# BUTSpeechFIT/TS-ASR-Whisper

Measured on AMD Instinct MI355X. Metric: train utterances/sec (30 s clips) whisper-large-v3-turbo DiCoW, higher is better.
Workload: dtype bf16; 1 GPU; whisper-large-v3-turbo DiCoW fine-tune step, per-GPU batch 16, L=128, decoder frozen, bf16 AMP; global_batch=16, parallelism=dp1, split_streams=False, trainable_params=637306880

## Files before the change

### include/dicow_hip.h

```cpp
#ifndef DICOW_HIP_H
#define DICOW_HIP_H

#include <stdint.h>

#ifdef __cplusplus
extern "C" {
#endif

#define DICOW_OK 0
#define DICOW_ERR_INVALID (-1)
#define DICOW_ERR_LAUNCH (-2)

#define DICOW_ABI_VERSION 7

int dicow_abi_version(void);
int dicow_set_gemm_cus(int n);
int dicow_gemm_dispatch_log(char* buf, int cap);
const char* dicow_last_error(void);

int dicow_cast_f32_to_bf16(const float* src, void* dst, int64_t n, void* stream);
int dicow_cast_transpose_f32_to_bf16(const float* src, void* dst, int64_t ld, void* dst_t, int64_t ld_t, int R, int C,
                                     void* stream);
#define DICOW_CAST_GROUP_MAX 8
typedef struct { const float* src; void* dst; void* dst_t; int R, C; int64_t ld, ld_t; } dicow_cast_problem;
// ... 213 lines not shown

int dicow_embed_fwd(const int64_t* ids, const float* tok, const float* pos, float* out, int B, int Lq, int D, void* stream);
int dicow_embed_bwd(const int64_t* ids, const float* g, float* d_tok, float* d_pos, int B, int Lq, int D, void* stream);

int dicow_gelu_bwd_bf16(const void* g, const void* pre, void* out, int64_t n, void* stream);
int dicow_conv2_col2im_gelu_bwd(const void* dA2, const void* pre1, void* d_pre1, int B, int T2, int C, void* stream);

int64_t dicow_logmel_ws_bytes(int B, int n_samples);
int dicow_logmel(const float* wave, int B, int n_samples, const float* tw_cos, const float* tw_sin, const float* fb,
                 const int* mel_range, int M, float* out, void* ws, int64_t ws_bytes, void* stream);

#define DICOW_NOISE_MIX_CHUNK 8192
int64_t dicow_noise_mix_ws_bytes(int n_plan, int max_len);
int dicow_noise_mix(const float* wave, int64_t ld_wave, float* out, int64_t ld_out, const float* bank, const int64_t* clip_start,
                    const int* clip_len, const int* plan_i, const float* plan_snr, int n_plan, void* ws, int64_t ws_bytes, void* stream);


#define DICOW_DIAR_FRAME 320
#define DICOW_DIAR_BIN 1600
#define DICOW_DIAR_WINDOW 300
#define DICOW_DIAR_MAX_SPEAKERS 64
int64_t dicow_diar_table_ws_bytes(int E);
int64_t dicow_diar_targets_ws_bytes(int n_targets);
int64_t dicow_enrollment_windows_ws_bytes(int64_t n_samples, int n_targets);
int dicow_diar_frame_counts(const int64_t* bounds, const uint64_t* active, int E, int S, int64_t n_samples, int32_t* cnt, int32_t* excl,
                            void* ws, int64_t ws_bytes, void* stream);
int dicow_stno_from_counts(const int32_t* cnt, int S, int64_t n_samples, const int* targets, int n_targets, float* out, int64_t ld_out,
                           void* ws, int64_t ws_bytes, void* stream);
int dicow_enrollment_windows(const int32_t* cnt, const int32_t* excl, int S, int64_t n_samples, const int* targets, int n_targets,
                             int32_t* start, int32_t* count, int32_t* fallback, int32_t* weights, int64_t ld_w, void* ws, int64_t ws_bytes,
                             void* stream);

#define DICOW_ENR_MIX_MAX_TRACKS 8
int dicow_enrollment_mix(float* out, int64_t ld_out, int B, int n, const float* bank, const int64_t* clip_start, const int32_t* plan_dev,
                         const int32_t* plan_host, int n_tracks, const int32_t* clip_len_host, int n_clips, void* stream);

#define DICOW_RESAMPLE_LDS_BYTES 49152
#define DICOW_RESAMPLE_MAX_RATIO 1048576
#define DICOW_RESAMPLE_MAX_CHANNELS 512
int64_t dicow_resample_ws_bytes(int n_segs, int n);
int dicow_resample(const void* in, int in_int16, int C, int channel, int64_t in_frames, float* out, int64_t out_samples, const float* taps_t,
                   const int32_t* first, int o, int n, int width, int S, const int64_t* segs, int n_segs, int frames_per_tile, void* ws,
                   int64_t ws_bytes, void* stream);

#define DICOW_EDIT_MAX_LEN 65535
#define DICOW_EDIT_K 8
#define DICOW_EDIT_LANES 512
#define DICOW_EDIT_LANES_NARROW 64
int64_t dicow_edit_distance_ws_bytes(const int64_t* pairs, int n_pairs);
int dicow_edit_distance(const int32_t* ref_ids, int64_t n_ref, const int32_t* hyp_ids, int64_t n_hyp, const int32_t* ref_iv, const int32_t* hyp_iv,
                        const int64_t* pairs, int n_pairs, int32_t* out, int lanes, int along, void* ws, int64_t ws_bytes, void* stream);

#define DICOW_ALIGN_MAX_WS_BYTES 1073741824LL
#define DICOW_ALIGN_TABLE_BYTES 56
int64_t dicow_edit_alignment_ws_bytes(const int64_t* pairs, int n_pairs, int lanes, int along);
int dicow_edit_alignment(const int32_t* ref_ids, int64_t n_ref, const int32_t* hyp_ids, int64_t n_hyp, const int32_t* ref_iv, const int32_t* hyp_iv,
                         const int64_t* pairs, int n_pairs, int32_t* out, uint8_t* ops, int64_t* spans, int lanes, int along, void* ws,
                         int64_t ws_bytes, void* stream);

#define DICOW_ORC_MAX_STREAMS 8
#define DICOW_ORC_K 8
#define DICOW_ORC_MAX_WORDS 65527
#define DICOW_ORC_MAX_STATES 4194304
#define DICOW_ORC_MAX_WS_BYTES 1073741824LL
#define DICOW_ORC_DESC_BYTES 288
#define DICOW_ORC_UTT_BYTES 16
int64_t dicow_orc_distance_ws_bytes(const int64_t* problems, int n_problems, const int64_t* utts, const int64_t* streams, int want_assignment);
int dicow_orc_distance(const int32_t* ref_ids, int64_t n_ref, const int32_t* hyp_ids, int64_t n_hyp, const int32_t* ref_iv, const int32_t* hyp_iv,
                       const int64_t* problems, int n_problems, const int64_t* utts, const int64_t* streams, int32_t* out, int32_t* assignment,
                       void* ws, int64_t ws_bytes, void* stream);

#define DICOW_DIAR_SCORE_CHUNK 256
#define DICOW_DIAR_SCORE_ROW 12
#define DICOW_DIAR_SCORE_OUT_WORDS 4232
#define DICOW_DIAR_SCORE_DESC_BYTES 120
#define DICOW_DIAR_SCORE_MAX_E 16777216
#define DICOW_DIAR_SCORE_MAX_TICK 1099511627776LL
#define DICOW_DIAR_SCORE_MAX_WS_BYTES 4294967296LL
int64_t dicow_diar_score_ws_bytes(const int64_t* bounds, int64_t n_bounds, const uint64_t* active, int64_t n_active, const int64_t* unscored,
                                  int64_t n_unscored, const int64_t* problems, int n_problems, int chunk);
int dicow_diar_score(const int64_t* bounds, int64_t n_bounds, const uint64_t* active, int64_t n_active, const int64_t* unscored,
                     int64_t n_unscored, const int64_t* problems, int n_problems, int chunk, int64_t* out, void* ws, int64_t ws_bytes,
                     void* stream);

#define DICOW_NGRAM_MAX_N 16
#define DICOW_NGRAM_MAX_WORDS 65535
#define DICOW_NGRAM_PLANS 4
#define DICOW_NGRAM_MAX_WS_BYTES 1073741824LL
#define DICOW_NGRAM_SEG_BYTES 24
#define DICOW_NGRAM_ITEM_BYTES 8
int64_t dicow_ngram_repeats_ws_bytes(const int64_t* table, int n, int plan);
int dicow_ngram_repeats(const int32_t* ids, const int32_t* fold, int64_t n_words, const int64_t* table, int n, int min_n, int max_n,
                        int min_words, int unigram_min_repeat, int repeat_threshold, int32_t* keep, int32_t* reason, int plan, void* ws,
                        int64_t ws_bytes, void* stream);

#define DICOW_BOOT_MAX_N 16777216
#define DICOW_BOOT_MAX_C 32
#define DICOW_BOOT_MAX_R 2147483647LL
#define DICOW_BOOT_LDS_BYTES 65536
#define DICOW_BOOT_PLANS 3
#define DICOW_BOOT_LANE_LDS 1
#define DICOW_BOOT_WAVE_LDS 2
#define DICOW_BOOT_WAVE_L2 3
#define DICOW_BOOT_RESAMPLE 0
#define DICOW_BOOT_SWAP 1
int dicow_bootstrap_plan(int n, int C);
int dicow_bootstrap_sums(const int64_t* table, int64_t ld, int n, int C, const int64_t* strata, const int64_t* strata_dev, int n_strata,
                         int64_t R, uint64_t first_replicate, uint64_t seed, int mode, int plan, int64_t* out, void* stream);

int dicow_stno_noise_rescale(float* stno, const int* rows, const float* noise, int n_rows, int C, int T, float sd,
                             void* stream);
int dicow_stno_segment_augment(float* stno, const int* segs, const float* coef, int n_seg, int C, int T, void* stream);
int dicow_specaug_joint(const float* mel, const float* stno, float* mel_out, float* stno_out, int B, int M, int T, int sub,
                        int center, int warped, const int* fmask, int n_fmask, const int* tmask, int n_tmask,
                        int n_maskable, void* stream);

typedef struct {
    const void* logits; int in_bf16; int64_t ld; const float* lse; const int* alias;
    const int* rows; const int* cs; const int* decoded_len; const int* last; const float* r_prev;
    float* psi; float* r;
    int n, C, T, blank, eos;
} dicow_ctc_prefix_args;
int dicow_ctc_frame_lse(const void* logits, int in_bf16, int64_t rows, int V1, int64_t ld, float* lse, void* stream);
int dicow_ctc_prefix_init(const void* logits, int in_bf16, int64_t ld, const float* lse, int B, int T, int blank_col, float* r0,
                          void* stream);
int dicow_ctc_prefix_score(const dicow_ctc_prefix_args* a, void* stream);

int dicow_whisper_timestamp_rules(float* scores, int64_t ld, int B, int V, const int64_t* input_ids, int L, int begin_index,
                                  int timestamp_begin, int eos, int no_timestamps, int max_initial_timestamp_index,
                                  int detect_from_logprob, void* stream);

int dicow_repetition_rules(float* scores, int64_t ld, int rows, int V, const int64_t* input_ids, int64_t ids_stride, int L,
                           float penalty, int ngram, void* stream);

int dicow_ctc_greedy_decode(const void* logits, int in_bf16, int64_t batch_stride, int64_t ld, int B, int Tn, int V1, int64_t blank,
                            int64_t pad_id, int* ws, int64_t* out, int64_t out_stride, void* stream);

#define DICOW_CTC_ALIGN_MAX_L 511
#define DICOW_CTC_ALIGN_MAX_WS_BYTES 1073741824LL
#define DICOW_CTC_ALIGN_PROB_BYTES 56
int64_t dicow_ctc_align_ws_bytes(const int64_t* table, int n);
int dicow_ctc_forced_align(const void* logits, int in_bf16, int B, int T, int V1, int64_t ld, const float* lse, const int32_t* alias, int blank,
                           const int64_t* table, int n, const int32_t* targets, int64_t n_targets, int32_t* path, int Fmax, int32_t* spans,
                           int Lmax, float* token_score, float* score, int32_t* status, int plan, void* ws, int64_t ws_bytes, void* stream);

int dicow_sumsq_f32(const float* x, int64_t n, float* out, void* stream);
int dicow_fabric_emulate(void* buf, int64_t bytes, double gbps, int workgroups, int passes, void* stream);
int dicow_adamw_f32(float* p, const float* g, float* m, float* v, int64_t n, float lr, float beta1, float beta2,
                    float eps, float weight_decay, int step, const float* gnorm_sq, float max_norm, void* stream);
int dicow_adamw_hyper(int* counters, float* hyper, const int* is_pre, int n_runs, int preheat_only, double lr, double mult,
                      int warmup_steps, int max_steps, int cosine, double beta1, double beta2, void* stream);
int dicow_adamw_f32_dev(float* p, const float* g, float* m, float* v, int64_t n, const float* hyper, float beta1, float beta2,
                        float eps, float weight_decay, const float* gnorm_sq, float max_norm, void* stream);

#define DICOW_MT_CHUNK 2048
#define DICOW_MT_MAX_CLASSES 32
#define DICOW_MT_ALIGNED_ALL 1
#define DICOW_MT_ALIGNED_G   2
typedef struct {
    float* p; float* g; float* m; float* v;
    int64_t n;
    int32_t cls;
    int32_t flags;
} dicow_mt_tensor;
typedef struct { int64_t start; int32_t tensor; int32_t len; } dicow_mt_chunk;
typedef struct {
    float decay[DICOW_MT_MAX_CLASSES]; float step_size[DICOW_MT_MAX_CLASSES]; float bc2_sqrt[DICOW_MT_MAX_CLASSES];
    float lerp_w[DICOW_MT_MAX_CLASSES]; float beta2[DICOW_MT_MAX_CLASSES]; float one_minus_beta2[DICOW_MT_MAX_CLASSES];
    float eps[DICOW_MT_MAX_CLASSES];
    int32_t n_classes;
} dicow_mt_adamw_classes;
int dicow_multi_chunk_elems(void);
int dicow_multi_adamw_f32(const dicow_mt_tensor* tensors, const dicow_mt_chunk* chunks, int64_t n_chunks,
                          const dicow_mt_adamw_classes* cls, int cls_base, const float* clip_coef, void* stream);
int64_t dicow_multi_sumsq_ws_bytes(int64_t n_chunks);
int dicow_multi_sumsq_f32(const dicow_mt_tensor* tensors, const dicow_mt_chunk* chunks, int64_t n_chunks, void* ws, int64_t ws_bytes,
                          float* out, float max_norm, void* stream);
int dicow_multi_scale_f32(const dicow_mt_tensor* tensors, const dicow_mt_chunk* chunks, int64_t n_chunks, const float* coef, void* stream);

#define DICOW_STATS_MAX_BINS 128
typedef struct {
    double sum, sumsq;
    float min, max, absmax;
    int32_t reserved;
    int64_t n_nan, n_posinf, n_neginf, n_zero;
} dicow_tensor_stats_rec;
int64_t dicow_tensor_stats_ws_bytes(int64_t n_tensors, int64_t n_chunks, int bins);
int dicow_tensor_stats_f32(const dicow_mt_tensor* tensors, const dicow_mt_chunk* chunks, int64_t n_tensors, int64_t n_chunks,
                           const int64_t* first_chunk, int which, int bins, void* ws, int64_t ws_bytes,
                           dicow_tensor_stats_rec* out, int64_t* hist, int grid , void* stream);


#ifdef DICOW_EXPERIMENTAL_ABI
#define DICOW_EPI_LNSTAT  2048
#define DICOW_EPI_LNFOLD  4096
#define DICOW_LN_SLOTS 16
int dicow_gemm_nt_lnstat_ok(const dicow_gemm_args* a);
int dicow_lnfold_prep(const float* W, const float* gamma, const float* beta, const float* bias, void* Wf, int64_t ldw, float* c, float* bf,
                      int N, int K, void* stream);
#endif

#ifdef __cplusplus
}
#endif
#endif
```

### ts-asr-whisper_amd/_lib.py

```python
import ctypes as C
import os

_HERE = os.path.dirname(os.path.abspath(__file__))
LIB_PATH = os.environ.get("DICOW_HIP_LIB") or os.path.join(_HERE, "libdicow_hip.so")
_lib = None

c_vp, c_i, c_i64, c_f, c_d = C.c_void_p, C.c_int, C.c_int64, C.c_float, C.c_double
c_u64 = C.c_uint64


class FddtLnFwdArgs(C.Structure):
    _fields_ = [("h_in", c_vp), ("in_bf16", c_i), ("mode", c_i), ("stno", c_vp), ("stno_bstride", c_i64),
                ("w", c_vp * 4), ("b", c_vp * 4), ("pos", c_vp), ("h_out", c_vp), ("ln_w", c_vp), ("ln_b", c_vp),
                ("y_bf16", c_vp), ("y_f32", c_vp), ("mean", c_vp), ("rstd", c_vp),
                ("rows", c_i), ("T", c_i), ("D", c_i), ("eps", c_f)]


class FddtLnBwdArgs(C.Structure):
    _fields_ = [("h_in", c_vp), ("in_bf16", c_i), ("mode", c_i), ("stno", c_vp), ("stno_bstride", c_i64),
                ("w", c_vp * 4), ("b", c_vp * 4), ("pos", c_vp), ("ln_w", c_vp), ("mean", c_vp), ("rstd", c_vp),
                ("d_y", c_vp), ("dy_f32", c_i), ("g_res", c_vp), ("g_out", c_vp), ("g_out_bf16", c_vp),
                ("dln_w", c_vp), ("dln_b", c_vp), ("dw", c_vp * 4), ("db", c_vp * 4), ("colsum_out", c_vp),
                ("dpos_rows", c_vp), ("rows", c_i), ("T", c_i), ("D", c_i), ("ws", c_vp), ("ws_bytes", c_i64)]


class GemmArgs(C.Structure):
    _fields_ = [("A", c_vp), ("B", c_vp), ("C", c_vp), ("bias", c_vp), ("residual", c_vp), ("aux", c_vp),
                ("M", c_i), ("N", c_i), ("K", c_i),
                ("lda", c_i64), ("ldb", c_i64), ("ldc", c_i64), ("ldr", c_i64), ("ldaux", c_i64),
                ("batch", c_i), ("strideA", c_i64), ("strideB", c_i64), ("strideC", c_i64), ("strideAux", c_i64),
                ("flags", c_i), ("scale", c_f), ("scale_ncols", c_i),
                ("colsum_out", c_vp), ("colsum_ws", c_vp), ("colsum_ws_bytes", c_i64),
                ("fddt_w", c_vp * 4), ("fddt_b", c_vp * 4), ("fddt_rowmask", c_vp),
                ("lnstat", c_vp), ("ln_c", c_vp), ("ln_inv_dim", c_f), ("ln_eps", c_f), ("ln_nslots", c_i)]


class GemmTnArgs(C.Structure):
    _fields_ = [("A", c_vp), ("B", c_vp), ("C", c_vp), ("Mk", c_i), ("N1", c_i), ("N2", c_i),
                ("lda", c_i64), ("ldb", c_i64), ("ldc", c_i64),
                ("batch", c_i), ("strideA", c_i64), ("strideB", c_i64), ("accumulate", c_i),
                ("C_seg", c_vp * 2), ("seg_rows", c_i), ("ws", c_vp), ("ws_bytes", c_i64)]


TN_GROUP_MAX = 24
CAST_GROUP_MAX = 8


class CastProblem(C.Structure):
    _fields_ = [("src", c_vp), ("dst", c_vp), ("dst_t", c_vp), ("R", c_i), ("C", c_i), ("ld", c_i64), ("ld_t", c_i64)]


class GemmTnGroupArgs(C.Structure):
    _fields_ = [("n", c_i), ("p", GemmTnArgs * TN_GROUP_MAX), ("ws", c_vp), ("ws_bytes", c_i64)]


class AttnFwdArgs(C.Structure):
    _fields_ = [("q", c_vp), ("k", c_vp), ("v", c_vp), ("o", c_vp), ("lse", c_vp),
                ("q_bs", c_i64), ("q_rs", c_i64), ("k_bs", c_i64), ("k_rs", c_i64),
                ("v_bs", c_i64), ("v_rs", c_i64), ("o_bs", c_i64), ("o_rs", c_i64),
                ("B", c_i), ("H", c_i), ("Lq", c_i), ("Lk", c_i), ("causal", c_i), ("q_log2", c_i)]


class AttnDecodeArgs(C.Structure):
    _fields_ = [("q", c_vp), ("o", c_vp), ("k", c_vp), ("v", c_vp),
                ("q_rs", c_i64), ("o_rs", c_i64), ("k_bs", c_i64), ("k_rs", c_i64), ("v_bs", c_i64), ("v_rs", c_i64),
                ("anc", c_vp), ("anc_rs", c_i64), ("R", c_i), ("H", c_i), ("Lk", c_i), ("group", c_i), ("n_slots", c_i)]


ATTN_DECODE_MAX_GROUP = 8

NOISE_MIX_CHUNK = 8192

DIAR_FRAME, DIAR_BIN, DIAR_WINDOW, DIAR_MAX_SPEAKERS = 320, 1600, 300, 64

ENR_MIX_MAX_TRACKS = 8

RESAMPLE_LDS_BYTES, RESAMPLE_MAX_RATIO, RESAMPLE_MAX_CHANNELS = 49152, 1 << 20, 512

EDIT_MAX_LEN, EDIT_K, EDIT_LANES, EDIT_LANES_NARROW = 65535, 8, 512, 64

ALIGN_MAX_WS_BYTES, ALIGN_TABLE_BYTES = 1 << 30, 56

CTC_ALIGN_MAX_L, CTC_ALIGN_MAX_WS_BYTES, CTC_ALIGN_PROB_BYTES = 511, 1 << 30, 56

ORC_MAX_STREAMS, ORC_K, ORC_MAX_WORDS, ORC_MAX_STATES, ORC_MAX_WS_BYTES, ORC_DESC_BYTES, ORC_UTT_BYTES = 8, 8, 65527, 1 << 22, 1 << 30, 288, 16

DIAR_SCORE_CHUNK, DIAR_SCORE_ROW, DIAR_SCORE_OUT_WORDS, DIAR_SCORE_DESC_BYTES = 256, 12, 4232, 120
DIAR_SCORE_MAX_E, DIAR_SCORE_MAX_TICK, DIAR_SCORE_MAX_WS_BYTES = 1 << 24, 1 << 40, 1 << 32

NGRAM_MAX_N, NGRAM_MAX_WORDS, NGRAM_PLANS, NGRAM_MAX_WS_BYTES, NGRAM_SEG_BYTES, NGRAM_ITEM_BYTES = 16, 65535, 4, 1 << 30, 24, 8
NGRAM_PLAN_TILES = {1: (64, 256), 2: (64, 1024), 3: (256, 256), 4: (256, 1024)}

BOOT_MAX_N, BOOT_MAX_C, BOOT_MAX_R, BOOT_LDS_BYTES, BOOT_PLANS = 1 << 24, 32, (1 << 31) - 1, 65536, 3
BOOT_LANE_LDS, BOOT_WAVE_LDS, BOOT_WAVE_L2 = 1, 2, 3
BOOT_RESAMPLE, BOOT_SWAP = 0, 1

LORA_MAX_R, LORA_MAX_SEG = 192, 24
LORA_BLOCK, LORA_OUT_F32, LORA_GELU, LORA_MUL_AUX = 1, 2, 4, 8


class LoraDownArgs(C.Structure):
    _fields_ = [("X", c_vp), ("V", c_vp), ("T", c_vp), ("ldx", c_i64), ("ldv", c_i64), ("ldt", c_i64),
                ("M", c_i), ("K", c_i), ("R", c_i), ("r", c_i), ("flags", c_i)]


class LoraUpArgs(C.Structure):
    _fields_ = [("T", c_vp), ("U", c_vp), ("P", c_vp), ("Y", c_vp), ("aux", c_vp),
                ("ldt", c_i64), ("ldu", c_i64), ("ldp", c_i64), ("ldy", c_i64), ("ldaux", c_i64),
                ("M", c_i), ("N", c_i), ("R", c_i), ("r", c_i), ("flags", c_i), ("seg_scale", c_f * LORA_MAX_SEG)]


class LoraWgradArgs(C.Structure):
    _fields_ = [("T", c_vp), ("P", c_vp), ("G", c_vp * LORA_MAX_SEG), ("ldt", c_i64), ("ldp", c_i64), ("g_rs", c_i64), ("g_cs", c_i64),
                ("M", c_i), ("N", c_i), ("R", c_i), ("r", c_i), ("flags", c_i), ("scale", c_f), ("accumulate", c_i),
                ("ws", c_vp), ("ws_bytes", c_i64)]


class AttnBwdArgs(C.Structure):
    _fields_ = [("q", c_vp), ("k", c_vp), ("v", c_vp), ("o", c_vp), ("d_o", c_vp), ("lse", c_vp), ("delta", c_vp),
                ("dq", c_vp), ("dk", c_vp), ("dv", c_vp),
                ("q_bs", c_i64), ("q_rs", c_i64), ("k_bs", c_i64), ("k_rs", c_i64), ("v_bs", c_i64), ("v_rs", c_i64),
                ("o_bs", c_i64), ("o_rs", c_i64), ("do_bs", c_i64), ("do_rs", c_i64),
                ("dq_bs", c_i64), ("dq_rs", c_i64), ("dk_bs", c_i64), ("dk_rs", c_i64), ("dv_bs", c_i64), ("dv_rs", c_i64),
                ("B", c_i), ("H", c_i), ("Lq", c_i), ("Lk", c_i), ("causal", c_i), ("dq_scale", c_f),
                ("dq_colsum", c_vp), ("dv_colsum", c_vp), ("cs_ws", c_vp), ("cs_ws_bytes", c_i64), ("q_log2", c_i),
                ("fused_ws", c_vp), ("fused_ws_bytes", c_i64), ("fused_mode", c_i)]


class CeArgs(C.Structure):
    _fields_ = [("logits", c_vp), ("ld", c_i64), ("rows", c_i), ("V", c_i), ("labels", c_vp), ("upp_labels", c_vp),
                ("soft", c_i), ("ts_index", c_vp), ("ts_ids", c_vp), ("ts_w", c_vp), ("n_ts", c_i),
                ("lse", c_vp), ("row_loss", c_vp), ("choice", c_vp), ("loss_sum", c_vp), ("count", c_vp),
                ("d_logits", c_vp)]


class CtcArgs(C.Structure):
    _fields_ = [("logits", c_vp), ("ld", c_i64), ("B", c_i), ("Tn", c_i), ("C", c_i), ("labels", c_vp), ("Lc", c_i),
                ("blank", c_i), ("lse", c_vp), ("alpha", c_vp), ("beta", c_vp), ("Smax", c_i), ("nll", c_vp), ("tlen", c_vp),
                ("loss_sum", c_vp), ("d_logits", c_vp)]


class CtcPrefixArgs(C.Structure):
    _fields_ = [("logits", c_vp), ("in_bf16", c_i), ("ld", c_i64), ("lse", c_vp), ("alias", c_vp), ("rows", c_vp), ("cs", c_vp),
                ("decoded_len", c_vp), ("last", c_vp), ("r_prev", c_vp), ("psi", c_vp), ("r", c_vp), ("n", c_i), ("C", c_i),
                ("T", c_i), ("blank", c_i), ("eos", c_i)]


MT_MAX_CLASSES = 32
STATS_MAX_BINS = 128
STATS_REC_BYTES = 64


class MtAdamwClasses(C.Structure):
    _fields_ = [("decay", c_f * MT_MAX_CLASSES), ("step_size", c_f * MT_MAX_CLASSES), ("bc2_sqrt", c_f * MT_MAX_CLASSES),
                ("lerp_w", c_f * MT_MAX_CLASSES), ("beta2", c_f * MT_MAX_CLASSES), ("one_minus_beta2", c_f * MT_MAX_CLASSES),
                ("eps", c_f * MT_MAX_CLASSES), ("n_classes", C.c_int32)]


EPI_BIAS, EPI_GELU, EPI_RESIDUAL, EPI_OUT_F32, EPI_SCALE_N, EPI_GELU_BWD, EPI_ACCUM = 1, 2, 4, 8, 16, 32, 64
EPI_GELU_DAUX, EPI_MUL_AUX, EPI_COLSUM, EPI_FDDT = 128, 256, 512, 1024
EPI_LNSTAT, EPI_LNFOLD, LN_SLOTS = 2048, 4096, 16

_SIGS = {
    "dicow_set_gemm_cus": [c_i],
    "dicow_cast_transpose_group": [C.POINTER(CastProblem), c_i, c_vp],
    "dicow_gemm_dispatch_log": [c_vp, c_i],
    "dicow_cast_f32_to_bf16": [c_vp, c_vp, c_i64, c_vp],
    "dicow_cast_transpose_f32_to_bf16": [c_vp, c_vp, c_i64, c_vp, c_i64, c_i, c_i, c_vp],
    "dicow_conv_weight_pack": [c_vp, c_vp, c_vp, c_i, c_i, c_i, c_vp],
    "dicow_conv_weight_unpack_grad": [c_vp, c_vp, c_i, c_i, c_i, c_vp],
    "dicow_mel_to_timemajor": [c_vp, c_vp, c_i, c_i, c_i, c_vp],
    "dicow_colsum_bf16": [c_vp, c_i64, c_vp, c_i, c_i, c_vp, c_i64, c_vp],
    "dicow_sum_over_batch": [c_vp, c_vp, c_i, c_i64, c_vp],
    "dicow_scb_split": [c_vp, c_vp, c_vp, c_vp, c_i64, c_i, c_i, c_i, c_vp],
    "dicow_scb_merge_fwd": [c_vp, c_vp, c_vp, c_vp, c_i, c_i, c_i, c_vp],
    "dicow_scb_gate_bwd": [c_vp, c_vp, c_vp, c_vp, c_vp, c_i, c_i, c_i, c_vp, c_i64, c_vp],
    "dicow_scb_merge_bwd": [c_vp, c_vp, c_vp, c_i64, c_vp, c_vp, c_i, c_i, c_i, c_vp],
    "dicow_fddt_ln_fwd": [C.POINTER(FddtLnFwdArgs), c_vp],
    "dicow_fddt_ln_bwd": [C.POINTER(FddtLnBwdArgs), c_vp],
    "dicow_fddt_full_combine_fwd": [c_vp, c_vp, c_i, c_vp, c_i64, c_i, c_vp, c_i, c_i, c_i, c_vp],
    "dicow_fddt_full_combine_bwd": [c_vp, c_vp, c_i64, c_i, c_vp, c_vp, c_i, c_i, c_i, c_vp],
    "dicow_gemm_nt": [C.POINTER(GemmArgs), c_vp],
    "dicow_gemm_nt_is_persistent": [C.POINTER(GemmArgs)],
    "dicow_gemm_tn": [C.POINTER(GemmTnArgs), c_vp],
    "dicow_gemm_tn_group": [C.POINTER(GemmTnGroupArgs), c_vp],
    "dicow_attn_fwd": [C.POINTER(AttnFwdArgs), c_vp],
    "dicow_attn_decode": [C.POINTER(AttnDecodeArgs), c_vp],
    "dicow_lora_down": [C.POINTER(LoraDownArgs), c_vp],
    "dicow_lora_up": [C.POINTER(LoraUpArgs), c_vp],
    "dicow_lora_wgrad": [C.POINTER(LoraWgradArgs), c_vp],
    "dicow_attn_bwd": [C.POINTER(AttnBwdArgs), c_vp],
    "dicow_attn_bwd_fused_status": [c_vp],
    "dicow_attn_bwd_fused_eligible": [c_i, c_i, c_i, c_i, c_i, c_i],
    "dicow_ce_loss_fwd": [C.POINTER(CeArgs), c_vp],
    "dicow_ce_loss_bwd": [C.POINTER(CeArgs), c_vp, c_vp],
    "dicow_ctc_loss_fwd": [C.POINTER(CtcArgs), c_vp],
    "dicow_ctc_loss_bwd": [C.POINTER(CtcArgs), c_vp, c_vp],
    "dicow_embed_fwd": [c_vp, c_vp, c_vp, c_vp, c_i, c_i, c_i, c_vp],
    "dicow_embed_bwd": [c_vp, c_vp, c_vp, c_vp, c_i, c_i, c_i, c_vp],
    "dicow_gelu_bwd_bf16": [c_vp, c_vp, c_vp, c_i64, c_vp],
    "dicow_conv2_col2im_gelu_bwd": [c_vp, c_vp, c_vp, c_i, c_i, c_i, c_vp],
    "dicow_logmel": [c_vp, c_i, c_i, c_vp, c_vp, c_vp, c_vp, c_i, c_vp, c_vp, c_i64, c_vp],
    "dicow_stno_noise_rescale": [c_vp, c_vp, c_vp, c_i, c_i, c_i, c_f, c_vp],
    "dicow_stno_segment_augment": [c_vp, c_vp, c_vp, c_i, c_i, c_i, c_vp],
    "dicow_specaug_joint": [c_vp, c_vp, c_vp, c_vp, c_i, c_i, c_i, c_i, c_i, c_i, c_vp, c_i, c_vp, c_i, c_i, c_vp],
    "dicow_ctc_frame_lse": [c_vp, c_i, c_i64, c_i, c_i64, c_vp, c_vp],
    "dicow_ctc_prefix_init": [c_vp, c_i, c_i64, c_vp, c_i, c_i, c_i, c_vp, c_vp],
    "dicow_ctc_prefix_score": [C.POINTER(CtcPrefixArgs), c_vp],
    "dicow_whisper_timestamp_rules": [c_vp, c_i64, c_i, c_i, c_vp, c_i, c_i, c_i, c_i, c_i, c_i, c_i, c_vp],
    "dicow_repetition_rules": [c_vp, c_i64, c_i, c_i, c_vp, c_i64, c_i, c_f, c_i, c_vp],
    "dicow_ctc_greedy_decode": [c_vp, c_i, c_i64, c_i64, c_i, c_i, c_i, c_i64, c_i64, c_vp, c_vp, c_i64, c_vp],
    "dicow_ctc_forced_align": [c_vp, c_i, c_i, c_i, c_i, c_i64, c_vp, c_vp, c_i, c_vp, c_i, c_vp, c_i64, c_vp, c_i, c_vp, c_i, c_vp, c_vp, c_vp,
                               c_i, c_vp, c_i64, c_vp],
    "dicow_noise_mix": [c_vp, c_i64, c_vp, c_i64, c_vp, c_vp, c_vp, c_vp, c_vp, c_i, c_vp, c_i64, c_vp],
    "dicow_diar_frame_counts": [c_vp, c_vp, c_i, c_i, c_i64, c_vp, c_vp, c_vp, c_i64, c_vp],
    "dicow_stno_from_counts": [c_vp, c_i, c_i64, c_vp, c_i, c_vp, c_i64, c_vp, c_i64, c_vp],
    "dicow_enrollment_windows": [c_vp, c_vp, c_i, c_i64, c_vp, c_i, c_vp, c_vp, c_vp, c_vp, c_i64, c_vp, c_i64, c_vp],
    "dicow_enrollment_mix": [c_vp, c_i64, c_i, c_i, c_vp, c_vp, c_vp, c_vp, c_i, c_vp, c_i, c_vp],
    "dicow_resample": [c_vp, c_i, c_i, c_i, c_i64, c_vp, c_i64, c_vp, c_vp, c_i, c_i, c_i, c_i, c_vp, c_i, c_i, c_vp, c_i64, c_vp],
    "dicow_edit_distance": [c_vp, c_i64, c_vp, c_i64, c_vp, c_vp, c_vp, c_i, c_vp, c_i, c_i, c_vp, c_i64, c_vp],
    "dicow_edit_alignment": [c_vp, c_i64, c_vp, c_i64, c_vp, c_vp, c_vp, c_i, c_vp, c_vp, c_vp, c_i, c_i, c_vp, c_i64, c_vp],
    "dicow_orc_distance": [c_vp, c_i64, c_vp, c_i64, c_vp, c_vp, c_vp, c_i, c_vp, c_vp, c_vp, c_vp, c_vp, c_i64, c_vp],
    "dicow_diar_score": [c_vp, c_i64, c_vp, c_i64, c_vp, c_i64, c_vp, c_i, c_i, c_vp, c_vp, c_i64, c_vp],
    "dicow_ngram_repeats": [c_vp, c_vp, c_i64, c_vp, c_i, c_i, c_i, c_i, c_i, c_i, c_vp, c_vp, c_i, c_vp, c_i64, c_vp],
    "dicow_bootstrap_plan": [c_i, c_i],
    "dicow_bootstrap_sums": [c_vp, c_i64, c_i, c_i, c_vp, c_vp, c_i, c_i64, c_u64, c_u64, c_i, c_i, c_vp, c_vp],
    "dicow_sumsq_f32": [c_vp, c_i64, c_vp, c_vp],
    "dicow_fabric_emulate": [c_vp, c_i64, c_d, c_i, c_i, c_vp],
    "dicow_adamw_f32": [c_vp, c_vp, c_vp, c_vp, c_i64, c_f, c_f, c_f, c_f, c_f, c_i, c_vp, c_f, c_vp],
    "dicow_adamw_hyper": [c_vp, c_vp, c_vp, c_i, c_i, c_d, c_d, c_i, c_i, c_i, c_d, c_d, c_vp],
    "dicow_adamw_f32_dev": [c_vp, c_vp, c_vp, c_vp, c_i64, c_vp, c_f, c_f, c_f, c_f, c_vp, c_f, c_vp],
    "dicow_multi_chunk_elems": [],
    "dicow_multi_adamw_f32": [c_vp, c_vp, c_i64, C.POINTER(MtAdamwClasses), c_i, c_vp, c_vp],
    "dicow_multi_sumsq_f32": [c_vp, c_vp, c_i64, c_vp, c_i64, c_vp, c_f, c_vp],
    "dicow_multi_scale_f32": [c_vp, c_vp, c_i64, c_vp, c_vp],
    "dicow_tensor_stats_f32": [c_vp, c_vp, c_i64, c_i64, c_vp, c_i, c_i, c_vp, c_i64, c_vp, c_vp, c_i, c_vp],
}


_SIGS_EXPERIMENTAL = {
    "dicow_gemm_nt_lnstat_ok": [C.POINTER(GemmArgs)],
    "dicow_lnfold_prep": [c_vp, c_vp, c_vp, c_vp, c_vp, c_i64, c_vp, c_vp, c_i, c_i, c_vp],
}


class DicowError(RuntimeError):
    pass


def lib():
    global _lib
    if _lib is None:
        if not os.path.exists(LIB_PATH):
            raise DicowError(f"{LIB_PATH} is missing: build it with ts-asr-whisper_amd/csrc/build.sh "
                             "(or __graft_entry__.build()); there is no CPU fallback")
        l = C.CDLL(LIB_PATH)
        l.dicow_abi_version.restype = c_i
        l.dicow_last_error.restype = C.c_char_p
        for name, at in _SIGS.items():
            fn = getattr(l, name)
            fn.argtypes = at
            fn.restype = c_i
        for name, at in _SIGS64.items():
            fn = getattr(l, name)
            fn.argtypes = at
            fn.restype = c_i64
        for name, at in _SIGS_STR.items():
            fn = getattr(l, name)
            fn.argtypes = at
            fn.restype = C.c_char_p
        l._dicow_experimental = True
        for name, at in _SIGS_EXPERIMENTAL.items():
            try:
                fn = getattr(l, name)
            except AttributeError:
                l._dicow_experimental = False
                continue
            fn.argtypes = at
            fn.restype = c_i
        _lib = l
    return _lib


def has_experimental():
    return bool(lib()._dicow_experimental)


_SIGS64 = {
    "dicow_colsum_ws_bytes": [c_i, c_i],
    "dicow_gemm_nt_colsum_ws_bytes": [c_i, c_i],
    "dicow_attn_bwd_colsum_ws_bytes": [c_i, c_i, c_i, c_i],
    "dicow_attn_bwd_fused_ws_bytes": [c_i, c_i, c_i, c_i],
    "dicow_fddt_ln_bwd_ws_bytes": [c_i, c_i],
    "dicow_gemm_tn_ws_bytes": [C.POINTER(GemmTnArgs)],
    "dicow_gemm_nt_splitk_ws_bytes": [C.POINTER(GemmArgs)],
    "dicow_gemm_tn_group_ws_bytes": [C.POINTER(GemmTnGroupArgs)],
    "dicow_logmel_ws_bytes": [c_i, c_i],
    "dicow_scb_gate_bwd_ws_bytes": [],
    "dicow_ctc_ws_bytes": [c_i, c_i, c_i],
    "dicow_multi_sumsq_ws_bytes": [c_i64],
    "dicow_tensor_stats_ws_bytes": [c_i64, c_i64, c_i],
    "dicow_lora_wgrad_ws_bytes": [c_i, c_i, c_i, c_i, c_i],
    "dicow_noise_mix_ws_bytes": [c_i, c_i],
    "dicow_diar_table_ws_bytes": [c_i],
    "dicow_diar_targets_ws_bytes": [c_i],
    "dicow_enrollment_windows_ws_bytes": [c_i64, c_i],
    "dicow_resample_ws_bytes": [c_i, c_i],
    "dicow_edit_distance_ws_bytes": [c_vp, c_i],
    "dicow_edit_alignment_ws_bytes": [c_vp, c_i, c_i, c_i],
    "dicow_ctc_align_ws_bytes": [c_vp, c_i],
    "dicow_orc_distance_ws_bytes": [c_vp, c_i, c_vp, c_vp, c_i],
    "dicow_diar_score_ws_bytes": [c_vp, c_i64, c_vp, c_i64, c_vp, c_i64, c_vp, c_i, c_i],
    "dicow_ngram_repeats_ws_bytes": [c_vp, c_i, c_i],
}


_SIGS_STR = {
    "dicow_fddt_ln_fwd_route": [C.POINTER(FddtLnFwdArgs)],
    "dicow_fddt_ln_bwd_route": [C.POINTER(FddtLnBwdArgs)],
    "dicow_attn_fwd_route": [C.POINTER(AttnFwdArgs)],
    "dicow_attn_bwd_route": [C.POINTER(AttnBwdArgs)],
}


def declared_symbols():
    return ["dicow_abi_version", "dicow_last_error"] + list(_SIGS) + list(_SIGS64) + list(_SIGS_STR)


def check(rc, what):
    if rc != 0:
        raise DicowError(f"{what} failed ({rc}): {lib().dicow_last_error().decode()}")


def ptr(t):
    return None if t is None else t.data_ptr()


def stream():
    import torch
    return torch.cuda.current_stream().cuda_stream


def call(name, *args):
    check(getattr(lib(), name)(*args), name)


def call_struct(name, st):
    check(getattr(lib(), name)(C.byref(st), stream()), name)
```

### ts-asr-whisper_amd/csrc/elementwise.hip

```cpp
#include <stdarg.h>
#include <new>
#include "host_table.h"

static thread_local char g_err[512] = "";

void dicow_set_error(const char* fmt, ...) {
    va_list ap;
    va_start(ap, fmt);
    vsnprintf(g_err, sizeof(g_err), fmt, ap);
    va_end(ap);
}

int dicow_upload(const char* who, void* dst, const void* src, int64_t bytes, hipStream_t stream) {
    if (bytes == 0) return DICOW_OK;
    hipStreamCaptureStatus cs = hipStreamCaptureStatusNone;
    if (hipStreamIsCapturing(stream, &cs) != hipSuccess) (void)hipGetLastError();
    if (cs == hipStreamCaptureStatusActive) src = memcpy(::operator new((size_t)bytes), src, (size_t)bytes);
    hipError_t e = hipMemcpyAsync(dst, src, (size_t)bytes, hipMemcpyHostToDevice, stream);
    if (e != hipSuccess) DICOW_FAIL(DICOW_ERR_LAUNCH, "%s: table upload: %s", who, hipGetErrorString(e));
    return DICOW_OK;
}

extern "C" int dicow_abi_version(void) { return DICOW_ABI_VERSION; }
extern "C" const char* dicow_last_error(void) { return g_err; }

__global__ void cast_f32_bf16_kernel(const float* __restrict__ src, unsigned short* __restrict__ dst, int64_t n) {
    const int64_t n4 = n >> 2;
    const int64_t stride = (int64_t)gridDim.x * blockDim.x;
    for (int64_t i = (int64_t)blockIdx.x * blockDim.x + threadIdx.x; i < n4; i += stride) {
        const float4 v = reinterpret_cast<const float4*>(src)[i];
        reinterpret_cast<uint2*>(dst)[i] = make_uint2(pack_bf16x2(v.x, v.y), pack_bf16x2(v.z, v.w));
    }
    for (int64_t i = (n4 << 2) + (int64_t)blockIdx.x * blockDim.x + threadIdx.x; i < n; i += stride)
        dst[i] = f2bfbits(src[i]);
}

extern "C" int dicow_cast_f32_to_bf16(const float* src, void* dst, int64_t n, void* stream) {
    DICOW_REQUIRE(src && dst && n > 0, "cast_f32_to_bf16: bad args");
    int grid = (int)((n / 4 + 255) / 256);
    if (grid < 1) grid = 1;
    if (grid > 4096) grid = 4096;
    hipLaunchKernelGGL(cast_f32_bf16_kernel, dim3(grid), dim3(256), 0, (hipStream_t)stream, src, (unsigned short*)dst, n);
    DICOW_CHECK_LAUNCH("cast_f32_to_bf16");
    return DICOW_OK;
}

__global__ void cast_transpose_kernel(const float* __restrict__ src, unsigned short* __restrict__ dst,
                                      unsigned short* __restrict__ dst_t, int R, int C, int64_t ld, int64_t ld_t) {
    __shared__ unsigned short tile[64][66];
    const int r0 = blockIdx.y * 64, c0 = blockIdx.x * 64;
    const int tx = threadIdx.x & 63, ty = threadIdx.x >> 6;
    for (int i = ty; i < 64; i += 4) {
        const int r = r0 + i, c = c0 + tx;
        unsigned short v = 0;
        if (r < R && c < C) {
            v = f2bfbits(src[(int64_t)r * C + c]);
            if (dst) dst[(int64_t)r * ld + c] = v;
        }
        tile[i][tx] = v;
    }
    __syncthreads();
    if (!dst_t) return;
    for (int i = ty; i < 64; i += 4) {
        const int c = c0 + i, r = r0 + tx;
        if (r < R && c < C) dst_t[(int64_t)c * ld_t + r] = tile[tx][i];
    }
}

__global__ void cast_transpose4_kernel(const float* __restrict__ src, unsigned short* __restrict__ dst,
                                       unsigned short* __restrict__ dst_t, int R, int C, int64_t ld, int64_t ld_t) {
    __shared__ unsigned short tile[64][68];
    const int r0 = blockIdx.y * 64, c0 = blockIdx.x * 64;
    const int tq = threadIdx.x & 15, tr = threadIdx.x >> 4;
#pragma unroll
    for (int k = 0; k < 4; ++k) {
        const int i = k * 16 + tr, r = r0 + i, c = c0 + tq * 4;
        uint2 u = make_uint2(0, 0);
        if (r < R && c < C) {
            const float4 f = *reinterpret_cast<const float4*>(src + (int64_t)r * C + c);
            u = make_uint2(pack_bf16x2(f.x, f.y), pack_bf16x2(f.z, f.w));
            if (dst) *reinterpret_cast<uint2*>(dst + (int64_t)r * ld + c) = u;
        }
        *reinterpret_cast<uint2*>(&tile[i][tq * 4]) = u;
    }
    __syncthreads();
    if (!dst_t) return;
#pragma unroll
    for (int k = 0; k < 4; ++k) {
        const int i = k * 16 + tr, c = c0 + i, r = r0 + tq * 4;
        if (c < C && r < R) {
            const unsigned lo = (unsigned)tile[tq * 4][i] | ((unsigned)tile[tq * 4 + 1][i] << 16);
            const unsigned hi = (unsigned)tile[tq * 4 + 2][i] | ((unsigned)tile[tq * 4 + 3][i] << 16);
            *reinterpret_cast<uint2*>(dst_t + (int64_t)c * ld_t + r) = make_uint2(lo, hi);
        }
    }
}

extern "C" int dicow_cast_transpose_f32_to_bf16(const float* src, void* dst, int64_t ld, void* dst_t, int64_t ld_t, int R,
                                                int C, void* stream) {
    DICOW_REQUIRE(src && (dst || dst_t) && R > 0 && C > 0, "cast_transpose: bad args");
    DICOW_REQUIRE((!dst || ld >= C) && (!dst_t || ld_t >= R), "cast_transpose: leading dimensions too small");
    dim3 grid(dicow_cdiv(C, 64), dicow_cdiv(R, 64));
    const bool vec = (R % 4 == 0) && (C % 4 == 0) && (ld % 4 == 0) && (ld_t % 4 == 0) &&
                     ((uintptr_t)src % 16 == 0) && ((uintptr_t)dst % 8 == 0) && ((uintptr_t)dst_t % 8 == 0);
    if (vec)
        hipLaunchKernelGGL(cast_transpose4_kernel, grid, dim3(256), 0, (hipStream_t)stream, src, (unsigned short*)dst,
                           (unsigned short*)dst_t, R, C, ld, ld_t);
    else
        hipLaunchKernelGGL(cast_transpose_kernel, grid, dim3(256), 0, (hipStream_t)stream, src, (unsigned short*)dst,
                           (unsigned short*)dst_t, R, C, ld, ld_t);
    DICOW_CHECK_LAUNCH("cast_transpose");
    return DICOW_OK;
}

struct cast_group_kargs_t { dicow_cast_problem p[DICOW_CAST_GROUP_MAX]; int tile0[DICOW_CAST_GROUP_MAX + 1]; int n; };
__global__ void cast_transpose4_group_kernel(const cast_group_kargs_t g) {
    __shared__ unsigned short tile[64][68];
    int pi = 0;
#pragma unroll
    for (int i = 1; i < DICOW_CAST_GROUP_MAX; ++i) if (i < g.n && (int)blockIdx.x >= g.tile0[i]) pi = i;
    const dicow_cast_problem& q = g.p[pi];
    const int R = q.R, C = q.C;
    const int64_t ld = q.ld, ld_t = q.ld_t;
    const float* __restrict__ src = q.src;
    unsigned short* __restrict__ dst = reinterpret_cast<unsigned short*>(q.dst);
    unsigned short* __restrict__ dst_t = reinterpret_cast<unsigned short*>(q.dst_t);
    const int lb = (int)blockIdx.x - g.tile0[pi], ntc = (C + 63) / 64;
    const int r0 = (lb / ntc) * 64, c0 = (lb % ntc) * 64;
    const int tq = threadIdx.x & 15, tr = threadIdx.x >> 4;
#pragma unroll
    for (int k = 0; k < 4; ++k) {
        const int i = k * 16 + tr, r = r0 + i, c = c0 + tq * 4;
        uint2 u = make_uint2(0, 0);
        if (r < R && c < C) {
            const float4 f = *reinterpret_cast<const float4*>(src + (int64_t)r * C + c);
            u = make_uint2(pack_bf16x2(f.x, f.y), pack_bf16x2(f.z, f.w));
            if (dst) *reinterpret_cast<uint2*>(dst + (int64_t)r * ld + c) = u;
        }
        *reinterpret_cast<uint2*>(&tile[i][tq * 4]) = u;
    }
    __syncthreads();
    if (!dst_t) return;
#pragma unroll
    for (int k = 0; k < 4; ++k) {
        const int i = k * 16 + tr, c = c0 + i, r = r0 + tq * 4;
        if (c < C && r < R) {
            const unsigned lo = (unsigned)tile[tq * 4][i] | ((unsigned)tile[tq * 4 + 1][i] << 16);
            const unsigned hi = (unsigned)tile[tq * 4 + 2][i] | ((unsigned)tile[tq * 4 + 3][i] << 16);
            *reinterpret_cast<uint2*>(dst_t + (int64_t)c * ld_t + r) = make_uint2(lo, hi);
        }
    }
}

extern "C" int dicow_cast_transpose_group(const dicow_cast_problem* p, int n, void* stream) {
// ... 363 lines not shown
    __threadfence();
    float t = 0.f;
    for (int i = threadIdx.x; i < (int)gridDim.x; i += 256) t += __builtin_nontemporal_load(&g_sumsq_part[i]);
    t = wave_sum(t);
    if ((threadIdx.x & 63) == 0) red[threadIdx.x >> 6] = t;
    __syncthreads();
    if (threadIdx.x == 0) {
        out[0] += (red[0] + red[1]) + (red[2] + red[3]);
        g_sumsq_ticket = 0;
    }
}

__global__ void __launch_bounds__(256) fabric_emulate_kernel(f32x4_t* buf, int64_t n16, double ticks_per_f4_per_block, int passes) {
    const int64_t per = (n16 + gridDim.x - 1) / gridDim.x, lo = per * blockIdx.x, hi = lo + per < n16 ? lo + per : n16;
    const long long t0 = wall_clock64();
    int64_t done = 0;
    for (int p = 0; p < passes; ++p)
        for (int64_t i = lo; i < hi; i += 256 * 16) {
            f32x4_t v[16];
#pragma unroll
            for (int k = 0; k < 16; ++k) { const int64_t j = i + k * 256 + threadIdx.x; if (j < hi) v[k] = __builtin_nontemporal_load(buf + j); }
#pragma unroll
            for (int k = 0; k < 16; ++k) { const int64_t j = i + k * 256 + threadIdx.x; if (j < hi) __builtin_nontemporal_store(v[k], buf + j); }
            done += (hi - i < 256 * 16 ? hi - i : 256 * 16);
            const long long due = t0 + (long long)((double)done * ticks_per_f4_per_block / passes);
            while (wall_clock64() < due) __builtin_amdgcn_s_sleep(32);
        }
}

extern "C" int dicow_fabric_emulate(void* buf, int64_t bytes, double gbps, int workgroups, int passes, void* stream) {
    DICOW_REQUIRE(buf && bytes > 0 && bytes % 16 == 0 && gbps > 0.0 && workgroups > 0 && workgroups <= 1024 && passes > 0 && passes <= 8,
                  "fabric_emulate: bad arguments");
    const int64_t n16 = bytes / 16;
    const double ticks_total = (double)bytes / (gbps * 1e9) * 1e8;
    const double per_block_f4 = (double)((n16 + workgroups - 1) / workgroups);
    hipLaunchKernelGGL(fabric_emulate_kernel, dim3(workgroups), dim3(256), 0, (hipStream_t)stream, reinterpret_cast<f32x4_t*>(buf), n16,
                       ticks_total / per_block_f4, passes);
    DICOW_CHECK_LAUNCH("fabric_emulate");
    return DICOW_OK;
}

extern "C" int dicow_sumsq_f32(const float* x, int64_t n, float* out, void* stream) {
    DICOW_REQUIRE(x && out && n > 0, "sumsq_f32: bad args");
    int grid = (int)((n / 4 + 255) / 256); if (grid < 1) grid = 1; if (grid > SUMSQ_MAX_BLOCKS) grid = SUMSQ_MAX_BLOCKS;
    hipLaunchKernelGGL(sumsq_kernel, dim3(grid), dim3(256), 0, (hipStream_t)stream, x, n, out);
    DICOW_CHECK_LAUNCH("sumsq_f32");
    return DICOW_OK;
}

#ifndef ADAMW_NT
#define ADAMW_NT 0
#endif
typedef __attribute__((ext_vector_type(4))) float f32x4a_t;
__global__ void adamw_kernel(float* __restrict__ p, const float* __restrict__ g, float* __restrict__ m, float* __restrict__ v,
                             int64_t n, float lr, float b1, float b2, float eps, float wd, float bc1, float bc2,
                             const float* __restrict__ gnorm_sq, float max_norm, const float* __restrict__ hyper) {
    if (hyper) { lr = hyper[0]; bc1 = hyper[1]; bc2 = hyper[2]; }
    float clip = 1.f;
    if (gnorm_sq && max_norm > 0.f) {
        const float c = max_norm / (sqrtf(gnorm_sq[0]) + 1e-6f);
        clip = c < 1.f ? c : 1.f;
    }
    const int64_t n4 = n >> 2;
    for (int64_t i = (int64_t)blockIdx.x * blockDim.x + threadIdx.x; i < n4; i += (int64_t)gridDim.x * blockDim.x) {
        float4 pp, gg, mm, vv;
        if (ADAMW_NT & 1) {
            const f32x4a_t p_ = __builtin_nontemporal_load(reinterpret_cast<const f32x4a_t*>(p) + i), g_ = __builtin_nontemporal_load(reinterpret_cast<const f32x4a_t*>(g) + i);
            const f32x4a_t m_ = __builtin_nontemporal_load(reinterpret_cast<const f32x4a_t*>(m) + i), v_ = __builtin_nontemporal_load(reinterpret_cast<const f32x4a_t*>(v) + i);
            pp = make_float4(p_.x, p_.y, p_.z, p_.w); gg = make_float4(g_.x, g_.y, g_.z, g_.w);
            mm = make_float4(m_.x, m_.y, m_.z, m_.w); vv = make_float4(v_.x, v_.y, v_.z, v_.w);
        } else {
            pp = reinterpret_cast<float4*>(p)[i]; gg = reinterpret_cast<const float4*>(g)[i];
            mm = reinterpret_cast<float4*>(m)[i]; vv = reinterpret_cast<float4*>(v)[i];
        }
        float* pa = &pp.x; float* ga = &gg.x; float* ma = &mm.x; float* va = &vv.x;
#pragma unroll
        for (int e = 0; e < 4; ++e) {
            const float gr = ga[e] * clip;
            pa[e] *= 1.f - lr * wd;
            ma[e] = b1 * ma[e] + (1.f - b1) * gr;
            va[e] = b2 * va[e] + (1.f - b2) * gr * gr;
            const float denom = sqrtf(va[e]) / sqrtf(bc2) + eps;
            pa[e] -= (lr / bc1) * (ma[e] / denom);
        }
        if (ADAMW_NT & 2) {
            __builtin_nontemporal_store(f32x4a_t{pp.x, pp.y, pp.z, pp.w}, reinterpret_cast<f32x4a_t*>(p) + i);
            __builtin_nontemporal_store(f32x4a_t{mm.x, mm.y, mm.z, mm.w}, reinterpret_cast<f32x4a_t*>(m) + i);
            __builtin_nontemporal_store(f32x4a_t{vv.x, vv.y, vv.z, vv.w}, reinterpret_cast<f32x4a_t*>(v) + i);
        } else {
            reinterpret_cast<float4*>(p)[i] = pp; reinterpret_cast<float4*>(m)[i] = mm; reinterpret_cast<float4*>(v)[i] = vv;
        }
    }
    for (int64_t i = (n4 << 2) + (int64_t)blockIdx.x * blockDim.x + threadIdx.x; i < n; i += (int64_t)gridDim.x * blockDim.x) {
        const float gr = g[i] * clip;
        float pv = p[i] * (1.f - lr * wd);
        const float mv = b1 * m[i] + (1.f - b1) * gr, vv2 = b2 * v[i] + (1.f - b2) * gr * gr;
        pv -= (lr / bc1) * (mv / (sqrtf(vv2) / sqrtf(bc2) + eps));
        p[i] = pv; m[i] = mv; v[i] = vv2;
    }
}

extern "C" int dicow_adamw_f32(float* p, const float* g, float* m, float* v, int64_t n, float lr, float beta1, float beta2,
                               float eps, float weight_decay, int step, const float* gnorm_sq, float max_norm, void* stream) {
    DICOW_REQUIRE(p && g && m && v && n > 0 && step >= 1, "adamw_f32: bad args");
    const float bc1 = 1.f - powf(beta1, (float)step), bc2 = 1.f - powf(beta2, (float)step);
    int grid = (int)((n / 4 + 255) / 256); if (grid < 1) grid = 1; if (grid > 4096) grid = 4096;
    hipLaunchKernelGGL(adamw_kernel, dim3(grid), dim3(256), 0, (hipStream_t)stream, p, g, m, v, n, lr, beta1, beta2, eps,
                       weight_decay, bc1, bc2, gnorm_sq, max_norm, (const float*)nullptr);
    DICOW_CHECK_LAUNCH("adamw_f32");
    return DICOW_OK;
}

__global__ void adamw_hyper_kernel(int* __restrict__ counters, float* __restrict__ hyper, const int* __restrict__ is_pre, int n_runs,
                                   int preheat_only, double lr, double mult, int warmup, int max_steps, int cosine, double b1, double b2) {
    const int k = counters[0] + 1;
    __syncthreads();
    if (threadIdx.x == 0) counters[0] = k;
    const int ss = k - 1;
    double l = lr;
    if (ss < warmup) l = lr * (double)ss / (double)(warmup > 1 ? warmup : 1);
    else if (cosine && max_steps > 0) {
        const double prog = (double)(ss - warmup) / (double)((max_steps - warmup) > 1 ? (max_steps - warmup) : 1);
        const double c = 0.5 * (1.0 + cos(3.14159265358979323846 * prog));
        l = lr * (c > 0.0 ? c : 0.0);
    }
    for (int i = threadIdx.x; i < n_runs; i += blockDim.x) {
        const int pre = is_pre[i];
        if (preheat_only && !pre) continue;
        const int t = counters[1 + i] + 1;
        counters[1 + i] = t;
        hyper[3 * i] = (float)(l * (pre ? mult : 1.0));
        hyper[3 * i + 1] = (float)(1.0 - pow(b1, (double)t));
        hyper[3 * i + 2] = (float)(1.0 - pow(b2, (double)t));
    }
}

extern "C" int dicow_adamw_hyper(int* counters, float* hyper, const int* is_pre, int n_runs, int preheat_only, double lr, double mult,
                                 int warmup_steps, int max_steps, int cosine, double beta1, double beta2, void* stream) {
    DICOW_REQUIRE(counters && hyper && is_pre && n_runs > 0, "adamw_hyper: bad args");
    const int block = n_runs >= 1024 ? 1024 : (n_runs + 63) / 64 * 64;
    hipLaunchKernelGGL(adamw_hyper_kernel, dim3(1), dim3(block), 0, (hipStream_t)stream, counters, hyper, is_pre, n_runs, preheat_only,
                       lr, mult, warmup_steps, max_steps, cosine, beta1, beta2);
    DICOW_CHECK_LAUNCH("adamw_hyper");
    return DICOW_OK;
}

extern "C" int dicow_adamw_f32_dev(float* p, const float* g, float* m, float* v, int64_t n, const float* hyper, float beta1,
                                   float beta2, float eps, float weight_decay, const float* gnorm_sq, float max_norm, void* stream) {
    DICOW_REQUIRE(p && g && m && v && n > 0 && hyper, "adamw_f32_dev: bad args");
    int grid = (int)((n / 4 + 255) / 256); if (grid < 1) grid = 1; if (grid > 4096) grid = 4096;
    hipLaunchKernelGGL(adamw_kernel, dim3(grid), dim3(256), 0, (hipStream_t)stream, p, g, m, v, n, 0.f, beta1, beta2, eps,
                       weight_decay, 1.f, 1.f, gnorm_sq, max_norm, hyper);
    DICOW_CHECK_LAUNCH("adamw_f32_dev");
    return DICOW_OK;
}

__device__ __forceinline__ float4 bf4_to_f4(uint2 u) {
    return make_float4(__uint_as_float(u.x << 16), __uint_as_float(u.x & 0xffff0000u), __uint_as_float(u.y << 16), __uint_as_float(u.y & 0xffff0000u));
}
__global__ void scb_split_kernel(const float* __restrict__ hf, unsigned short* __restrict__ q_in, unsigned short* __restrict__ kv_in,
                                 unsigned short* __restrict__ cat, int64_t td, int D, int64_t ldcat, int Bp) {
    const int64_t n4 = (int64_t)Bp * td / 4;
    for (int64_t i = (int64_t)blockIdx.x * blockDim.x + threadIdx.x; i < n4; i += (int64_t)gridDim.x * blockDim.x) {
        const int64_t e = i * 4, b = e / td, off = e - b * td;
        const float4 m = *reinterpret_cast<const float4*>(hf + (2 * b) * td + off);
        const float4 r = *reinterpret_cast<const float4*>(hf + (2 * b + 1) * td + off);
        const uint2 mb = make_uint2(pack_bf16x2(m.x, m.y), pack_bf16x2(m.z, m.w));
        *reinterpret_cast<uint2*>(q_in + e) = mb;
        *reinterpret_cast<uint2*>(kv_in + e) = make_uint2(pack_bf16x2(r.x, r.y), pack_bf16x2(r.z, r.w));
        const int64_t row = e / D; const int col = (int)(e - row * D);
        *reinterpret_cast<uint2*>(cat + row * ldcat + D + col) = mb;
    }
}
__global__ void scb_merge_fwd_kernel(const float* __restrict__ hf, const unsigned short* __restrict__ upd, const float* __restrict__ gate,
                                     float* __restrict__ out, int64_t td, int Bp) {
    const float tg = tanhf(gate[0]);
    const int64_t n4 = (int64_t)2 * Bp * td / 4;
    for (int64_t i = (int64_t)blockIdx.x * blockDim.x + threadIdx.x; i < n4; i += (int64_t)gridDim.x * blockDim.x) {
        const int64_t e = i * 4, slot = e / td, off = e - slot * td;
        float4 v = *reinterpret_cast<const float4*>(hf + e);
        if ((slot & 1) == 0) {
            const float4 u = bf4_to_f4(*reinterpret_cast<const uint2*>(upd + (slot >> 1) * td + off));
            v.x += u.x * tg; v.y += u.y * tg; v.z += u.z * tg; v.w += u.w * tg;
        }
        *reinterpret_cast<float4*>(out + e) = v;
    }
}
__global__ void __launch_bounds__(256) scb_gate_bwd_kernel(const float* __restrict__ g, const unsigned short* __restrict__ upd,
                                                           const float* __restrict__ gate, unsigned short* __restrict__ d_upd,
                                                           float* __restrict__ partial, int64_t td, int Bp) {
    __shared__ float red[4];
    const float tg = tanhf(gate[0]);
    const int64_t n4 = (int64_t)Bp * td / 4;
    float acc = 0.f;
    for (int64_t i = (int64_t)blockIdx.x * blockDim.x + threadIdx.x; i < n4; i += (int64_t)gridDim.x * blockDim.x) {
        const int64_t e = i * 4, b = e / td, off = e - b * td;
        const float4 gq = *reinterpret_cast<const float4*>(g + (2 * b) * td + off);
        const float4 u = bf4_to_f4(*reinterpret_cast<const uint2*>(upd + e));
        acc += (gq.x * u.x + gq.y * u.y) + (gq.z * u.z + gq.w * u.w);
        *reinterpret_cast<uint2*>(d_upd + e) = make_uint2(pack_bf16x2(gq.x * tg, gq.y * tg), pack_bf16x2(gq.z * tg, gq.w * tg));
    }
    acc = wave_sum(acc);
    if ((threadIdx.x & 63) == 0) red[threadIdx.x >> 6] = acc;
    __syncthreads();
    if (threadIdx.x == 0) partial[blockIdx.x] = (red[0] + red[1]) + (red[2] + red[3]);
}
__global__ void scb_gate_finish_kernel(const float* __restrict__ partial, int n, const float* __restrict__ gate, float* __restrict__ d_gate) {
    __shared__ float red[256];
    float t = 0.f;
    for (int i = threadIdx.x; i < n; i += 256) t += partial[i];
    red[threadIdx.x] = t;
    __syncthreads();
    for (int o = 128; o > 0; o >>= 1) { if ((int)threadIdx.x < o) red[threadIdx.x] += red[threadIdx.x + o]; __syncthreads(); }
    if (threadIdx.x == 0) { const float tg = tanhf(gate[0]); d_gate[0] += red[0] * (1.f - tg * tg); }
}
__global__ void scb_merge_bwd_kernel(const float* __restrict__ g, const float* __restrict__ d_qin, const unsigned short* __restrict__ d_cat,
                                     int64_t ldcat, const float* __restrict__ d_kvin, float* __restrict__ gin, int64_t td, int D, int Bp) {
    const int64_t n4 = (int64_t)2 * Bp * td / 4;
    for (int64_t i = (int64_t)blockIdx.x * blockDim.x + threadIdx.x; i < n4; i += (int64_t)gridDim.x * blockDim.x) {
        const int64_t e = i * 4, slot = e / td, off = e - slot * td, b = slot >> 1, pe = b * td + off;
        float4 v = *reinterpret_cast<const float4*>(g + e);
        if ((slot & 1) == 0) {
            const float4 a = *reinterpret_cast<const float4*>(d_qin + pe);
            const int64_t row = pe / D; const int col = (int)(pe - row * D);
            const float4 c = bf4_to_f4(*reinterpret_cast<const uint2*>(d_cat + row * ldcat + D + col));
            v.x += a.x + c.x; v.y += a.y + c.y; v.z += a.z + c.z; v.w += a.w + c.w;
        } else {
            const float4 a = *reinterpret_cast<const float4*>(d_kvin + pe);
            v.x += a.x; v.y += a.y; v.z += a.z; v.w += a.w;
        }
        *reinterpret_cast<float4*>(gin + e) = v;
    }
}
static int scb_grid(int64_t n4) { int64_t g = (n4 + 255) / 256; return (int)(g > 2048 ? 2048 : (g < 1 ? 1 : g)); }
#define SCB_CHECK(name) DICOW_REQUIRE(Bp > 0 && T > 0 && D > 0 && D % 4 == 0, name ": bad shape")
extern "C" int dicow_scb_split(const float* hf, void* q_in, void* kv_in, void* cat, int64_t ldcat, int Bp, int T, int D, void* stream) {
    DICOW_REQUIRE(hf && q_in && kv_in && cat && ldcat >= 2 * D && ldcat % 4 == 0, "scb_split: bad args");
    SCB_CHECK("scb_split");
    const int64_t td = (int64_t)T * D;
    hipLaunchKernelGGL(scb_split_kernel, dim3(scb_grid(Bp * td / 4)), dim3(256), 0, (hipStream_t)stream, hf, (unsigned short*)q_in,
                       (unsigned short*)kv_in, (unsigned short*)cat, td, D, ldcat, Bp);
    DICOW_CHECK_LAUNCH("scb_split");
    return DICOW_OK;
}
extern "C" int dicow_scb_merge_fwd(const float* hf, const void* upd, const float* gate, float* out, int Bp, int T, int D, void* stream) {
    DICOW_REQUIRE(hf && upd && gate && out, "scb_merge_fwd: null operand");
    SCB_CHECK("scb_merge_fwd");
    const int64_t td = (int64_t)T * D;
    hipLaunchKernelGGL(scb_merge_fwd_kernel, dim3(scb_grid(2 * Bp * td / 4)), dim3(256), 0, (hipStream_t)stream, hf,
                       (const unsigned short*)upd, gate, out, td, Bp);
    DICOW_CHECK_LAUNCH("scb_merge_fwd");
    return DICOW_OK;
}
extern "C" int64_t dicow_scb_gate_bwd_ws_bytes(void) { return 1024 * 4; }
extern "C" int dicow_scb_gate_bwd(const float* g, const void* upd, const float* gate, void* d_upd, float* d_gate, int Bp, int T, int D,
                                  void* ws, int64_t ws_bytes, void* stream) {
    DICOW_REQUIRE(g && upd && gate && d_upd && ws && ws_bytes >= 1024 * 4, "scb_gate_bwd: bad args (ws: dicow_scb_gate_bwd_ws_bytes)");
    SCB_CHECK("scb_gate_bwd");
    const int64_t td = (int64_t)T * D;
    int grid = scb_grid(Bp * td / 4); if (grid > 1024) grid = 1024;
    hipLaunchKernelGGL(scb_gate_bwd_kernel, dim3(grid), dim3(256), 0, (hipStream_t)stream, g, (const unsigned short*)upd, gate,
                       (unsigned short*)d_upd, (float*)ws, td, Bp);
    DICOW_CHECK_LAUNCH("scb_gate_bwd");
    if (d_gate) {
        hipLaunchKernelGGL(scb_gate_finish_kernel, dim3(1), dim3(256), 0, (hipStream_t)stream, (const float*)ws, grid, gate, d_gate);
        DICOW_CHECK_LAUNCH("scb_gate_finish");
    }
    return DICOW_OK;
}
extern "C" int dicow_scb_merge_bwd(const float* g, const float* d_qin, const void* d_cat, int64_t ldcat, const float* d_kvin, float* gin,
                                   int Bp, int T, int D, void* stream) {
    DICOW_REQUIRE(g && d_qin && d_cat && d_kvin && gin && ldcat >= 2 * D && ldcat % 4 == 0, "scb_merge_bwd: bad args");
    SCB_CHECK("scb_merge_bwd");
    const int64_t td = (int64_t)T * D;
    hipLaunchKernelGGL(scb_merge_bwd_kernel, dim3(scb_grid(2 * Bp * td / 4)), dim3(256), 0, (hipStream_t)stream, g, d_qin,
                       (const unsigned short*)d_cat, ldcat, d_kvin, gin, td, D, Bp);
    DICOW_CHECK_LAUNCH("scb_merge_bwd");
    return DICOW_OK;
}

#ifdef DICOW_EXPERIMENTS
__global__ void __launch_bounds__(256) lnfold_prep_kernel(const float* __restrict__ W, const float* __restrict__ gamma,
                                                          const float* __restrict__ beta, const float* __restrict__ bias,
                                                          unsigned short* __restrict__ Wf, int64_t ldw, float* __restrict__ c,
                                                          float* __restrict__ bf, int K) {
    __shared__ float red[2][4];
    const int n = blockIdx.x;
    const float* w = W + (int64_t)n * K;
    unsigned short* o = Wf + (int64_t)n * ldw;
    float sc = 0.f, sb = 0.f;
    for (int k = threadIdx.x * 2; k < K; k += 512) {
        const float w0 = w[k], w1 = w[k + 1];
        const unsigned pf = pack_bf16x2(w0 * gamma[k], w1 * gamma[k + 1]);
        *reinterpret_cast<unsigned*>(o + k) = pf;
        sc += __uint_as_float(pf << 16) + __uint_as_float(pf & 0xffff0000u);
        const unsigned pw = pack_bf16x2(w0, w1);
        sb = fmaf(beta[k], __uint_as_float(pw << 16), sb);
        sb = fmaf(beta[k + 1], __uint_as_float(pw & 0xffff0000u), sb);
    }
    sc = wave_sum_dpp(sc); sb = wave_sum_dpp(sb);
    if ((threadIdx.x & 63) == 0) { red[0][threadIdx.x >> 6] = sc; red[1][threadIdx.x >> 6] = sb; }
    __syncthreads();
    if (threadIdx.x == 0) {
        c[n] = (red[0][0] + red[0][1]) + (red[0][2] + red[0][3]);
        bf[n] = (bias ? bias[n] : 0.f) + ((red[1][0] + red[1][1]) + (red[1][2] + red[1][3]));
    }
// ... 13 lines not shown
```

### ts-asr-whisper_amd/engine.py

```python
import contextlib
import os
from types import SimpleNamespace as NS

import torch

from . import _lib as L
from . import ops

BF16, F32 = torch.bfloat16, torch.float32
CLS = ("silence_linear", "target_linear", "non_target_linear", "overlap_linear")


def _e(shape, dtype, dev):
    return torch.empty(shape, dtype=dtype, device=dev)


def _ceil(a, b):
    return (a + b - 1) // b * b


SPLIT_FWD = os.environ.get("DICOW_SPLIT_FWD", "1") != "0"
SPLIT_FWD_MIN_ROWS = int(os.environ.get("DICOW_SPLIT_FWD_MIN_ROWS", "16000"))
SPLIT_DEC = os.environ.get("DICOW_SPLIT_DEC", "1") != "0"
SPLIT_BWD = os.environ.get("DICOW_SPLIT_BWD", "1") != "0"
SPLIT_BWD_WGRAD = os.environ.get("DICOW_SPLIT_BWD_WGRAD", "alt")
SPLIT_BWD_MEM_FRACTION = float(os.environ.get("DICOW_SPLIT_BWD_MEM_FRACTION", "0.6"))
_FWD_STREAMS = {}
if SPLIT_BWD_WGRAD not in ("alt", "main"):
    raise ValueError(f"DICOW_SPLIT_BWD_WGRAD must be 'alt' or 'main', not {SPLIT_BWD_WGRAD!r}")


def _split_allowed():
    return not torch.cuda.is_current_stream_capturing()


def fwd_side_stream(dev, k=0):
    cur = torch.cuda.current_stream(dev)
    key = (dev.index, cur.cuda_stream, k)
    st = _FWD_STREAMS.get(key)
    if st is None:
        st = _FWD_STREAMS[key] = torch.cuda.Stream(device=dev, priority=-1)
    return st


def _fwd_parts(B, T, dev):
    main_st, side_st, Bh = torch.cuda.current_stream(dev), fwd_side_stream(dev), B // 2
    side_st.wait_stream(main_st)
    return main_st, [(main_st, slice(0, Bh * T), slice(0, Bh)), (side_st, slice(Bh * T, B * T), slice(Bh, B))], Bh


def _one_part(B):
    return ((None, slice(None), slice(0, B)),)


def _on(st):
    return torch.cuda.stream(st) if st is not None else contextlib.nullcontext()


class GradSink:

    def __init__(self, params, dev, extra_rows=None):
        self.index, self.direct = {}, {}
        off = 0
        extra_rows = extra_rows or {}
        for p in params:
            if p is None or not p.requires_grad or id(p) in self.index or id(p) in self.direct:
                continue
            if getattr(p, "_direct_grad", None) is not None:
                self.direct[id(p)] = p._direct_grad
                continue
            n = p.numel() + extra_rows.get(id(p), 0)
            self.index[id(p)] = (off, p.shape, p.numel())
            off += _ceil(n, 64)
        self.flat = torch.zeros(max(off, 1), dtype=F32, device=dev)

    def get(self, p):
        if p is None:
            return None
        if id(p) in self.direct:
            return self.direct[id(p)]
        if id(p) not in self.index:
            return None
        off, shape, n = self.index[id(p)]
        return self.flat[off:off + n].view(shape)

    def result(self, p):
        return None if (p is None or id(p) in self.direct) else self.get(p)

    def is_direct(self, p):
        return p is not None and id(p) in self.direct

    def raw(self, p, n):
        if id(p) in self.direct:
            d = self.direct[id(p)]
            assert d.numel() == n, "GradSink.raw: a flat-store gradient has no padding rows"
            return d.view(-1)
        off, _, _ = self.index[id(p)]
        return self.flat[off:off + n]


class LinW:
    __slots__ = ("w", "wt", "b", "N", "K")


_BIAS_COPIES = None


def prep_linear(weights, biases, dev, need_t=True, n_pad=None, scale_info=None, bias_buf=None):
    K = weights[0].shape[1]
    Ns = [w.shape[0] for w in weights]
    N = sum(Ns)
    Np = N if n_pad is None else n_pad
    lw = LinW()
    lw.N, lw.K = Np, K
    lw.w = torch.zeros(Np, K, dtype=BF16, device=dev) if Np != N else _e((Np, K), BF16, dev)
    lw.wt = (torch.zeros(K, Np, dtype=BF16, device=dev) if Np != N else _e((K, Np), BF16, dev)) if need_t else None
    off = 0
    for w, n in zip(weights, Ns):
        ops.cast_transpose_bf16(w.detach(), out=lw.w[off:off + n], out_t=None if lw.wt is None else lw.wt[:, off:off + n],
                                ld=K, ld_t=Np)
        off += n
    if biases is None or all(b is None for b in biases):
        lw.b = None
    else:
        if bias_buf is not None and _BIAS_COPIES is not None and len(Ns) > 1:
            off = 0
            for b, n in zip(biases, Ns):
                if b is not None:
                    _BIAS_COPIES.append((bias_buf[off:off + n], b.detach()))
                off += n
            lw.b = bias_buf
        else:
            parts = [(b.detach() if b is not None else torch.zeros(n, dtype=F32, device=dev)) for b, n in zip(biases, Ns)]
            lw.b = parts[0] if len(parts) == 1 else torch.cat(parts)
    return lw


def prep_attention(att, dev, fuse_qkv=True, bias_buf=None):
    a = NS()
    if fuse_qkv:
        a.qkv = prep_linear([att.q_proj.weight, att.k_proj.weight, att.v_proj.weight],
                            [att.q_proj.bias, None, att.v_proj.bias], dev, bias_buf=bias_buf)
    else:
        a.q = prep_linear([att.q_proj.weight], [att.q_proj.bias], dev)
        a.kv = prep_linear([att.k_proj.weight, att.v_proj.weight], [None, att.v_proj.bias], dev)
    a.o = prep_linear([att.out_proj.weight], [att.out_proj.bias], dev)
    return a


def fddt_ptrs(fddt, cfg):
    if fddt is None:
        return ops.MODE_NONE, (None,) * 4, (None,) * 4
    w, b = [], []
    for c in CLS:
        m = getattr(fddt, c, None)
        if fddt.bias_only:
            w.append(None)
            b.append(None if m is None else m)
        else:
            w.append(None if m is None else m.weight)
            b.append(None if m is None else m.bias)
    return (ops.MODE_BIAS if fddt.bias_only else ops.MODE_DIAG), tuple(w), tuple(b)


def fddt_is_full(fddt):
    return fddt is not None and not fddt.is_diagonal


def prep_full_fddt(fddt, dev):
    D = fddt.d_model
    w = NS(use=0)
    w.Wc = torch.zeros(4 * D, D, dtype=BF16, device=dev)
    w.Wct = torch.zeros(D, 4 * D, dtype=BF16, device=dev)
    w.bias = torch.zeros(4 * D, dtype=F32, device=dev)
    for c, name in enumerate(CLS):
        m = getattr(fddt, name, None)
        if m is not None:
            w.use |= 1 << c
            ops.cast_transpose_bf16(m.weight.detach(), out=w.Wc[c * D:(c + 1) * D], out_t=w.Wct[:, c * D:(c + 1) * D], ld=D, ld_t=4 * D)
            w.bias[c * D:(c + 1) * D] = m.bias.detach()
    return w


def full_fddt_fwd(w, h, stno, bstride, rows, T, D):
    hb = h if h.dtype == BF16 else ops.cast_bf16(h)
    y4 = _e((rows, 4 * D), BF16, h.device)
    ops.gemm_nt(hb, w.Wc, y4, rows, 4 * D, D, bias=w.bias)
    out = _e((rows, D), F32, h.device)
    L.call("dicow_fddt_full_combine_fwd", y4.data_ptr(), h.data_ptr(), int(h.dtype == BF16), stno.data_ptr(), bstride, w.use,
           out.data_ptr(), rows, T, D, L.stream())
    return out, hb


def full_fddt_bwd(fddt, w, hb, g, stno, bstride, G, rows, T, D):
    dev = g.device
    d_y4 = torch.zeros(rows, 4 * D, dtype=BF16, device=dev)
    gh = _e((rows, D), F32, dev)
    L.call("dicow_fddt_full_combine_bwd", g.data_ptr(), stno.data_ptr(), bstride, w.use, d_y4.data_ptr(), gh.data_ptr(), rows, T, D,
           L.stream())
    ops.gemm_nt(d_y4, w.Wct, gh, rows, D, 4 * D, flags=L.EPI_ACCUM)
    for c, name in enumerate(CLS):
        m = getattr(fddt, name, None)
        if m is None:
            continue
        sl = d_y4[:, c * D:(c + 1) * D]
        if G.get(m.bias) is not None:
            ops.colsum_bf16(sl, G.get(m.bias))
        if G.get(m.weight) is not None:
            ops.gemm_tn(sl, hb, G.get(m.weight), rows, D, D, lda=4 * D, ldb=D, ldc=D)
    return gh


QK_LOG2 = True
FUSE_NEXT_FDDT = True
LN_FOLD = os.environ.get("DICOW_LN_FOLD", "0") == "1"
Q_SCALE = 0.125 * (ops.LOG2E if QK_LOG2 else 1.0)


def linear_fwd(x, lw, M, out_dtype=BF16, residual=None, gelu_aux=None, flags=0, scale=1.0, scale_ncols=0, out=None, fddt=None):
    dev = x.device
    if out is None:
        out = _e((M, lw.N), out_dtype, dev)
    ops.gemm_nt(x, lw.w, out, M, lw.N, lw.K, bias=lw.b, residual=residual, aux=gelu_aux,
                flags=flags | ((L.EPI_GELU | L.EPI_GELU_DAUX) if gelu_aux is not None else 0), scale=scale, scale_ncols=scale_ncols, fddt=fddt)
    return out


def linear_dgrad(dy, lw, M, aux=None, out=None, out_dtype=BF16, accumulate=False, dy_cols=None, colsum_out=None):
    N = lw.N if dy_cols is None else dy_cols
    if out is None:
        out = _e((M, lw.K), out_dtype, dy.device)
    flags = (L.EPI_MUL_AUX if aux is not None else 0) | (L.EPI_ACCUM if accumulate else 0)
    ops.gemm_nt(dy, lw.wt, out, M, lw.K, N, lda=dy.stride(0), ldb=lw.wt.stride(0), aux=aux, flags=flags, colsum_out=colsum_out)
    return out


def _first_writer(*params):
    if not params or not all(getattr(p, "_grad_overwrite", False) for p in params):
        return False
    for p in params:
        p._grad_overwrite = False
    return True


def linear_wgrad(dy, x, gw, M, n_rows=None, group=None, param=None):
    if gw is None:
        return
    N = dy.shape[1] if n_rows is None else n_rows
    acc = not (param is not None and _first_writer(param))
    if group is not None:
        group.add(dy, x, gw, M, N, x.shape[1], lda=dy.stride(0), ldb=x.stride(0), ldc=gw.stride(0), accumulate=acc)
        return
    ops.gemm_tn(dy, x, gw, M, N, x.shape[1], lda=dy.stride(0), ldb=x.stride(0), ldc=gw.stride(0), accumulate=acc)


class LoraW:
    __slots__ = ("mods", "r", "s", "R", "K", "N", "A", "Bt")

    def refresh(self):
        r = self.r
        for j, m in enumerate(self.mods):
            ops.cast_transpose_bf16(m.lora_A.weight.detach(), out=self.A[j * r:(j + 1) * r], ld=self.K)
            ops.cast_transpose_bf16(m.lora_B.weight.detach(), out_t=self.Bt[j * r:(j + 1) * r], ld_t=self.N)


def prep_lora(mods, dev):
    has = [hasattr(m, "lora_A") for m in mods]
    if not any(has):
        return None
    if not all(has) or len({(m.r, m.lora_alpha) for m in mods}) != 1:
        raise NotImplementedError("LoRA: the projections of one fused Linear (q/k/v, k/v) must all carry adapters of one rank and alpha")
    la = LoraW()
    la.mods, la.r, la.s = list(mods), mods[0].r, mods[0].scaling
    la.R, la.K, la.N = la.r * len(mods), mods[0].in_features, mods[0].out_features
    la.A, la.Bt = _e((la.R, la.K), BF16, dev), _e((la.R, la.N), BF16, dev)
    la.refresh()
    return la


def lora_fwd(x, la, y, M, q_scale=None, gelu=False, gelu_aux=None):
    if la is None:
        return None
    t = _e((M, la.R), BF16, x.device)
    ops.lora_down(x, la.A, t, la.r)
    scales = [la.s] * len(la.mods)
    if q_scale is not None:
        scales[0] *= q_scale
    ops.lora_up(t, la.Bt, y, y, la.r, scales, block=True, gelu=gelu, aux=gelu_aux)
    return t


def lora_bwd(dy, x, t, la, M, G, dx=None, mul_aux=None, dx_out=None):
    if la is None:
        return
    r = la.r
    dt = _e((M, la.R), BF16, dy.device)
    ops.lora_down(dy, la.Bt, dt, r, block=True)
    gB = [G.get(m.lora_B.weight) for m in la.mods]
    gA = [G.get(m.lora_A.weight) for m in la.mods]
# ... 26 lines not shown
    if gb is not None:
        ops.colsum_bf16(dy, gb)


def heads(t, B, Lx, H):
    return t.as_strided((B, Lx, H, 64), (Lx * t.stride(0), t.stride(0), 64, 1), t.storage_offset())


def _fddt_kw(fddt, bsl, T):
    if fddt is None:
        return {}
    mode, fw, fb, stno, bstride = fddt
    return dict(mode=mode, stno=stno[bsl.start * (bstride // (4 * T)):], stno_bstride=bstride, T=T, w=fw, b=fb)


def layer_fwd_buffers(Ls, B, T, H, F_, own_hp):
    h = Ls.h_in
    (rows, D), dev = h.shape, h.device
    Ls.xln, Ls.mean, Ls.rstd = _e((rows, D), BF16, dev), _e((rows,), F32, dev), _e((rows,), F32, dev)
    Ls.hp = _e((rows, D), F32, dev) if own_hp else h
    Ls.qkv, Ls.o, Ls.lse = _e((rows, 3 * D), BF16, dev), _e((rows, D), BF16, dev), _e((B, H, T), F32, dev)
    Ls.h2, Ls.xln2 = _e((rows, D), F32, dev), _e((rows, D), BF16, dev)
    Ls.mean2, Ls.rstd2 = _e((rows,), F32, dev), _e((rows,), F32, dev)
    Ls.u, Ls.a = _e((rows, F_), BF16, dev), _e((rows, F_), BF16, dev)
    return _e((rows, D), F32, dev)


def layer_rows_fwd(lyr, w, Ls, hn, r, bsl, Bh, T, H, fddt=None):
    rh, D = Bh * T, Ls.xln.shape[1]
    ln, ln2 = lyr.self_attn_layer_norm, lyr.final_layer_norm
    ops.fddt_ln_fwd(Ls.h_in[r], rh, D, h_out=Ls.hp[r] if Ls.hp is not Ls.h_in else None, ln_w=ln.weight.detach(), ln_b=ln.bias.detach(),
                    y_bf16=Ls.xln[r], mean=Ls.mean[r], rstd=Ls.rstd[r], **_fddt_kw(fddt, bsl, T))
    qkv, o = Ls.qkv[r], Ls.o[r]
    linear_fwd(Ls.xln[r], w.att.qkv, rh, flags=L.EPI_SCALE_N, scale=Q_SCALE, scale_ncols=D, out=qkv)
    ops.attn_fwd(heads(qkv[:, :D], Bh, T, H), heads(qkv[:, D:2 * D], Bh, T, H), heads(qkv[:, 2 * D:], Bh, T, H), heads(o, Bh, T, H),
                 Ls.lse[bsl], q_log2=QK_LOG2)
    linear_fwd(o, w.att.o, rh, out_dtype=F32, residual=Ls.hp[r], out=Ls.h2[r])
    ops.fddt_ln_fwd(Ls.h2[r], rh, D, mode=ops.MODE_NONE, ln_w=ln2.weight.detach(), ln_b=ln2.bias.detach(), y_bf16=Ls.xln2[r],
                    mean=Ls.mean2[r], rstd=Ls.rstd2[r])
    linear_fwd(Ls.xln2[r], w.fc1, rh, gelu_aux=Ls.u[r], out=Ls.a[r])
    linear_fwd(Ls.a[r], w.fc2, rh, out_dtype=F32, residual=Ls.h2[r], out=hn[r])


def layer_bwd_buffers(rows, D, F_, dev, tail=True, g0b=True):
    bf = NS()
    bf.d_u, bf.d_xln2 = _e((rows, F_), BF16, dev), _e((rows, D), BF16, dev)
    bf.g2, bf.g2b, bf.d_o = _e((rows, D), F32, dev), _e((rows, D), BF16, dev), _e((rows, D), BF16, dev)
    bf.d_qkv, bf.d_xln = _e((rows, 3 * D), BF16, dev), _e((rows, D), BF16, dev)
    bf.g0 = _e((rows, D), F32, dev) if tail else None
    bf.g0b = _e((rows, D), BF16, dev) if (tail and g0b) else None
    return bf


def layer_rows_bwd(lyr, w, Ls, bf, r, bsl, Bh, T, H, g, gb, gg, tail=True, fddt=None, prev_b2=None):
    rh, D = Bh * T, gb.shape[1]
    att, ln, ln2 = lyr.self_attn, lyr.self_attn_layer_norm, lyr.final_layer_norm
    linear_dgrad(gb[r], w.fc2, rh, aux=Ls.u[r], colsum_out=gg(lyr.fc1.bias), out=bf.d_u[r])
    linear_dgrad(bf.d_u[r], w.fc1, rh, out=bf.d_xln2[r])
    ops.fddt_ln_bwd(Ls.h2[r], rh, D, mode=ops.MODE_NONE, ln_w=ln2.weight.detach(), mean=Ls.mean2[r], rstd=Ls.rstd2[r], d_y=bf.d_xln2[r],
                    g_res=g[r], g_out=bf.g2[r], g_out_bf16=bf.g2b[r], dln_w=gg(ln2.weight), dln_b=gg(ln2.bias),
                    colsum_out=gg(att.out_proj.bias))
    linear_dgrad(bf.g2b[r], w.att.o, rh, out=bf.d_o[r])
    delta = _e((2, Bh, H, T), F32, gb.device)
    qkv, d_qkv = Ls.qkv[r], bf.d_qkv[r]
    ops.attn_bwd(heads(qkv[:, :D], Bh, T, H), heads(qkv[:, D:2 * D], Bh, T, H), heads(qkv[:, 2 * D:], Bh, T, H), heads(Ls.o[r], Bh, T, H),
                 heads(bf.d_o[r], Bh, T, H), Ls.lse[bsl], delta, heads(d_qkv[:, :D], Bh, T, H), heads(d_qkv[:, D:2 * D], Bh, T, H),
                 heads(d_qkv[:, 2 * D:], Bh, T, H), dq_scale=0.125, q_log2=QK_LOG2, dq_colsum=gg(att.q_proj.bias),
                 dv_colsum=gg(att.v_proj.bias))
    linear_dgrad(d_qkv, w.att.qkv, rh, out=bf.d_xln[r])
    if tail:
        fk = _fddt_kw(fddt, bsl, T)
        if fddt is not None:
            fk.update(dw=tuple(gg(x) for x in fddt[1]), db=tuple(gg(x) for x in fddt[2]))
        ops.fddt_ln_bwd(Ls.h_in[r], rh, D, ln_w=ln.weight.detach(), mean=Ls.mean[r], rstd=Ls.rstd[r], d_y=bf.d_xln[r], g_res=bf.g2[r],
                        g_out=bf.g0[r], g_out_bf16=bf.g0b[r] if bf.g0b is not None else None, dln_w=gg(ln.weight), dln_b=gg(ln.bias),
                        colsum_out=gg(prev_b2), **fk)
    return delta


def layer_wgrads(lyr, Ls, bf, gb, G, rows, group=None):
    att = lyr.self_attn
    linear_wgrad(gb, Ls.a, G.get(lyr.fc2.weight), rows, group=group, param=lyr.fc2.weight)
    linear_wgrad(bf.d_u, Ls.xln2, G.get(lyr.fc1.weight), rows, group=group, param=lyr.fc1.weight)
    linear_wgrad(bf.g2b, Ls.o, G.get(att.out_proj.weight), rows, group=group, param=att.out_proj.weight)
    qkv_wgrad(bf.d_qkv, Ls.xln, G.get(att.q_proj.weight), G.get(att.k_proj.weight), G.get(att.v_proj.weight), rows, gb.shape[1], group=group,
              params=(att.q_proj.weight, att.k_proj.weight, att.v_proj.weight))


def plain_layer_fwd(lyr, w, h, B, T, H, F_):
    s = NS(h_in=h)
    hn = layer_fwd_buffers(s, B, T, H, F_, own_hp=False)
    layer_rows_fwd(lyr, w, s, hn, slice(None), slice(0, B), B, T, H)
    return hn, s


def plain_layer_bwd(lyr, w, s, gb, G, B, T, H):
    rows, D = gb.shape
    g = gb.float()
    bias_grad(gb, G.get(lyr.fc2.bias))
    bf = layer_bwd_buffers(rows, D, w.fc1.N, gb.device, g0b=False)
    layer_rows_bwd(lyr, w, s, bf, slice(None), slice(0, B), B, T, H, g, gb, G.get)
    layer_wgrads(lyr, s, bf, gb, G, rows)
    return bf.g0


def conv_stem_fwd(enc, W, input_features, need_grad=True):
    dev = input_features.device
    B, M, Tin = input_features.shape
    T, D = Tin // 2, enc.conv1.weight.shape[0]
    xt = torch.zeros(B * (Tin + 2) * M + W.k1, dtype=BF16, device=dev)
    ops.mel_to_timemajor(input_features.to(F32), out=xt)
    g1p = _e((B, Tin + 2, D), BF16, dev)
    g1p[:, 0].zero_()
    g1p[:, Tin + 1].zero_()
    pre1 = _e((B, Tin, D), BF16, dev) if need_grad else None
    ops.gemm_nt(xt, W.conv1, g1p[:, 1:], Tin, D, W.k1, lda=M, bias=enc.conv1.bias.detach(), aux=pre1, flags=L.EPI_GELU,
                batch=B, strideA=(Tin + 2) * M, strideC=(Tin + 2) * D, strideAux=Tin * D)
    x2 = _e((B * T, D), BF16, dev)
    pre2 = _e((B * T, D), BF16, dev) if need_grad else None
    ops.gemm_nt(g1p, W.conv2, x2, T, D, 3 * D, lda=2 * D, bias=enc.conv2.bias.detach(), aux=pre2, flags=L.EPI_GELU,
                batch=B, strideA=(Tin + 2) * D, strideC=T * D, strideAux=T * D)
    return x2, NS(xt=xt, g1p=g1p, pre1=pre1, pre2=pre2, B=B, T=T, M=M)


def conv_stem_bwd(enc, W, st, d_x2, G):
    dev = d_x2.device
    B, T, M = st.B, st.T, st.M
    Tin, rows, D = 2 * T, B * T, d_x2.shape[1]
    d_pre2 = _e((rows, D), BF16, dev)
    ops.gelu_bwd_bf16(d_x2, st.pre2, d_pre2)
    bias_grad(d_pre2, G.get(enc.conv2.bias))
    gw2 = G.get(enc.conv2.weight)
    if gw2 is not None:
        tmp = torch.zeros(D, 3 * D, dtype=F32, device=dev)
        ops.gemm_tn(d_pre2, st.g1p, tmp, T, D, 3 * D, lda=D, ldb=2 * D, batch=B, strideA=T * D, strideB=(Tin + 2) * D)
        ops.conv_weight_unpack_grad(tmp, gw2)
    dA2 = _e((rows, 3 * D), BF16, dev)
    ops.gemm_nt(d_pre2, W.conv2_t, dA2, rows, 3 * D, D)
    d_pre1 = _e((B, Tin, D), BF16, dev)
    ops.conv2_col2im_gelu_bwd(dA2, st.pre1, d_pre1, B, T, D)
    bias_grad(d_pre1.view(B * Tin, D), G.get(enc.conv1.bias))
    gw1 = G.get(enc.conv1.weight)
    if gw1 is not None:
        tmp = torch.zeros(D, W.k1, dtype=F32, device=dev)
        ops.gemm_tn(d_pre1, st.xt, tmp, Tin, D, W.k1, lda=D, ldb=M, batch=B, strideA=Tin * D, strideB=(Tin + 2) * M)
        ops.conv_weight_unpack_grad(tmp, gw1)


class EncoderEngine:
    def __init__(self, enc):
        self.enc = enc
        self.cfg = enc.config

    def prepare(self):
        enc, cfg = self.enc, self.cfg
        dev = enc.conv1.weight.device
        D, M = cfg.d_model, cfg.num_mel_bins
        W = NS()
        W.k1 = _ceil(3 * M, 64)
        W.conv1, W.conv1_t = ops.conv_weight_pack(enc.conv1.weight.detach(), W.k1, want_t=True)
        W.conv2, W.conv2_t = ops.conv_weight_pack(enc.conv2.weight.detach(), 3 * D, want_t=True)
        W.layers = []
        global _BIAS_COPIES
        if getattr(self, "_qkv_bias", None) is None or self._qkv_bias[0].device != dev:
            self._qkv_bias = [torch.zeros(3 * D, dtype=F32, device=dev) for _ in enc.layers]
        _BIAS_COPIES = []
        for li, lyr in enumerate(enc.layers):
            w = NS()
            with ops.cast_group():
                w.att = prep_attention(lyr.self_attn, dev, bias_buf=self._qkv_bias[li])
                w.fc1 = prep_linear([lyr.fc1.weight], [lyr.fc1.bias], dev)
                w.fc2 = prep_linear([lyr.fc2.weight], [lyr.fc2.bias], dev)
            W.layers.append(w)
        if _BIAS_COPIES:
            torch._foreach_copy_([d for d, _ in _BIAS_COPIES], [s_ for _, s_ in _BIAS_COPIES])
        _BIAS_COPIES = None
        W.scb = []
        if cfg.use_enrollments and cfg.scb_layers:
            for blk in enc.ca_enrolls:
                s = NS()
                with ops.cast_group():
                    s.att = prep_attention(blk.cae.cross_attn, dev, fuse_qkv=False)
                    s.f0 = prep_linear([blk.cae.ffn[0].weight], [blk.cae.ffn[0].bias], dev)
                    s.f3 = prep_linear([blk.cae.ffn[3].weight], [blk.cae.ffn[3].bias], dev)
                W.scb.append(s)
        W.full_init = prep_full_fddt(enc.initial_fddt, dev) if (cfg.use_fddt and cfg.use_pre_pos_fddt and fddt_is_full(enc.initial_fddt)) else None
        W.full = [prep_full_fddt(f, dev) if fddt_is_full(f) else None for f in (enc.fddts if cfg.use_fddt else [])]
        W.fold = None
        self.W = W
        return W

    def prepare_fold(self):
        W, enc = self.W, self.enc
        if W.fold is not None:
            return W.fold
        dev = enc.conv1.weight.device
        D, F_ = self.cfg.d_model, self.cfg.encoder_ffn_dim
        fold = []
        for lyr in enc.layers:
            f = NS()
            att, ln1, ln2 = lyr.self_attn, lyr.self_attn_layer_norm, lyr.final_layer_norm
            f.qkv_w, f.qkv_c, f.qkv_b = _e((3 * D, D), BF16, dev), _e((3 * D,), F32, dev), _e((3 * D,), F32, dev)
            for k, (lin, has_b) in enumerate(((att.q_proj, True), (att.k_proj, False), (att.v_proj, True))):
                sl = slice(k * D, (k + 1) * D)
                ops.lnfold_prep(lin.weight.detach(), ln1.weight.detach(), ln1.bias.detach(), lin.bias.detach() if has_b else None,
                                f.qkv_w[sl], f.qkv_c[sl], f.qkv_b[sl])
            f.fc1_w, f.fc1_c, f.fc1_b = _e((F_, D), BF16, dev), _e((F_,), F32, dev), _e((F_,), F32, dev)
            ops.lnfold_prep(lyr.fc1.weight.detach(), ln2.weight.detach(), ln2.bias.detach(), lyr.fc1.bias.detach(), f.fc1_w, f.fc1_c, f.fc1_b)
            f.eps1, f.eps2 = float(ln1.eps), float(ln2.eps)
            fold.append(f)
        W.fold = fold
        return fold

    def forward(self, input_features, stno_mask, enrollments=None, need_grad=True):
        cfg = self.cfg
        B, T = input_features.shape[0], cfg.max_source_positions
        if (SPLIT_FWD and not need_grad and enrollments is None and not cfg.use_enrollments and input_features.is_cuda and B % 2 == 0
                and B * T >= SPLIT_FWD_MIN_ROWS and input_features.dim() == 3 and input_features.shape[2] == 2 * T
                and _split_allowed()):
            dev, D = input_features.device, cfg.d_model
            enc_out, enc_bf = _e((B * T, D), F32, dev), _e((B * T, D), BF16, dev)
            stno_mask = stno_mask.to(device=dev)
            main_st, parts, _ = _fwd_parts(B, T, dev)
            S = None
            for st_, r, bsl in parts:
                with torch.cuda.stream(st_):
                    _, Sh = self._forward_impl(input_features[bsl], stno_mask[bsl], None, False, out=(enc_out[r], enc_bf[r]))
                    del Sh.layers
                S = S or Sh
            for st_, _, _ in parts[1:]:
                main_st.wait_stream(st_)
            S.B0, S.B_out, S.enc_bf, S.h_last = B, B, enc_bf, None
            return enc_out.view(B, T, D), S
        return self._forward_impl(input_features, stno_mask, enrollments, need_grad)

    def _forward_impl(self, input_features, stno_mask, enrollments=None, need_grad=True, out=None):
        enc, cfg, W = self.enc, self.cfg, self.W
        dev = input_features.device
        if enrollments is not None:
            input_features = torch.stack((input_features, enrollments["input_features"].to(dev)), dim=1).flatten(0, 1)
            stno_mask = torch.stack((stno_mask, enrollments["stno_mask"].to(dev)), dim=1).flatten(0, 1)
        B, M, Tin = input_features.shape
        T, D, H, F_ = cfg.max_source_positions, cfg.d_model, cfg.encoder_attention_heads, cfg.encoder_ffn_dim
        if Tin != 2 * T:
            raise ValueError(f"Whisper expects the mel input features to be of length {2 * T}, but found {Tin}. "
                             f"Make sure to pad the input mel features to {2 * T}.")
        stno = stno_mask.to(device=dev, dtype=F32).contiguous()
        S = NS(B0=B, T=T, stno=stno, layers=[], scb=[])
        x2, stem = conv_stem_fwd(enc, W, input_features, need_grad=need_grad)
        if need_grad:
            S.stem, S.x2 = stem, x2
        rows = B * T
        pos = enc.embed_positions.weight
        init_fddt = enc.initial_fddt if (cfg.use_fddt and cfg.use_pre_pos_fddt) else None
        mode, fw, fb = fddt_ptrs(init_fddt, cfg)
        h = _e((rows, D), F32, dev)
        if W.full_init is not None:
            hf0, S.x2b = full_fddt_fwd(W.full_init, x2, stno, 4 * T, rows, T, D)
            ops.fddt_ln_fwd(hf0, rows, D, mode=ops.MODE_NONE, T=T, pos=pos.detach(), h_out=h)
        else:
            ops.fddt_ln_fwd(x2, rows, D, mode=mode, stno=stno, T=T, w=fw, b=fb, pos=pos.detach(), h_out=h)
        bstride = 4 * T
        Bc = B
        fuse_next = (FUSE_NEXT_FDDT and not need_grad and cfg.use_fddt and not cfg.use_enrollments and all(f is None for f in W.full)
                     and ops.gemm_nt(h, W.layers[0].fc2.w, h, rows, D, F_, residual=h, bias=W.layers[0].fc2.b, query_persistent=True))
        rowmask = None
        if fuse_next:
            rowmask = torch.zeros(_ceil(rows, 192) + 64, 4, dtype=F32, device=dev)
            rowmask[:rows].view(B, T, 4).copy_(stno.permute(0, 2, 1))
        fold = None
        if (LN_FOLD and not need_grad and not cfg.use_enrollments and all(f is None for f in W.full) and D % 320 == 0 and D <= 1280
                and ops.gemm_nt(h, W.layers[0].fc2.w, h, rows, D, F_, residual=h, bias=W.layers[0].fc2.b, query_lnstat=True)
                and ops.gemm_nt(h, W.layers[0].att.o.w, h, rows, D, D, residual=h, bias=W.layers[0].att.o.b, query_lnstat=True)
                and ops.gemm_nt(h, W.layers[0].att.qkv.w, h, rows, 3 * D, D, query_persistent=True)):
            fold = self.prepare_fold()
            stat1 = torch.zeros(rows, L.LN_SLOTS, 2, dtype=F32, device=dev)
            stat2 = torch.zeros(rows, L.LN_SLOTS, 2, dtype=F32, device=dev)
        hb = None
        fddt_done = False
        split_ok = (SPLIT_FWD and need_grad and fold is None and not fuse_next and all(f is None for f in W.full)
                    and _split_allowed())
        split_from = cfg.scb_layers if (cfg.use_enrollments and cfg.scb_layers) else 0
        halves = None
        for i, lyr in enumerate(enc.layers):
            w = W.layers[i]
            Ls = NS(h_in=h, B=Bc, bstride=bstride)
            rows = Bc * T
            if split_ok and halves is None and i == split_from and Bc % 2 == 0 and rows >= SPLIT_FWD_MIN_ROWS:
                S.split_from = i
                main_st, halves, _ = _fwd_parts(Bc, T, dev)
            fd =enc.fddts[i] if (cfg.use_fddt and i < len(enc.fddts)) else None
            mode, fw, fb = fddt_ptrs(fd, cfg)
            use_scb = cfg.use_enrollments and cfg.scb_layers is not None and i < cfg.scb_layers
            wfull = W.full[i] if (fd is not None and i < len(W.full)) else None
            if need_grad and not use_scb and wfull is None:
                Ls.rows, Ls.B_after = rows, Bc
                hn = layer_fwd_buffers(Ls, Bc, T, H, F_, own_hp=mode != ops.MODE_NONE)
                for st_, r, bsl in halves or _one_part(Bc):
                    with _on(st_):
                        layer_rows_fwd(lyr, w, Ls, hn, r, bsl, bsl.stop - bsl.start, T, H, fddt=(mode, fw, fb, stno, bstride))
                h = hn
                S.layers.append(Ls)
                continue
            if fddt_done:
                mode, fw, fb = ops.MODE_NONE, (None,) * 4, (None,) * 4
            nfd = enc.fddts[i + 1] if (fuse_next and i + 1 < len(enc.layers) and i + 1 < len(enc.fddts)) else None
            nmode, nfw, nfb = fddt_ptrs(nfd, cfg)
            fuse_here = nfd is not None and nmode == ops.MODE_DIAG and all(t is not None for t in nfw) and all(t is not None for t in nfb)
            if wfull is not None:
                h, Ls.full_hb = full_fddt_fwd(wfull, h, stno, bstride, rows, T, D)
                Ls.h_in = h
                mode, fw, fb = ops.MODE_NONE, (None,) * 4, (None,) * 4
            xln = _e((rows, D), BF16, dev)
            mean, rstd = _e((rows,), F32, dev), _e((rows,), F32, dev)
            ln = lyr.self_attn_layer_norm
            fold1 = fold is not None and hb is not None and mode == ops.MODE_NONE
            if fold1:
                hp = h
            elif not use_scb:
                hp = _e((rows, D), F32, dev) if mode != ops.MODE_NONE else h
                ops.fddt_ln_fwd(h, rows, D, mode=mode, stno=stno, stno_bstride=bstride, T=T, w=fw, b=fb,
                                h_out=hp if mode != ops.MODE_NONE else None, ln_w=ln.weight.detach(),
                                ln_b=ln.bias.detach(), y_bf16=xln, mean=mean, rstd=rstd)
            else:
                hf = _e((rows, D), F32, dev) if mode != ops.MODE_NONE else h
# ... 764 lines not shown
```

### ts-asr-whisper_amd/modeling.py

```python
import math
import re
from collections import OrderedDict
from types import SimpleNamespace as NS_
from typing import Optional

import torch
from torch import nn

from . import _lib as L
from . import ops
from .config import DiCoWConfig, _HF

if _HF:
    from transformers import PreTrainedModel as _ModelBase, GenerationConfig as _GenerationConfig
else:
    _ModelBase, _GenerationConfig = nn.Module, None
from .engine import EncoderEngine, DecoderEngine, CtcEngine, GradSink, fddt_ptrs, CLS, prep_full_fddt, full_fddt_fwd, full_fddt_bwd

F32, BF16 = torch.float32, torch.bfloat16


class ModelOutput(OrderedDict):

    def __getattr__(self, k):
# ... 133 lines not shown
                           "(the CPU oracle under oracle/ is test infrastructure only)")


def _param_sig(params):
    return tuple((p.data_ptr(), p._version) for p in params)


class _FDDTFn(torch.autograd.Function):
    @staticmethod
    def forward(ctx, mod, hidden, stno, *params):
        _require_cuda(hidden, "FDDT")
        B, T, D = hidden.shape
        h = hidden.contiguous()
        if h.dtype not in (F32, BF16):
            h = h.to(F32)
        st = stno.to(device=h.device, dtype=F32).contiguous()
        mode, w, b = fddt_ptrs(mod, None)
        out = torch.empty(B, T, D, dtype=F32, device=h.device)
        ops.fddt_ln_fwd(h, B * T, D, mode=mode, stno=st, T=T, w=tuple(None if x is None else x.detach() for x in w),
                        b=tuple(None if x is None else x.detach() for x in b), h_out=out)
        ctx.mod, ctx.h, ctx.st, ctx.params = mod, h, st, params
        return out

    @staticmethod
    def backward(ctx, g):
        mod, h, st = ctx.mod, ctx.h, ctx.st
        B, T, D = h.shape
        G = GradSink(ctx.params, h.device)
        mode, w, b = fddt_ptrs(mod, None)
        gh = torch.empty(B, T, D, dtype=F32, device=h.device)
        ops.fddt_ln_bwd(h, B * T, D, mode=mode, stno=st, T=T, w=tuple(None if x is None else x.detach() for x in w),
                        b=tuple(None if x is None else x.detach() for x in b), g_res=g.contiguous().to(F32), g_out=gh,
                        dw=tuple(G.get(x) for x in w), db=tuple(G.get(x) for x in b))
        return (None, gh.to(ctx.h.dtype) if ctx.h.dtype != F32 else gh, None) + tuple(G.result(p) for p in ctx.params)


class FDDT(nn.Module):

    def __init__(self, d_model, non_target_rate=0.01, fddt_init=None, is_diagonal=False, bias_only=False, use_silence=True,
                 use_target=True, use_overlap=True, use_non_target=True):
        super().__init__()

        def make(val):
            if bias_only:
                return nn.Parameter(torch.zeros(d_model))
            if is_diagonal:
                return DiagonalLinear(d_model, bias=True, fddt_init=fddt_init, init_eye_val=val)
            return DenseLinear(d_model, d_model, bias=True, fddt_init=fddt_init, init_eye_val=val)

        if use_target:
            self.target_linear = make(1.0)
        if use_non_target:
            self.non_target_linear = make(non_target_rate)
        if use_overlap:
            self.overlap_linear = make(1.0)
        if use_silence:
            self.silence_linear = make(non_target_rate)
        self.use_silence, self.use_target, self.use_overlap, self.use_non_target = use_silence, use_target, use_overlap, use_non_target
        self.bias_only, self.is_diagonal, self.d_model = bias_only, is_diagonal or bias_only, d_model

    def forward(self, hidden_states, stno_mask):
        if not self.is_diagonal:
            return self._forward_full(hidden_states, stno_mask)
        params = [p for p in self.parameters()]
        return _FDDTFn.apply(self, hidden_states, stno_mask, *params)

    def _forward_full(self, hidden_states, stno_mask):
        params = [p for p in self.parameters()]
        return _FDDTFullFn.apply(self, hidden_states, stno_mask, *params)


class _FDDTFullFn(torch.autograd.Function):
    @staticmethod
    def forward(ctx, mod, hidden, stno, *params):
        _require_cuda(hidden, "FDDT")
        B, T, D = hidden.shape
        if D % 64 != 0:
            raise L.DicowError("full FDDT needs d_model % 64 == 0")
        dev = hidden.device
        h = hidden.contiguous().to(F32).view(B * T, D)
        st = stno.to(device=dev, dtype=F32).contiguous()
        w = prep_full_fddt(mod, dev)
        out, hb = full_fddt_fwd(w, h, st, 4 * T, B * T, T, D)
        ctx.mod, ctx.w, ctx.hb, ctx.st, ctx.params, ctx.shape = mod, w, hb, st, params, (B, T, D)
        return out.view(B, T, D)

    @staticmethod
    def backward(ctx, g):
        B, T, D = ctx.shape
        G = GradSink(ctx.params, g.device)
        gh = full_fddt_bwd(ctx.mod, ctx.w, ctx.hb, g.contiguous().to(F32).view(B * T, D), ctx.st, 4 * T, G, B * T, T, D)
        return (None, gh.view(B, T, D), None) + tuple(G.result(p) for p in ctx.params)


def _refuse_unsupported(where, **kw):
    bad = [k for k, v in kw.items() if v is not None]
    if bad:
        raise NotImplementedError(f"{where}: {', '.join(bad)} not supported by the HIP path (per-head masks, attention / "
                                  "hidden-state outputs, decoder masks / positions have no kernels here)")


class _EncoderFn(torch.autograd.Function):
    @staticmethod
    def forward(ctx, enc, input_features, stno, enrollments, need_grad, *params):
        eng = enc._engine()
        out, S = eng.forward(input_features, stno, enrollments, need_grad=need_grad)
        ctx.enc, ctx.S, ctx.params = enc, (S if need_grad else None), params
        return out

    @staticmethod
    def backward(ctx, d_enc):
        enc, S = ctx.enc, ctx.S
        G = GradSink(ctx.params, d_enc.device)
        D = enc.config.d_model
        enc._engine(prepare=False).backward(S, d_enc.contiguous().view(-1, D).to(F32), G)
        return (None, None, None, None, None) + tuple(G.result(p) for p in ctx.params)


class DiCoWEncoder(nn.Module):
    def __init__(self, config: DiCoWConfig):
        super().__init__()
        self.config = config
        d, f = config.d_model, config.encoder_ffn_dim
        self.conv1 = nn.Conv1d(config.num_mel_bins, d, kernel_size=3, padding=1)
        self.conv2 = nn.Conv1d(d, d, kernel_size=3, stride=2, padding=1)
        self.embed_positions = nn.Embedding(config.max_source_positions, d)
        self.embed_positions.requires_grad_(False)
        self.layers = nn.ModuleList([EncoderLayer(d, f) for _ in range(config.encoder_layers)])
        self.layer_norm = nn.LayerNorm(d)
        self.ctc_weight = config.ctc_weight
        if config.ctc_weight > 0.0:
            if config.additional_layer:
                self.additional_layer = EncoderLayer(d, f)
            if config.additional_self_attention_layer:
                self.additional_self_attention_layer = Attention(d)
            if config.pre_ctc_sub_sample:
                self.subsample_conv1 = nn.Conv1d(d, d, kernel_size=3, stride=2, padding=1, bias=False)
                self.subsample_conv2 = nn.Conv1d(d, d, kernel_size=3, stride=2, padding=1, bias=False)
            self.lm_head = nn.Linear(d, config.vocab_size + 1, bias=False)
        self.first_task_token = config.vocab_size - 30 * 50 - 1 - 6
        if config.use_fddt:
            def mk(rate):
                return FDDT(d_model=d, non_target_rate=rate, fddt_init=config.fddt_init, is_diagonal=config.fddt_is_diagonal,
                            bias_only=config.fddt_bias_only, use_silence=config.fddt_use_silence,
                            use_target=config.fddt_use_target, use_overlap=config.fddt_use_overlap,
                            use_non_target=config.fddt_use_non_target)
            self.fddts = nn.ModuleList([mk(1.0) for _ in range(config.num_fddts)])
            if config.use_pre_pos_fddt:
                self.initial_fddt = mk(config.non_target_fddt_value)
        if config.use_enrollments and config.scb_layers is not None:
            self.ca_enrolls = nn.ModuleList([SpeakerCommunicationBlock(config) for _ in range(config.scb_layers)])
        self._eng = None
        self._sig = None
        self._ctc_eng = None
        self._ctc_sig = None

    _CTC_PREFIXES = ("additional_layer.", "additional_self_attention_layer.", "subsample_conv", "lm_head.")
    main_input_name = "input_features"

    def get_loss(self, logits, labels):
        if int(labels.max()) >= self.config.vocab_size:
            raise ValueError(f"Label values must be <= vocab_size: {self.config.vocab_size}")
        lab = labels.to(logits.device)
        if self.config.remove_timestamps_from_ctc:
            keep = lab < self.first_task_token
            order = torch.argsort((~keep).to(torch.int8), dim=1, stable=True)
            lab = torch.gather(lab, 1, order)
            cnt = keep.sum(dim=1, keepdim=True)
            lab = torch.where(torch.arange(lab.shape[1], device=lab.device)[None, :] < cnt, lab, torch.full_like(lab, -100))
            lab = lab[:, :max(int(cnt.max()), 1)]
        valid = lab >= 0
        lab = torch.gather(lab, 1, torch.argsort((~valid).to(torch.int8), dim=1, stable=True)).contiguous()
        return _CtcLossFn.apply(self, logits, lab)

    def ctc_parameters(self):
        return [p for n, p in self.named_parameters() if n.startswith(self._CTC_PREFIXES)]

    def _ctc_engine(self, prepare=True):
        if self._ctc_eng is None:
            self._ctc_eng = CtcEngine(self)
        if prepare:
            sig = _param_sig(self.ctc_parameters())
            if sig != self._ctc_sig:
                self._ctc_eng.prepare()
                self._ctc_sig = sig
        return self._ctc_eng

    def _engine(self, prepare=True):
        if self._eng is None:
            self._eng = EncoderEngine(self)
        if prepare:
            ctc_ids = {id(p) for p in self.ctc_parameters()} if self.ctc_weight > 0.0 else set()
            sig = _param_sig([p for p in self.parameters() if id(p) not in ctc_ids])
            if sig != self._sig:
                self._eng.prepare()
                self._sig = sig
        return self._eng

    def get_max_len(self):
        return self.config.max_source_positions * 2

    def forward(self, input_features, attention_mask=None, head_mask=None, output_attentions=None, output_hidden_states=None,
                return_dict=None, stno_mask=None, return_logits=False, enrollments=None):
        _require_cuda(input_features, "DiCoWEncoder")
        if stno_mask is None:
            if self.config.use_fddt or enrollments is not None:
                raise ValueError("stno_mask is required")
            stno_mask = torch.zeros(input_features.shape[0], 4, self.config.max_source_positions, dtype=F32, device=input_features.device)
        _refuse_unsupported("DiCoWEncoder.forward", head_mask=head_mask, output_attentions=output_attentions or None,
                            output_hidden_states=output_hidden_states or None)
        ctc_ids = {id(p) for p in self.ctc_parameters()} if self.ctc_weight > 0.0 else set()
        params = [p for p in self.parameters() if id(p) not in ctc_ids]
        need_grad = torch.is_grad_enabled() and (input_features.requires_grad or any(p.requires_grad for p in params))
        out = _EncoderFn.apply(self, input_features, stno_mask, enrollments, need_grad, *params)
        if return_logits:
            if self.ctc_weight <= 0.0:
                raise L.DicowError("return_logits needs the CTC head (ctc_weight > 0)")
            logits = _CtcLogitsFn.apply(self, out, *self.ctc_parameters())
            return ModelOutput(loss=None, logits=logits, hidden_states=out)
        if return_dict is False:
            return (out,)
        return ModelOutput(last_hidden_state=out, hidden_states=None, attentions=None)

    def ctc_logits_into(self, input_features, stno_mask, out):
        if torch.is_grad_enabled():
            raise L.DicowError("ctc_logits_into keeps nothing for a backward pass: call it under torch.no_grad()")
        if self.ctc_weight <= 0.0:
            raise L.DicowError("ctc_logits_into needs the CTC head (ctc_weight > 0)")
        enc_out = self.forward(input_features, stno_mask=stno_mask).last_hidden_state
        enc_bf, enc_f, B, T = _ctc_head_input(enc_out)
        self._ctc_engine().encode_logits(enc_bf, B, T, enc_f, out=out)
        return out

    def ctc_logits_layout(self):
        if self.ctc_weight <= 0.0:
            raise L.DicowError("ctc_logits_layout needs the CTC head (ctc_weight > 0)")
        eng = self._ctc_engine()
        return eng.frames(self.config.max_source_positions), eng.W.cpad


def freeze_for_ctc_pretraining(encoder):
    head = {id(p) for p in encoder.ctc_parameters()}
    if not head:
        raise L.DicowError("freeze_for_ctc_pretraining: the encoder has no CTC head (ctc_weight > 0)")
    for p in encoder.parameters():
        p.requires_grad_(id(p) in head)
    return encoder


def _ctc_head_input(enc_out):
    B, T, D = enc_out.shape
    enc_f = enc_out.contiguous().to(F32).view(B * T, D)
    return ops.cast_bf16(enc_f).view(B * T, D), enc_f, B, T


class _CtcFn(torch.autograd.Function):

    @staticmethod
    def forward(ctx, enc, enc_out, ctc_labels, *params):
        eng = enc._ctc_engine()
        B, T, D = enc_out.shape
        enc_f = enc_out.contiguous().to(F32).view(B * T, D)
        enc_bf = ops.cast_bf16(enc_f).view(B * T, D)
        loss, S = eng.forward(enc_bf, B, T, ctc_labels, enc_f)
        ctx.enc, ctx.S, ctx.params = enc, S, params
        return loss

    @staticmethod
    def backward(ctx, g_loss):
        enc, S = ctx.enc, ctx.S
        G = GradSink(ctx.params, g_loss.device)
        d_enc = enc._ctc_engine(prepare=False).backward(S, g_loss, G)
        hook = getattr(enc, "_segment_hook", None)
        if hook is not None:
            hook("ctc")
        return (None, d_enc.view(S.B, S.T, -1), None) + tuple(G.result(p) for p in ctx.params)


class _CtcLogitsFn(torch.autograd.Function):

    @staticmethod
    def forward(ctx, enc, enc_out, *params):
        eng = enc._ctc_engine()
        enc_bf, enc_f, B, T = _ctc_head_input(enc_out)
        S = eng.encode_logits(enc_bf, B, T, enc_f)
        ctx.enc, ctx.S, ctx.params = enc, S, params
        return S.logits.view(B, S.Tn, -1)[:, :, :enc.config.vocab_size + 1]

    @staticmethod
    def backward(ctx, g):
        enc, S = ctx.enc, ctx.S
        eng = enc._ctc_engine(prepare=False)
        cpad, V1 = eng.W.cpad, enc.config.vocab_size + 1
        pad = getattr(enc, "_ctc_dlogits", None)
        if pad is not None and pad.shape == (S.B * S.Tn, cpad) and g.data_ptr() == pad.data_ptr() and g.stride() == (S.Tn * cpad, cpad, 1):
            d = pad
        else:
            d = torch.zeros(S.B * S.Tn, cpad, dtype=BF16, device=g.device)
            d.view(S.B, S.Tn, cpad)[:, :, :V1].copy_(g)
        enc._ctc_dlogits = None
        G = GradSink(ctx.params, g.device)
        d_enc = eng.backward_from_logits(S, d, G)
        hook = getattr(enc, "_segment_hook", None)
        if hook is not None:
            hook("ctc")
        return (None, d_enc.view(S.B, S.T, -1)) + tuple(G.result(p) for p in ctx.params)


class _CtcLossFn(torch.autograd.Function):

    @staticmethod
    def forward(ctx, enc, logits, labels):
        B, Tn, V1 = logits.shape
        dev = logits.device
        if logits.dtype == BF16 and logits.stride(2) == 1 and logits.stride(0) == Tn * logits.stride(1) and logits.stride(1) % 2 == 0:
            buf, ld = logits, logits.stride(1)
        else:
            ld = (V1 + 127) // 128 * 128
            buf = torch.zeros(B, Tn, ld, dtype=BF16, device=dev)
            buf[:, :, :V1].copy_(logits)
        lab = labels.contiguous()
        S = NS_(B=B, Tn=Tn, ld=ld, buf=buf)
        S.lse, S.nll, S.tlen = (torch.empty(n, dtype=F32, device=dev) for n in (B * Tn, B, B))
        S.ab = torch.empty(2, B, Tn, 2 * lab.shape[1] + 1, dtype=F32, device=dev)
        S.acc = torch.zeros(1, dtype=F32, device=dev)
        S.labels = lab
        S.ctc = ops.ctc_args(buf, ld, B, Tn, V1, lab, S.lse, S.ab[0], S.ab[1], S.nll, S.tlen, S.acc)
        ops.ctc_loss_fwd(S.ctc)
        ctx.enc, ctx.S, ctx.V1 = enc, S, V1
        return S.acc[0] / B

    @staticmethod
    def backward(ctx, g):
        enc, S = ctx.enc, ctx.S
        d = torch.empty(S.B * S.Tn, S.ld, dtype=BF16, device=g.device)
        S.ctc.d_logits = d.data_ptr()
        ops.ctc_loss_bwd(S.ctc, g.to(F32).reshape(1))
        enc._ctc_dlogits = d
        return None, d.view(S.B, S.Tn, S.ld)[:, :, :ctx.V1], None


def prepare_ctc_labels(labels, config, prefix_tokens, first_task_token):
    lab = labels.clone()
    for tok in prefix_tokens:
        if bool((lab[:, 0] == tok).all()):
            lab = lab[:, 1:]
    lab[lab == config.eos_token_id] = -100
    if config.remove_timestamps_from_ctc:
# ... 632 lines not shown
```

### ts-asr-whisper_amd/ops.py

```python
import ctypes as C
import os
from typing import Optional, Sequence

import torch

from . import _lib as L

BF16 = torch.bfloat16
F32 = torch.float32


def _req(t: torch.Tensor, dtype, name: str):
    if not t.is_cuda:
        raise L.DicowError(f"{name}: tensor must live on the GPU (no CPU fallback)")
    if t.dtype != dtype:
        raise L.DicowError(f"{name}: expected {dtype}, got {t.dtype}")
    return t


def _p(t):
    return None if t is None else t.data_ptr()


_WS = {}
# ... 409 lines not shown
def lora_wgrad(t, p, outs, r, scale, *, block=False, accumulate=True, g_rs=None, g_cs=1):
    _lora_2d(t, BF16, "lora_wgrad.t")
    _lora_2d(p, BF16, "lora_wgrad.p")
    a = L.LoraWgradArgs()
    a.T, a.P = t.data_ptr(), p.data_ptr()
    a.ldt, a.ldp = t.stride(0), p.stride(0)
    a.M, a.R, a.r, a.flags = t.shape[0], t.shape[1], int(r), L.LORA_BLOCK if block else 0
    nseg = max(a.R // max(a.r, 1), 1)
    assert p.shape[0] == a.M and len(outs) == nseg and nseg <= L.LORA_MAX_SEG, "lora_wgrad: shapes disagree"
    a.N = p.shape[1] // nseg if block else p.shape[1]
    assert not block or p.shape[1] == nseg * a.N
    a.g_rs, a.g_cs = (a.N if g_rs is None else g_rs), g_cs
    for j, g in enumerate(outs):
        if g is not None:
            _req(g, F32, "lora_wgrad.out")
            assert g.is_contiguous() and g.numel() == a.r * a.N, "lora_wgrad.out: need a contiguous r x N (or N x r) fp32 tensor"
            a.G[j] = g.data_ptr()
    a.scale, a.accumulate = float(scale), int(bool(accumulate))
    need = L.lib().dicow_lora_wgrad_ws_bytes(a.M, a.N, a.R, a.r, a.flags)
    ws = workspace(max(need, 1), t.device)
    a.ws, a.ws_bytes = ws.data_ptr(), ws.numel()
    L.call_struct("dicow_lora_wgrad", a)


_FWS = {}
ATTN_BWD_FUSED = os.environ.get("DICOW_ATTN_BWD_FUSED", "1") != "0"


def attn_bwd_fused_ws(B, H, Lq, Lk, device):
    n = L.lib().dicow_attn_bwd_fused_ws_bytes(B, H, Lq, Lk)
    key = (device.type, device.index, torch.cuda.current_stream(device).cuda_stream)
    t = _FWS.get(key)
    if t is None or t.numel() < n:
        t = torch.zeros(n + 4096, dtype=torch.uint8, device=device)
        _FWS[key] = t
    off = (-t.data_ptr()) % 4096
    return t[off:off + n]


def attn_bwd_fused_status(device=None) -> int:
    torch.cuda.synchronize(device)
    st = 0
    for (_, idx, _), t in _FWS.items():
        if device is None or idx == torch.device(device).index:
            off = (-t.data_ptr()) % 4096
            st |= L.lib().dicow_attn_bwd_fused_status(t.data_ptr() + off)
    return st


def attn_bwd(q, k, v, o, d_o, lse, delta, dq, dk, dv, causal=False, dq_scale=1.0, dq_colsum=None, dv_colsum=None, q_log2=False,
             fused=None):
    assert delta.numel() >= 2 * lse.numel(), "attn_bwd: delta workspace must hold 2*B*H*Lq floats"
    a = L.AttnBwdArgs()
    a.q, a.k, a.v, a.o, a.d_o = q.data_ptr(), k.data_ptr(), v.data_ptr(), o.data_ptr(), d_o.data_ptr()
    a.lse, a.delta = lse.data_ptr(), delta.data_ptr()
    a.dq, a.dk, a.dv = dq.data_ptr(), dk.data_ptr(), dv.data_ptr()
    a.q_bs, a.q_rs = _bs_rs(q, "q")
    a.k_bs, a.k_rs = _bs_rs(k, "k")
    a.v_bs, a.v_rs = _bs_rs(v, "v")
    a.o_bs, a.o_rs = _bs_rs(o, "o")
    a.do_bs, a.do_rs = _bs_rs(d_o, "d_o")
    a.dq_bs, a.dq_rs = _bs_rs(dq, "dq")
    a.dk_bs, a.dk_rs = _bs_rs(dk, "dk")
    a.dv_bs, a.dv_rs = _bs_rs(dv, "dv")
    a.B, a.Lq, a.H = q.shape[0], q.shape[1], q.shape[2]
    a.Lk, a.causal, a.dq_scale, a.q_log2 = k.shape[1], int(causal), dq_scale, int(q_log2)
    if dq_colsum is not None or dv_colsum is not None:
        ws = workspace(L.lib().dicow_attn_bwd_colsum_ws_bytes(a.B, a.H, a.Lq, a.Lk), q.device)
        a.dq_colsum, a.dv_colsum, a.cs_ws, a.cs_ws_bytes = _p(dq_colsum), _p(dv_colsum), ws.data_ptr(), ws.numel()
    want = ATTN_BWD_FUSED if fused is None else fused
    a.fused_mode = int(want == "force")
    if want and L.lib().dicow_attn_bwd_fused_eligible(a.B, a.H, a.Lq, a.Lk, a.causal, a.fused_mode):
        fws = attn_bwd_fused_ws(a.B, a.H, a.Lq, a.Lk, q.device)
        a.fused_ws, a.fused_ws_bytes = fws.data_ptr(), fws.numel()
    L.call_struct("dicow_attn_bwd", a)


def ce_args(logits, ld, rows, V, labels, upp_labels, soft, ts, lse, row_loss, choice, loss_sum, count, d_logits=None):
    _req(labels, torch.int64, "ce.labels")
    if upp_labels is not None:
        _req(upp_labels, torch.int64, "ce.upp_labels")
    a = L.CeArgs()
    a.logits, a.ld, a.rows, a.V = logits.data_ptr(), ld, rows, V
    a.labels, a.upp_labels, a.soft = labels.data_ptr(), _p(upp_labels), int(soft)
    if ts is not None:
        a.ts_index, a.ts_ids, a.ts_w, a.n_ts = ts["index"].data_ptr(), ts["ids"].data_ptr(), ts["w"].data_ptr(), ts["ids"].numel()
    a.lse, a.row_loss, a.choice = lse.data_ptr(), row_loss.data_ptr(), choice.data_ptr()
    a.loss_sum, a.count, a.d_logits = loss_sum.data_ptr(), count.data_ptr(), _p(d_logits)
    return a


def ce_loss_fwd(a):
    L.call_struct("dicow_ce_loss_fwd", a)


def ce_loss_bwd(a, grad_scale):
    L.check(L.lib().dicow_ce_loss_bwd(C.byref(a), grad_scale.data_ptr(), L.stream()), "dicow_ce_loss_bwd")


def embed_fwd(ids, tok, pos, out):
    B, Lq = ids.shape
    L.call("dicow_embed_fwd", ids.data_ptr(), tok.data_ptr(), pos.data_ptr(), out.data_ptr(), B, Lq, tok.shape[1], L.stream())


def embed_bwd(ids, g, d_tok, d_pos, D):
    B, Lq = ids.shape
    L.call("dicow_embed_bwd", ids.data_ptr(), g.data_ptr(), _p(d_tok), _p(d_pos), B, Lq, D, L.stream())


def gelu_bwd_bf16(g, pre, out):
    L.call("dicow_gelu_bwd_bf16", g.data_ptr(), pre.data_ptr(), out.data_ptr(), g.numel(), L.stream())


def conv2_col2im_gelu_bwd(dA2, pre1, d_pre1, B, T2, Cc):
    L.call("dicow_conv2_col2im_gelu_bwd", dA2.data_ptr(), _p(pre1), d_pre1.data_ptr(), B, T2, Cc, L.stream())


def ctc_args(logits, ld, B, Tn, Cc, labels, lse, alpha, beta, nll, tlen, loss_sum):
    _req(labels, torch.int64, "ctc.labels")
    a = L.CtcArgs()
    a.logits, a.ld, a.B, a.Tn, a.C = logits.data_ptr(), ld, B, Tn, Cc
    a.labels, a.Lc, a.blank = labels.data_ptr(), labels.shape[1], Cc - 1
    a.lse, a.alpha, a.beta, a.Smax = lse.data_ptr(), alpha.data_ptr(), beta.data_ptr(), 2 * labels.shape[1] + 1
    a.nll, a.tlen, a.loss_sum = nll.data_ptr(), tlen.data_ptr(), loss_sum.data_ptr()
    return a


def ctc_loss_fwd(a):
    L.call_struct("dicow_ctc_loss_fwd", a)


def ctc_loss_bwd(a, grad_scale):
    L.check(L.lib().dicow_ctc_loss_bwd(C.byref(a), grad_scale.data_ptr(), L.stream()), "dicow_ctc_loss_bwd")


def fabric_emulate(buf, gbps, workgroups=16, passes=2):
    L.call("dicow_fabric_emulate", buf.data_ptr(), buf.numel() * buf.element_size(), float(gbps), int(workgroups), int(passes), L.stream())


def sumsq(x, out):
    L.call("dicow_sumsq_f32", x.data_ptr(), x.numel(), out.data_ptr(), L.stream())


def adamw(p, g, m, v, lr, beta1, beta2, eps, wd, step, gnorm_sq=None, max_norm=0.0):
    L.call("dicow_adamw_f32", p.data_ptr(), g.data_ptr(), m.data_ptr(), v.data_ptr(), p.numel(), lr, beta1, beta2, eps, wd,
           step, _p(gnorm_sq), max_norm, L.stream())


def adamw_dev(p, g, m, v, hyper, beta1, beta2, eps, wd, gnorm_sq=None, max_norm=0.0):
    L.call("dicow_adamw_f32_dev", p.data_ptr(), g.data_ptr(), m.data_ptr(), v.data_ptr(), p.numel(), hyper.data_ptr(), beta1, beta2,
           eps, wd, _p(gnorm_sq), max_norm, L.stream())


def multi_adamw(tensors_ptr, chunks_ptr, n_chunks, classes, cls_base=0, clip_coef=None):
    L.check(L.lib().dicow_multi_adamw_f32(tensors_ptr, chunks_ptr, n_chunks, C.byref(classes), cls_base, _p(clip_coef), L.stream()),
            "dicow_multi_adamw_f32")


def multi_sumsq_ws_bytes(n_chunks) -> int:
    return int(L.lib().dicow_multi_sumsq_ws_bytes(n_chunks))


def multi_sumsq(tensors_ptr, chunks_ptr, n_chunks, ws, out, max_norm):
    _req(out, F32, "multi_sumsq: out")
    L.call("dicow_multi_sumsq_f32", tensors_ptr, chunks_ptr, n_chunks, ws.data_ptr(), ws.numel(), out.data_ptr(), float(max_norm),
           L.stream())


def multi_scale(tensors_ptr, chunks_ptr, n_chunks, coef):
    L.call("dicow_multi_scale_f32", tensors_ptr, chunks_ptr, n_chunks, coef.data_ptr(), L.stream())


def tensor_stats_ws_bytes(n_tensors, n_chunks, bins) -> int:
    return int(L.lib().dicow_tensor_stats_ws_bytes(n_tensors, n_chunks, bins))


def tensor_stats(tensors_ptr, chunks_ptr, n_tensors, n_chunks, first_chunk_ptr, which, bins, ws, out, hist, grid=0):
    if out is not None:
        _req(out, torch.uint8, "tensor_stats: out")
        if out.numel() < n_tensors * L.STATS_REC_BYTES:
            raise L.DicowError(f"tensor_stats: out holds {out.numel()} bytes, {n_tensors * L.STATS_REC_BYTES} needed")
    if hist is not None:
        _req(hist, torch.int64, "tensor_stats: hist")
        if hist.numel() < n_tensors * bins:
            raise L.DicowError(f"tensor_stats: hist holds {hist.numel()} counts, {n_tensors * bins} needed")
    L.call("dicow_tensor_stats_f32", tensors_ptr, chunks_ptr, n_tensors, n_chunks, first_chunk_ptr, int(which), int(bins),
           None if ws is None else ws.data_ptr(), 0 if ws is None else ws.numel(), _p(out), _p(hist), int(grid), L.stream())
```

### ts-asr-whisper_amd/trainer.py

```python
import collections
import logging
import math
import os
import time

import torch
import torch.distributed as dist

from . import ops
from . import tracing
from .engine import GradSink

F32 = torch.float32
log = logging.getLogger(__name__)


def freeze_by_keyword(model, frozen_keywords=("decoder",)):
    for n, p in model.named_parameters():
        p.requires_grad_("lora_" in n or not any(k in n for k in frozen_keywords))
    model.tie_weights()


def _backward_order(model):
    enc = model.model.encoder
    groups = []
    ctc_ids = set()
    if getattr(enc, "ctc_weight", 0.0) > 0.0:
        ctc = enc.ctc_parameters()
        ctc_ids = {id(p) for p in ctc}
        groups.append(("ctc", ctc))
    groups.append(("final_ln", list(enc.layer_norm.parameters())))
    nl = len(enc.layers)
    for i in range(nl - 1, -1, -1):
        ps = list(enc.layers[i].parameters())
        ps = [p for p in ps if p.dim() == 2] + [p for p in ps if p.dim() != 2]
        if hasattr(enc, "fddts") and i < len(enc.fddts):
            ps += list(enc.fddts[i].parameters())
        if hasattr(enc, "ca_enrolls") and i < len(enc.ca_enrolls):
            ps += list(enc.ca_enrolls[i].parameters())
        groups.append((f"layer{i}", ps))
    tail = []
    if hasattr(enc, "initial_fddt"):
        tail += list(enc.initial_fddt.parameters())
    tail += [enc.embed_positions.weight] + list(enc.conv2.parameters()) + list(enc.conv1.parameters())
    groups.append(("stem", tail))
    return groups


REFERENCE_PREHEAT_PREFIXES = ("model.encoder.additional_layer", "model.encoder.additional_self_attention_layer", "model.encoder.lm_head",
                              "model.encoder.subsample_conv1", "model.encoder.subsample_conv2", "model.encoder.fddts",
                              "model.encoder.initial_fddt", "model.encoder.ca_enrolls")


class FlatStore:

    def __init__(self, model, preheat_prefixes=None):
        preheat_prefixes = REFERENCE_PREHEAT_PREFIXES if preheat_prefixes is None else tuple(preheat_prefixes)
        names = {id(p): n for n, p in model.named_parameters()}
        dev = next(model.parameters()).device
        self.segments = []
        self.runs = []
        entries, off, seen = [], 0, set()
        grouped = _backward_order(model)
        enc_ids = {id(p) for _, ps in grouped for p in ps}
        rest = [p for p in model.parameters() if p.requires_grad and id(p) not in enc_ids]
        if rest:
            grouped = [("decoder", rest)] + grouped
        for gname, ps in grouped:
            start = off
            for p in ps:
                if not p.requires_grad or id(p) in seen:
                    continue
                seen.add(id(p))
                n = p.numel()
                pre = any(names[id(p)].startswith(pp) for pp in preheat_prefixes)
                entries.append((p, off, n, pre))
                off += (n + 63) // 64 * 64
            if off > start:
                self.segments.append((gname, start, off))
        self.numel = off
        self.params = torch.zeros(off, dtype=F32, device=dev)
        self.grads = torch.zeros(off, dtype=F32, device=dev)
        self.exp_avg = torch.zeros(off, dtype=F32, device=dev)
        self.exp_avg_sq = torch.zeros(off, dtype=F32, device=dev)
        self.entries = entries
        self._names = names
        for p, o, n, pre in entries:
            self.params[o:o + n].copy_(p.data.reshape(-1))
            p.data = self.params[o:o + n].view(p.shape)
            p.grad = self.grads[o:o + n].view(p.shape)
            p._direct_grad = p.grad
            pad_end = o + (n + 63) // 64 * 64
            if self.runs and self.runs[-1][2] == pre and self.runs[-1][1] == o:
                self.runs[-1] = (self.runs[-1][0], pad_end, pre)
            else:
                self.runs.append((o, pad_end, pre))
        self.n_trainable = sum(n for _, _, n, _ in entries)
        enc = model.model.encoder
        over = {id(p) for lyr in enc.layers for p in lyr.parameters() if p.dim() == 2}
        self._over = [(p, o, n) for p, o, n, _ in entries if id(p) in over]
        keep, cur = [], 0
        for p, o, n in sorted(self._over, key=lambda t: t[1]):
            if o > cur:
                keep.append((cur, o))
            cur = max(cur, o + n)
        if cur < self.numel:
            keep.append((cur, self.numel))
        self._zero_ranges = keep
        self._zero_views = None

    def fingerprint(self):
        return [(self._names[id(p)], int(o), int(n)) for p, o, n, _ in self.entries]

    def zero_grad(self, first_writer=False):
        if not first_writer or not self._over:
            self.grads.zero_()
            for p, _, _ in self._over:
                p._grad_overwrite = False
            return
        if self._zero_views is None:
            self._zero_views = [self.grads[a:b] for a, b in self._zero_ranges if b > a]
        if self._zero_views:
            torch._foreach_zero_(self._zero_views)
        for p, o, n in self._over:
            p._grad_overwrite = bool(p.requires_grad)
            if not p.requires_grad:
                self.grads[o:o + n].zero_()

    def settle_range(self, a, b):
        n_left = 0
        for p, o, n in self._over:
            if a <= o < b and getattr(p, "_grad_overwrite", False):
                self.grads[o:o + n].zero_()
                p._grad_overwrite = False
                n_left += 1
        return n_left

    def settle_first_writers(self):
        n_left = 0
        for p, o, n in self._over:
            if getattr(p, "_grad_overwrite", False):
                self.grads[o:o + n].zero_()
                p._grad_overwrite = False
                n_left += 1
        return n_left


class FusedAdamW:

    def __init__(self, store, lr=2e-6, fddt_lr_multiplier=100.0, betas=(0.9, 0.999), eps=1e-8, weight_decay=0.0,
                 max_grad_norm=1.0, warmup_steps=0, max_steps=0, schedule="cosine"):
        self.s, self.lr, self.mult, self.betas, self.eps, self.wd = store, lr, fddt_lr_multiplier, betas, eps, weight_decay
        self.max_norm, self.warmup, self.max_steps, self.schedule = max_grad_norm, warmup_steps, max_steps, schedule
        self.t = 0
        self.run_t = [0] * len(store.runs)
        self.gnorm_sq = torch.zeros(1, dtype=F32, device=store.params.device)
        dev = store.params.device
        self.counters = torch.zeros(1 + len(store.runs), dtype=torch.int32, device=dev)
        self.hyper = torch.zeros(len(store.runs), 3, dtype=F32, device=dev)
        self.is_pre = torch.tensor([int(pre) for _, _, pre in store.runs], dtype=torch.int32, device=dev)

    def sync_counters(self):
        self.counters.copy_(torch.tensor([self.t] + list(self.run_t), dtype=torch.int32))

    def lr_at(self, k):
        sched_step = k - 1
        if sched_step < self.warmup:
            return self.lr * sched_step / max(1, self.warmup)
        if self.schedule == "cosine" and self.max_steps > 0:
            prog = (sched_step - self.warmup) / max(1, self.max_steps - self.warmup)
            return self.lr * max(0.0, 0.5 * (1.0 + math.cos(math.pi * prog)))
        return self.lr

    def applied_lr(self):
        return self.hyper[:, 0].detach().cpu().tolist()

    def advance(self, preheat_only=False):
        self.t += 1
        for i, (a, b, pre) in enumerate(self.s.runs):
            if not (preheat_only and not pre):
                self.run_t[i] += 1

    def launch(self, preheat_only=False):
        s = self.s
        L_ = ops.L
        L_.call("dicow_adamw_hyper", self.counters.data_ptr(), self.hyper.data_ptr(), self.is_pre.data_ptr(), len(s.runs),
                int(preheat_only), float(self.lr), float(self.mult), int(self.warmup), int(self.max_steps),
                int(self.schedule == "cosine"), float(self.betas[0]), float(self.betas[1]), L_.stream())
        self.gnorm_sq.zero_()
        ops.sumsq(s.grads, self.gnorm_sq)
        for i, (a, b, pre) in enumerate(s.runs):
            if preheat_only and not pre:
                continue
            ops.adamw_dev(s.params[a:b], s.grads[a:b], s.exp_avg[a:b], s.exp_avg_sq[a:b], self.hyper[i], self.betas[0], self.betas[1],
                          self.eps, 0.0 if pre else self.wd, gnorm_sq=self.gnorm_sq, max_norm=self.max_norm)

    def step(self, preheat_only=False):
        self.advance(preheat_only)
        self.launch(preheat_only)


def _bit_checksum(t):
    flat = t.detach().reshape(-1)
    if flat.numel() == 0:
        return 0
    view = {1: torch.uint8, 2: torch.int16, 4: torch.int32, 8: torch.int64}[flat.element_size()]
    bits = flat.view(view)
    total, step = 0, 1 << 24
    for a in range(0, bits.numel(), step):
        c = bits[a:a + step].to(torch.int64)
        idx = torch.arange(a, a + c.numel(), device=c.device, dtype=torch.int64)
        total = (total + int((c * (2 * (idx % 1000003) + 1)).sum().item())) & 0xFFFFFFFFFFFFFFFF
    return total


_SYNC_COALESCE_BELOW = 64 << 20


def sync_replicas(model, store=None, process_group=None, mode="broadcast", src=0, extra=()):
    if mode not in ("broadcast", "verify", "none"):
        raise ValueError(f"replica_sync must be 'broadcast', 'verify' or 'none', not {mode!r}")
    if mode == "none" or not dist.is_initialized():
        return 0
    world = dist.get_world_size(process_group)
    in_store = set()
    tensors = []
    if store is not None:
        in_store = {id(p) for p, _, _, _ in store.entries}
        tensors.append(store.params)
    seen = set()
    rest = []
    for t in list(model.parameters()) + list(model.buffers()):
        if id(t) in in_store or id(t) in seen or t.data_ptr() in seen:
            continue
        seen.add(id(t))
        seen.add(t.data_ptr())
        rest.append(t.data)
    rest += [t for t in extra if t is not None]
    src_global = dist.get_global_rank(process_group, src) if process_group is not None else src
    if mode == "verify":
        mine = 0
        for t in tensors + rest:
            mine = (mine * 1000003 + _bit_checksum(t)) & 0x7FFFFFFFFFFFFFFF
        dev = tensors[0].device if tensors else (rest[0].device if rest else torch.device("cpu"))
        got = [torch.zeros(1, dtype=torch.int64, device=dev) for _ in range(world)]
        dist.all_gather(got, torch.tensor([mine], dtype=torch.int64, device=dev), group=process_group)
        sums = [int(g.item()) for g in got]
        if len(set(sums)) != 1:
            bad = [r for r, v in enumerate(sums) if v != sums[src]]
            raise RuntimeError(f"data-parallel replicas differ at start-up: ranks {bad} do not hold rank {src}'s parameters / buffers "
                               f"(checksums {[hex(v) for v in sums]}); construct TrainStep with replica_sync='broadcast' or load the "
                               f"same checkpoint on every rank")
        log.info("replica check: %d ranks hold identical state (checksum %s)", world, hex(sums[0]))
        return 8 * world
    nbytes = 0
    if world > 1 or os.environ.get("DICOW_FORCE_REDUCE") == "1":
        for t in tensors:
            dist.broadcast(t, src=src_global, group=process_group)
            nbytes += t.numel() * t.element_size()
        by_dtype = collections.OrderedDict()
        for t in rest:
            if t.numel() * t.element_size() >= _SYNC_COALESCE_BELOW and t.is_contiguous():
                dist.broadcast(t, src=src_global, group=process_group)
                nbytes += t.numel() * t.element_size()
            else:
                by_dtype.setdefault((t.dtype, t.device), []).append(t)
        for (dt, dev), ts in by_dtype.items():
            flat = torch.cat([t.reshape(-1) for t in ts]) if len(ts) > 1 else ts[0].reshape(-1).clone()
            dist.broadcast(flat, src=src_global, group=process_group)
            off = 0
            for t in ts:
                t.copy_(flat[off:off + t.numel()].view(t.shape))
                off += t.numel()
            nbytes += flat.numel() * flat.element_size()
        log.info("replica sync: rank %d's state broadcast to %d ranks (%d bytes: %d in the flat store)", src, world, nbytes,
                 sum(t.numel() * t.element_size() for t in tensors))
    return nbytes


def nccl_pg_options():
    try:
        opts = dist.ProcessGroupNCCL.Options()
        opts.is_high_priority_stream = True
        return opts
    except Exception:
        return None


class GradReducer:

    def __init__(self, store, process_group=None):
        self.s = store
        self.pg = process_group
        self.world = dist.get_world_size(process_group) if dist.is_initialized() else 1
        self.force = os.environ.get("DICOW_FORCE_REDUCE") == "1" and dist.is_initialized()
        self.stream = None
        if (self.world > 1 or self.force) and torch.cuda.is_available():
            self.stream = torch.cuda.Stream(priority=-1 if os.environ.get("DICOW_REDUCER_STREAM_PRIORITY", "high") == "high" else 0)
        if self.stream is not None and self.world > 1:
            from . import ops
            reserve = int(os.environ.get("DICOW_RCCL_CUS", "16"))
            ncu = torch.cuda.get_device_properties(torch.cuda.current_device()).multi_processor_count
            ops.set_gemm_cus(max(ncu - reserve, ncu // 2))
        self._avg_in_collective = bool(dist.is_initialized() and dist.get_backend(process_group) == "nccl")
        self.seg = {name: (a, b) for name, a, b in store.segments}
        self.pending = []
        self.time_exposed = False
        self._exposed = []
        self.time_buckets = False
        self._bucket_ev = []
        self._bucket_cpu = []
        g = os.environ.get("DICOW_EMULATE_FABRIC_GBPS")
        self.emulate_gbps = float(g) if g else 0.0
        self.emulate_workgroups = int(os.environ.get("DICOW_EMULATE_FABRIC_WGS", "16"))
        self.preheat_only = False
        self.hold = False

    def segment_ready(self, name):
        if (self.world == 1 and not self.force) or name not in self.seg or self.preheat_only or self.hold:
            return
        a, b = self.seg[name]
        self.s.settle_range(a, b)
        if self.stream is None:
            buf = self.s.grads[a:b]
            t0 = time.perf_counter()
            dist.all_reduce(buf, group=self.pg)
            buf.div_(self.world)
            if self.time_buckets:
                self._bucket_cpu.append((name, time.perf_counter() - t0))
            return
        ev = torch.cuda.Event(enable_timing=self.time_buckets)
        ev.record()
        with torch.cuda.stream(self.stream):
            self.stream.wait_event(ev)
            if self.time_buckets:
                e_start = torch.cuda.Event(enable_timing=True)
                e_start.record()
            buf = self.s.grads[a:b]
            if self._avg_in_collective:
                dist.all_reduce(buf, op=dist.ReduceOp.AVG, group=self.pg)
            else:
                dist.all_reduce(buf, group=self.pg)
                buf.div_(self.world)
            if self.emulate_gbps > 0.0 and buf.is_cuda:
                n = (b - a) // 4 * 4
                if n > 0:
                    ops.fabric_emulate(buf[:n], self.emulate_gbps, self.emulate_workgroups)
            if self.time_buckets:
                e_end = torch.cuda.Event(enable_timing=True)
                e_end.record()
                self._bucket_ev.append((name, ev, e_start, e_end))

    def _reduce_preheat_runs(self):
        runs = [(a, b) for a, b, pre in self.s.runs if pre]
        if not runs:
            return
        flat = torch.cat([self.s.grads[a:b] for a, b in runs])
        dist.all_reduce(flat, group=self.pg)
        flat.div_(self.world)
        off = 0
        for a, b in runs:
            self.s.grads[a:b].copy_(flat[off:off + b - a])
            off += b - a

    def finish(self):
        if self.preheat_only and (self.world > 1 or self.force):
            self._reduce_preheat_runs()
        if self.stream is not None:
            if self.time_exposed:
                e0, e1 = torch.cuda.Event(enable_timing=True), torch.cuda.Event(enable_timing=True)
                e0.record()
                torch.cuda.current_stream().wait_stream(self.stream)
                e1.record()
                self._exposed.append((e0, e1))
            else:
                torch.cuda.current_stream().wait_stream(self.stream)

    def bucket_report(self, steps=1):
        rows = []
        if self._bucket_ev:
            torch.cuda.synchronize()
            rows = [(n, r.elapsed_time(s_), s_.elapsed_time(e)) for n, r, s_, e in self._bucket_ev]
        elif self._bucket_cpu:
            rows = [(n, 0.0, dt * 1e3) for n, dt in self._bucket_cpu]
        self._bucket_ev, self._bucket_cpu = [], []
        if not rows:
            return None
        steps = max(1, steps)
        per = {}
        for n, lag, dur in rows:
            t = per.setdefault(n, [0, 0.0, 0.0])
            t[0] += 1; t[1] += lag; t[2] += dur
        worst = sorted(per.items(), key=lambda kv: -kv[1][1] / kv[1][0])[:3]
        return {"buckets_per_step": len(rows) // steps,
                "start_lag_ms": {"mean": round(sum(r[1] for r in rows) / len(rows), 4), "max": round(max(r[1] for r in rows), 4),
                                 "sum_per_step": round(sum(r[1] for r in rows) / steps, 3)},
                "busy_ms_per_step": round(sum(r[2] for r in rows) / steps, 3),
                "longest_queued": [{"bucket": n, "lag_ms": round(v[1] / v[0], 4), "collective_ms": round(v[2] / v[0], 4)} for n, v in worst]}

    def exposed_ms(self):
        if not self._exposed:
            return 0.0
        torch.cuda.synchronize()
        ms = sum(a.elapsed_time(b) for a, b in self._exposed) / len(self._exposed)
        self._exposed = []
        return ms


_SPLIT_GROUP = int(os.environ.get("DICOW_SPLIT_GROUP", "2"))


class SplitSync:

    def __init__(self, group=_SPLIT_GROUP):
        self.role, self.ev, self.group, self.free_until = None, {}, max(1, int(group)), None

    def reset(self):
        self.role, self.ev, self.free_until = None, {}, None

    def _gate(self, name):
        if not name.startswith("layer") or self.group == 1:
            return name
        i = int(name[5:])
        return f"layer{i - i % self.group}"

    def enter(self, name):
        if self.role == "follow":
            gate = self._gate(name)
            if gate == self.free_until:
                return
            ev = self.ev.get(gate)
            if ev is None:
                raise RuntimeError(f"SplitSync: the leader half never finished segment {gate!r} -- the two halves' backward passes differ")
            torch.cuda.current_stream().wait_event(ev)
            self.free_until = gate

    def done(self, name):
        if self.role == "lead" and self._gate(name) == name:
            ev = torch.cuda.Event()
            ev.record()
            self.ev[name] = ev


class TrainStep:

    def __init__(self, model, lr=2e-6, fddt_lr_multiplier=100.0, weight_decay=0.0, max_grad_norm=1.0, warmup_steps=0,
                 max_steps=0, frozen_keywords=("decoder",), preheat_prefixes=None,
                 process_group=None, augmenter=None, use_fddt_only_n_steps=0, graph=False, use_fddt_only_n_epochs=0,
                 steps_per_epoch=None, replica_sync="broadcast", split_streams=False, front_end=None, watch=None):
        self.model = model
        self.watch = watch
        self.split_streams = bool(split_streams)
        self._split_sync = SplitSync()
        self._split_side = None
        if use_fddt_only_n_epochs:
            if not steps_per_epoch:
                raise ValueError("use_fddt_only_n_epochs needs steps_per_epoch (optimizer steps in one pass over the training set)")
            use_fddt_only_n_steps = max(int(use_fddt_only_n_steps), int(use_fddt_only_n_epochs) * int(steps_per_epoch))
        self.first_writer = True
        self.graph = bool(graph)
        self._graphs = collections.OrderedDict()
        self.max_graphs = 8
        self._graph_pool = None
        self._eager_done = set()
        self.augmenter = augmenter
        self.front_end = front_end
        freeze_by_keyword(model, frozen_keywords)
        self.store = FlatStore(model, preheat_prefixes)
        self.opt = FusedAdamW(self.store, lr, fddt_lr_multiplier, weight_decay=weight_decay, max_grad_norm=max_grad_norm,
                              warmup_steps=warmup_steps, max_steps=max_steps)
        self.reducer = GradReducer(self.store, process_group)
        self.replica_sync = replica_sync
        self.replica_sync_bytes = sync_replicas(model, self.store, process_group, mode=replica_sync)
        if self.replica_sync_bytes and replica_sync == "broadcast":
            model.model.encoder._sig = None
            model.model.encoder._ctc_sig = None
            model._sig = None
        model.model.encoder._segment_hook = self.reducer.segment_ready
        model._segment_hook = self.reducer.segment_ready
        self.use_fddt_only_n_steps = use_fddt_only_n_steps
        self.warmup_phase = use_fddt_only_n_steps > 0
        names = {id(p): n for n, p in model.named_parameters()}
        self._preheat_is_vectors_only = all(p.dim() == 1 and "fddt" in names[id(p)] for p, _, _, pre in self.store.entries if pre)
        if self.warmup_phase:
            self._set_phase(preheat_only=True)

    def _set_phase(self, preheat_only):
        for p, _, _, pre in self.store.entries:
            p.requires_grad_(pre or not preheat_only)
        self.reducer.preheat_only = preheat_only
        self.model.model.encoder._sig = None
        self.model._sig = None

    def _invalidate_decoder_copies(self):
        base = lora = False
        for n, p in self.model.model.decoder.named_parameters():
            if p.requires_grad:
                if "lora_" in n:
                    lora = True
                else:
                    base = True
                    break
        if base:
            self.model._sig = None
        elif lora:
            self.model._lora_sig = None

    @property
    def global_step(self):
        return self.opt.t

    def begin_step(self):
        if self.warmup_phase and self.global_step >= self.use_fddt_only_n_steps:
            self._set_phase(preheat_only=False)
            self.warmup_phase = False
        self.store.zero_grad(first_writer=self.first_writer and not self.warmup_phase)

    def finish_step(self):
        with tracing.range("exchange"):
            self.reducer.finish()
        if self.first_writer and not self.warmup_phase:
            self.store.settle_first_writers()
        with tracing.range("optimizer"):
            self.opt.step(preheat_only=self.warmup_phase)
        enc = self.model.model.encoder
        if not (self.warmup_phase and self._preheat_is_vectors_only):
            enc._sig = None
            enc._ctc_sig = None
        self._invalidate_decoder_copies()

    def _micro(self, batch, scale):
        if self.split_streams and self._can_split(batch):
            return self._micro_split(batch, scale)
        if self.front_end is not None and "input_waves" in batch:
            batch = self.front_end(dict(batch))
        if self.augmenter is not None:
            batch = self.augmenter(dict(batch))
        with tracing.range("forward"):
            out = self.model(**batch)
        with tracing.range("backward"):
            (out.loss if scale == 1.0 else out.loss * scale).backward()
        return out.loss.detach()

    def _can_split(self, batch):
        cfg = self.model.config
        lab = batch.get("labels")
        return (self.split_streams and self.augmenter is None and self.front_end is None and cfg.ctc_weight == 0.0 and batch.get("enrollments") is None and
                lab is not None and lab.is_cuda and lab.shape[0] >= 2 and lab.shape[0] % 2 == 0 and
                all(not torch.is_tensor(v) or v.dim() == 0 or v.shape[0] == lab.shape[0] for v in batch.values()))

    def _micro_split(self, batch, scale):
        model, enc, sync = self.model, self.model.model.encoder, self._split_sync
        cur = torch.cuda.current_stream()
        if self._split_side is None:
            self._split_side = (torch.cuda.Stream(priority=-1), torch.cuda.Stream(priority=-1))
        s_f, s_l = self._split_side
        hb = batch["labels"].shape[0] // 2
        halves = [{k: (v[i * hb:(i + 1) * hb] if torch.is_tensor(v) and v.dim() > 0 else v) for k, v in batch.items()} for i in (0, 1)]
        if getattr(model, "_ts_tables", None) is not None:
            cnt = torch.stack([(h["labels"] != -100).sum() for h in halves]).to(torch.float32)
            wts = cnt / cnt.sum().clamp_min(1.0) * scale
        else:
            wts = torch.full((2,), 0.5 * scale, dtype=torch.float32, device=batch["labels"].device)
        enc._engine()
        model._engine()
        sync.reset()
        enc._split_sync = model._split_sync = sync
        try:
            with tracing.range("forward"):
                outs = [None, None]
                for i, st in ((1, s_l), (0, s_f)):
                    st.wait_stream(cur)
                    with torch.cuda.stream(st):
                        outs[i] = model(**halves[i])
            with tracing.range("backward"):
                hold = self.reducer.hold
                self.reducer.hold = True
                sync.role = "lead"
                with torch.cuda.stream(s_l):
                    (outs[1].loss * wts[1]).backward()
                self.reducer.hold = hold
                sync.role = "follow"
                with torch.cuda.stream(s_f):
                    (outs[0].loss * wts[0]).backward()
        finally:
            sync.role = None
            enc._split_sync = model._split_sync = None
        cur.wait_stream(s_l)
        cur.wait_stream(s_f)
        for o in outs:
            o.loss.record_stream(cur)
        return (outs[0].loss.detach() * wts[0] + outs[1].loss.detach() * wts[1]) / scale

    @staticmethod
    def _sig_of(batch):
        out = []
        for k in sorted(batch):
            v = batch[k]
            out.append((k, TrainStep._sig_of(v)) if isinstance(v, dict) else (k, tuple(v.shape), str(v.dtype)))
        return tuple(out)

    @staticmethod
    def _clone(batch):
        return {k: (TrainStep._clone(v) if isinstance(v, dict) else v.clone()) for k, v in batch.items()}

    @staticmethod
    def _copy_into(dst, src):
        for k, v in src.items():
            if isinstance(v, dict):
                TrainStep._copy_into(dst[k], v)
            else:
                dst[k].copy_(v, non_blocking=True)

    def _invalidate_weight_copies(self):
        enc = self.model.model.encoder
        enc._sig = None
        enc._ctc_sig = None
        self._invalidate_decoder_copies()

    def _graph_step(self, batch):
        if self.reducer.world > 1 or self.reducer.force:
            raise NotImplementedError("TrainStep(graph=True) captures the single-GPU step; the bucketed side-stream exchange is not captured")
        if self.model.config.ctc_weight > 0.0 or self.augmenter is not None or self.front_end is not None:
            raise NotImplementedError("TrainStep(graph=True): the CTC label preparation / the augmentation planner read device data on "
                                      "the host; their steps cannot be captured")
        if self.warmup_phase and self.global_step >= self.use_fddt_only_n_steps:
            self._set_phase(preheat_only=False)
            self.warmup_phase = False
        key = (self.warmup_phase, self._sig_of(batch))
        if key not in self._eager_done:
            self._eager_done.add(key)
            return self._eager_step([batch])
        if key not in self._graphs:
            while len(self._graphs) >= max(1, self.max_graphs):
                self._graphs.popitem(last=False)
            if self._graph_pool is None:
                self._graph_pool = torch.cuda.graph_pool_handle()
            static = self._clone(batch)
            self._invalidate_weight_copies()
            torch.cuda.synchronize()
            g = torch.cuda.CUDAGraph()
            with torch.cuda.graph(g, pool=self._graph_pool):
                self.store.zero_grad(first_writer=self.first_writer and not self.warmup_phase)
                out = self.model(**static)
                out.loss.backward()
                self.opt.launch(preheat_only=self.warmup_phase)
                loss = out.loss.detach()
            self._graphs[key] = (g, static, loss)
        self._graphs.move_to_end(key)
        g, static, loss = self._graphs[key]
        self._copy_into(static, batch)
        self.opt.advance(preheat_only=self.warmup_phase)
        g.replay()
        self._invalidate_weight_copies()
        return loss.clone()

    def step(self, batch, eager=False):
        micro = list(batch) if isinstance(batch, (list, tuple)) else [batch]
        if self.graph and not eager and len(micro) == 1:
            loss = self._graph_step(micro[0])
        else:
            loss = self._eager_step(micro)
        if self.watch is not None and self.watch.due(self.global_step):
            self.watch.collect(self.global_step)
        return loss

    def _eager_step(self, micro):
        self.begin_step()
        loss = None
        for i, b in enumerate(micro):
            self.reducer.hold = i + 1 < len(micro)
            l = self._micro(b, 1.0 / len(micro))
            loss = l if loss is None else loss + l
        self.finish_step()
        return loss / len(micro)

    def logged_loss(self, loss):
        r = self.reducer
        if r.world == 1:
            return loss
        t = loss.detach().clone().float().reshape(1)
        dist.all_reduce(t, op=dist.ReduceOp.SUM, group=r.pg)
        return (t / r.world)[0]

    def state_dict(self):
        o = self.opt
        return {"global_step": o.t, "run_t": list(o.run_t), "warmup_phase": self.warmup_phase,
                "exp_avg": self.store.exp_avg.clone(), "exp_avg_sq": self.store.exp_avg_sq.clone(),
                "layout": [(a, b, pre) for a, b, pre in self.store.runs], "entries": self.store.fingerprint()}

    def resync(self):
        if self.replica_sync == "none" or self.reducer.world <= 1:
            return 0
        n = sync_replicas(self.model, self.store, self.reducer.pg, mode=self.replica_sync)
        self.model.model.encoder._sig = None
        self.model.model.encoder._ctc_sig = None
        self.model._sig = None
        return n

    def _sync_host_counters_phase(self, phase):
        keep = self.warmup_phase
        self.warmup_phase = phase
        try:
            return self._sync_host_counters()
        finally:
            self.warmup_phase = keep

    def _sync_host_counters(self):
        if self.replica_sync == "none" or self.reducer.world <= 1 or not dist.is_initialized():
            return
        dev = self.store.params.device
        mine = torch.tensor([int(self.opt.t), int(bool(self.warmup_phase))] + [int(x) for x in self.opt.run_t], dtype=torch.int64, device=dev)
        if self.replica_sync == "verify":
            got = [torch.zeros_like(mine) for _ in range(self.reducer.world)]
            dist.all_gather(got, mine, group=self.reducer.pg)
            bad = [r for r, g in enumerate(got) if not torch.equal(g, got[0])]
            if bad:
                raise RuntimeError(f"data-parallel replicas resumed with different step counters: ranks {bad} differ from rank 0 "
                                   f"(global_step / warmup_phase / per-run steps {[g.tolist()[:3] for g in got]})")
            return
        src = dist.get_global_rank(self.reducer.pg, 0) if self.reducer.pg is not None else 0
        dist.broadcast(mine, src=src, group=self.reducer.pg)
        vals = mine.tolist()
        self.opt.t, self.opt.run_t = int(vals[0]), [int(x) for x in vals[2:]]
        self.opt.sync_counters()
        return bool(vals[1])

    def load_state_dict(self, sd, allow_legacy_layout=False, sync_model=True):
        if [tuple(r) for r in sd["layout"]] != [tuple(r) for r in self.store.runs]:
            raise ValueError("optimizer state was saved for a different set of trainable parameters")
        if "entries" not in sd:
            if not allow_legacy_layout:
                raise ValueError("optimizer state has no per-parameter layout fingerprint (saved by an older version): the order of the "
                                 "parameters inside the flat buffers cannot be checked; pass allow_legacy_layout=True if it was saved by "
                                 "a version with today's parameter order (weight matrices before vectors inside a layer), or re-save it")
            log.warning("optimizer state without a layout fingerprint accepted on request: only the run boundaries were checked")
        elif [tuple(e) for e in sd["entries"]] != self.store.fingerprint():
            mine = {e[0]: e for e in self.store.fingerprint()}
            diff = [e[0] for e in sd["entries"] if tuple(e) != mine.get(e[0])][:4]
            raise ValueError(f"optimizer state was saved under a different flat-buffer layout (first differing parameters: {diff})")
        self.opt.t, self.opt.run_t = int(sd["global_step"]), list(sd["run_t"])
        self.opt.sync_counters()
        self.store.exp_avg.copy_(sd["exp_avg"])
        self.store.exp_avg_sq.copy_(sd["exp_avg_sq"])
        phase = bool(sd["warmup_phase"])
        if self.replica_sync != "none" and self.reducer.world > 1:
            if sync_model or self.replica_sync == "verify":
                if self.replica_sync == "broadcast":
                    try:
                        sync_replicas(self.model, self.store, self.reducer.pg, mode="verify")
                    except RuntimeError as ex:
                        log.warning("load_state_dict: the ranks' model weights differ before the resume broadcast -- rank 0's replace the others' (%s)", ex)
                sync_replicas(self.model, self.store, self.reducer.pg, mode=self.replica_sync,
                              extra=(self.store.exp_avg, self.store.exp_avg_sq, self.opt.counters))
            else:
                sync_replicas(torch.nn.Module(), None, self.reducer.pg, mode=self.replica_sync,
                              extra=(self.store.exp_avg, self.store.exp_avg_sq, self.opt.counters))
            p0 = self._sync_host_counters_phase(phase)
            phase = p0 if p0 is not None else phase
            self.model.model.encoder._sig = None
            self.model.model.encoder._ctc_sig = None
            self.model._sig = None
        sd = dict(sd, warmup_phase=phase)
        if bool(sd["warmup_phase"]) != self.warmup_phase:
            self._set_phase(preheat_only=bool(sd["warmup_phase"]))
            self.warmup_phase = bool(sd["warmup_phase"])
```

Baseline: 125.7 utt/s.

## Fuse AdamW update with bf16 weight and transposed-copy refresh via piece table

Result: slower. 121.6 utt/s (-3.3%).

```diff
diff --git a/include/dicow_hip.h b/include/dicow_hip.h
--- a/include/dicow_hip.h
+++ b/include/dicow_hip.h
@@ -389,6 +389,16 @@
                       int warmup_steps, int max_steps, int cosine, double beta1, double beta2, void* stream);
 int dicow_adamw_f32_dev(float* p, const float* g, float* m, float* v, int64_t n, const float* hyper, float beta1, float beta2,
                         float eps, float weight_decay, const float* gnorm_sq, float max_norm, void* stream);
+typedef struct {
+    int64_t start, len;
+    int32_t run, pre, R, C;
+    void* dst; int64_t ld; const void* dst_lo; int64_t dst_bytes;
+    void* dst_t; int64_t ld_t; const void* dst_t_lo; int64_t dst_t_bytes;
+} dicow_adamw_entry;
+int64_t dicow_adamw_table_ws_bytes(int n);
+int dicow_adamw_table(float* p, const float* g, float* m, float* v, int64_t numel, const dicow_adamw_entry* table, int n,
+                      const float* hyper, int n_runs, int preheat_only, float beta1, float beta2, float eps, float weight_decay,
+                      const float* gnorm_sq, float max_norm, int upload, void* ws, int64_t ws_bytes, void* stream);
 
 #define DICOW_MT_CHUNK 2048
 #define DICOW_MT_MAX_CLASSES 32
diff --git a/ts-asr-whisper_amd/_lib.py b/ts-asr-whisper_amd/_lib.py
--- a/ts-asr-whisper_amd/_lib.py
+++ b/ts-asr-whisper_amd/_lib.py
@@ -48,6 +48,12 @@
 
 class CastProblem(C.Structure):
     _fields_ = [("src", c_vp), ("dst", c_vp), ("dst_t", c_vp), ("R", c_i), ("C", c_i), ("ld", c_i64), ("ld_t", c_i64)]
+
+
+class AdamwEntry(C.Structure):
+    _fields_ = [("start", c_i64), ("len", c_i64), ("run", c_i), ("pre", c_i), ("R", c_i), ("C", c_i),
+                ("dst", c_vp), ("ld", c_i64), ("dst_lo", c_vp), ("dst_bytes", c_i64),
+                ("dst_t", c_vp), ("ld_t", c_i64), ("dst_t_lo", c_vp), ("dst_t_bytes", c_i64)]
 
 
 class GemmTnGroupArgs(C.Structure):
@@ -230,6 +236,8 @@
     "dicow_adamw_f32": [c_vp, c_vp, c_vp, c_vp, c_i64, c_f, c_f, c_f, c_f, c_f, c_i, c_vp, c_f, c_vp],
     "dicow_adamw_hyper": [c_vp, c_vp, c_vp, c_i, c_i, c_d, c_d, c_i, c_i, c_i, c_d, c_d, c_vp],
     "dicow_adamw_f32_dev": [c_vp, c_vp, c_vp, c_vp, c_i64, c_vp, c_f, c_f, c_f, c_f, c_vp, c_f, c_vp],
+    "dicow_adamw_table": [c_vp, c_vp, c_vp, c_vp, c_i64, C.POINTER(AdamwEntry), c_i, c_vp, c_i, c_i, c_f, c_f, c_f, c_f, c_vp, c_f, c_i, c_vp,
+                          c_i64, c_vp],
     "dicow_multi_chunk_elems": [],
     "dicow_multi_adamw_f32": [c_vp, c_vp, c_i64, C.POINTER(MtAdamwClasses), c_i, c_vp, c_vp],
     "dicow_multi_sumsq_f32": [c_vp, c_vp, c_i64, c_vp, c_i64, c_vp, c_f, c_vp],
@@ -298,6 +306,7 @@
     "dicow_logmel_ws_bytes": [c_i, c_i],
     "dicow_scb_gate_bwd_ws_bytes": [],
     "dicow_ctc_ws_bytes": [c_i, c_i, c_i],
+    "dicow_adamw_table_ws_bytes": [c_i],
     "dicow_multi_sumsq_ws_bytes": [c_i64],
     "dicow_tensor_stats_ws_bytes": [c_i64, c_i64, c_i],
     "dicow_lora_wgrad_ws_bytes": [c_i, c_i, c_i, c_i, c_i],
diff --git a/ts-asr-whisper_amd/csrc/elementwise.hip b/ts-asr-whisper_amd/csrc/elementwise.hip
--- a/ts-asr-whisper_amd/csrc/elementwise.hip
+++ b/ts-asr-whisper_amd/csrc/elementwise.hip
@@ -1,5 +1,6 @@
 #include <stdarg.h>
 #include <new>
+#include <vector>
 #include "host_table.h"
 
 static thread_local char g_err[512] = "";
@@ -669,6 +670,212 @@
     hipLaunchKernelGGL(adamw_kernel, dim3(grid), dim3(256), 0, (hipStream_t)stream, p, g, m, v, n, 0.f, beta1, beta2, eps,
                        weight_decay, 1.f, 1.f, gnorm_sq, max_norm, hyper);
     DICOW_CHECK_LAUNCH("adamw_f32_dev");
+    return DICOW_OK;
+}
+
+#define ADAMW_CHUNK 4096
+#ifndef ADAMW_TABLE_WGS_PER_CU
+#define ADAMW_TABLE_WGS_PER_CU 4
+#endif
+struct adamw_piece_t {
+    int64_t start, len;
+    unsigned short* dst; unsigned short* dst_t;
+    int64_t ld, ld_t;
+    int R, C, run, pre;
+};
+struct adamw_table_kargs_t {
+    float* p; const float* g; float* m; float* v;
+    const adamw_piece_t* piece; const int* item0; int n, items;
+    const float* hyper; const float* gnorm_sq;
+    float b1, b2, eps, wd, max_norm; int preheat_only;
+};
+
+__device__ __forceinline__ void adamw_update4(float4& pp, const float4& gg, float4& mm, float4& vv, float clip, float lr, float b1,
+                                              float b2, float eps, float wd, float bc1, float bc2) {
+#pragma clang fp contract(off)
+    float* pa = &pp.x; const float* ga = &gg.x; float* ma = &mm.x; float* va = &vv.x;
+    const float decay = __builtin_fmaf(-wd, lr, 1.f), c1 = 1.f - b1, c2 = 1.f - b2, step = lr / bc1, rbc2 = sqrtf(bc2);
+#pragma unroll
+    for (int e = 0; e < 4; ++e) {
+        const float gr = ga[e] * clip;
+        ma[e] = __builtin_fmaf(c1, gr, b1 * ma[e]);
+        va[e] = __builtin_fmaf(gr, c2 * gr, b2 * va[e]);
+        const float denom = sqrtf(va[e]) / rbc2 + eps;
+        const float x = step * (ma[e] / denom);
+        pa[e] = __builtin_fmaf(decay, pa[e], -x);
+    }
+}
+
+template <bool GUARD>
+__device__ __forceinline__ void adamw_tile(const adamw_table_kargs_t& a, const adamw_piece_t& q, int r0, int c0, unsigned short (*tile)[68],
+                                           float clip, float lr, float wd, float bc1, float bc2) {
+    const int R = q.R, C = q.C;
+    const int tq = threadIdx.x & 15, tr = threadIdx.x >> 4;
+#pragma unroll 1
+    for (int h = 0; h < 4; h += 2) {
+        float4 pp[2], gg[2], mm[2], vv[2];
+        bool in[2];
+#pragma unroll
+        for (int k = 0; k < 2; ++k) {
+            const int r = r0 + (h + k) * 16 + tr, c = c0 + tq * 4;
+            in[k] = !GUARD || (r < R && c < C);
+            if (in[k]) {
+                const int64_t o = q.start + (int64_t)r * C + c;
+                pp[k] = *reinterpret_cast<const float4*>(a.p + o); gg[k] = *reinterpret_cast<const float4*>(a.g + o);
+                mm[k] = *reinterpret_cast<const float4*>(a.m + o); vv[k] = *reinterpret_cast<const float4*>(a.v + o);
+            }
+        }
+#pragma unroll
+        for (int k = 0; k < 2; ++k) {
+            const int i = (h + k) * 16 + tr, r = r0 + i, c = c0 + tq * 4;
+            uint2 u = make_uint2(0, 0);
+            if (in[k]) {
+                adamw_update4(pp[k], gg[k], mm[k], vv[k], clip, lr, a.b1, a.b2, a.eps, wd, bc1, bc2);
+                const int64_t o = q.start + (int64_t)r * C + c;
+                *reinterpret_cast<float4*>(a.p + o) = pp[k]; *reinterpret_cast<float4*>(a.m + o) = mm[k];
+                *reinterpret_cast<float4*>(a.v + o) = vv[k];
+                u = make_uint2(pack_bf16x2(pp[k].x, pp[k].y), pack_bf16x2(pp[k].z, pp[k].w));
+                if (q.dst) *reinterpret_cast<uint2*>(q.dst + (int64_t)r * q.ld + c) = u;
+            }
+            if (q.dst_t) *reinterpret_cast<uint2*>(&tile[i][tq * 4]) = u;
+        }
+    }
+    if (!q.dst_t) return;
+    __syncthreads();
+#pragma unroll
+    for (int k = 0; k < 4; ++k) {
+        const int i = k * 16 + tr, c = c0 + i, r = r0 + tq * 4;
+        if (!GUARD || (c < C && r < R)) {
+            const unsigned lo = (unsigned)tile[tq * 4][i] | ((unsigned)tile[tq * 4 + 1][i] << 16);
+            const unsigned hi = (unsigned)tile[tq * 4 + 2][i] | ((unsigned)tile[tq * 4 + 3][i] << 16);
+            *reinterpret_cast<uint2*>(q.dst_t + (int64_t)c * q.ld_t + r) = make_uint2(lo, hi);
+        }
+    }
+    __syncthreads();
+}
+
+__global__ void __launch_bounds__(256) __attribute__((amdgpu_waves_per_eu(4))) adamw_table_kernel(const adamw_table_kargs_t a) {
+    __shared__ unsigned short tile[64][68];
+    float clip = 1.f;
+    if (a.gnorm_sq && a.max_norm > 0.f) {
+        const float c = a.max_norm / (sqrtf(a.gnorm_sq[0]) + 1e-6f);
+        clip = c < 1.f ? c : 1.f;
+    }
+    for (int item = blockIdx.x; item < a.items; item += gridDim.x) {
+        int lo = 0, hi = a.n;
+        while (hi - lo > 1) {
+            const int mid = (lo + hi) >> 1;
+            if (a.item0[mid] <= item) lo = mid; else hi = mid;
+        }
+        const adamw_piece_t q = a.piece[lo];
+        if (a.preheat_only && !q.pre) continue;
+        const float lr = a.hyper[3 * q.run], bc1 = a.hyper[3 * q.run + 1], bc2 = a.hyper[3 * q.run + 2];
+        const float wd = q.pre ? 0.f : a.wd;
+        const int lb = item - a.item0[lo];
+        if (q.R == 0) {
+            const int64_t e0 = q.start + (int64_t)lb * ADAMW_CHUNK;
+            const int64_t left = q.start + q.len - e0;
+            const int n4 = (int)((left < ADAMW_CHUNK ? left : ADAMW_CHUNK) >> 2);
+#pragma unroll 1
+            for (int h = 0; h < 4; h += 2) {
+                float4 pp[2], gg[2], mm[2], vv[2];
+#pragma unroll
+                for (int k = 0; k < 2; ++k) {
+                    const int j = (h + k) * 256 + threadIdx.x;
+                    if (j < n4) {
+                        pp[k] = reinterpret_cast<const float4*>(a.p + e0)[j]; gg[k] = reinterpret_cast<const float4*>(a.g + e0)[j];
+                        mm[k] = reinterpret_cast<const float4*>(a.m + e0)[j]; vv[k] = reinterpret_cast<const float4*>(a.v + e0)[j];
+                    }
+                }
+#pragma unroll
+                for (int k = 0; k < 2; ++k) {
+                    const int j = (h + k) * 256 + threadIdx.x;
+                    if (j < n4) {
+                        adamw_update4(pp[k], gg[k], mm[k], vv[k], clip, lr, a.b1, a.b2, a.eps, wd, bc1, bc2);
+                        reinterpret_cast<float4*>(a.p + e0)[j] = pp[k]; reinterpret_cast<float4*>(a.m + e0)[j] = mm[k];
+                        reinterpret_cast<float4*>(a.v + e0)[j] = vv[k];
+                    }
+                }
+            }
+            continue;
+        }
+        const int ntc = (q.C + 63) / 64;
+        const int r0 = (lb / ntc) * 64, c0 = (lb % ntc) * 64;
+        if (r0 + 64 <= q.R && c0 + 64 <= q.C) adamw_tile<false>(a, q, r0, c0, tile, clip, lr, wd, bc1, bc2);
+        else adamw_tile<true>(a, q, r0, c0, tile, clip, lr, wd, bc1, bc2);
+    }
+}
+
+static int64_t adamw_piece_items(const dicow_adamw_entry& e) {
+    return e.R ? (int64_t)dicow_cdiv(e.R, 64) * dicow_cdiv(e.C, 64) : (e.len + ADAMW_CHUNK - 1) / ADAMW_CHUNK;
+}
+
+extern "C" int64_t dicow_adamw_table_ws_bytes(int n) {
+    if (n < 1) { dicow_set_error("adamw_table_ws_bytes: n=%d pieces", n); return -1; }
+    return ((int64_t)n * (int64_t)sizeof(adamw_piece_t) + ((int64_t)n + 1) * 4 + 15) / 16 * 16;
+}
+
+static bool adamw_image_ok(const void* at, int64_t ld, int rows, int cols, const void* lo, int64_t bytes) {
+    if (!lo || bytes < 0 || ld < cols || (const char*)at < (const char*)lo) return false;
+    const int64_t off = (const char*)at - (const char*)lo, need = (((int64_t)rows - 1) * ld + cols) * 2;
+    return dicow_span_ok(off, need, bytes);
+}
+
+extern "C" int dicow_adamw_table(float* p, const float* g, float* m, float* v, int64_t numel, const dicow_adamw_entry* table, int n,
+                                 const float* hyper, int n_runs, int preheat_only, float beta1, float beta2, float eps, float weight_decay,
+                                 const float* gnorm_sq, float max_norm, int upload, void* ws, int64_t ws_bytes, void* stream) {
+    static thread_local std::vector<char> stage;
+    DICOW_REQUIRE(p && g && m && v && numel > 0 && table && n >= 1 && hyper && n_runs >= 1 && ws, "adamw_table: bad args");
+    DICOW_REQUIRE(dicow_aligned(16, p, g, m, v, ws), "adamw_table: p / g / m / v / ws not 16-byte aligned");
+    const int64_t need = dicow_adamw_table_ws_bytes(n);
+    DICOW_REQUIRE(ws_bytes >= need, "adamw_table: ws_bytes=%lld, need %lld", (long long)ws_bytes, (long long)need);
+    stage.assign((size_t)need, 0);
+    adamw_piece_t* piece = reinterpret_cast<adamw_piece_t*>(stage.data());
+    int* item0 = reinterpret_cast<int*>(stage.data() + (size_t)n * sizeof(adamw_piece_t));
+    int64_t items = 0, end = 0;
+    for (int i = 0; i < n; ++i) {
+        const dicow_adamw_entry& e = table[i];
+        DICOW_REQUIRE(e.len > 0 && e.start % 4 == 0 && e.len % 4 == 0, "adamw_table: piece %d: start=%lld len=%lld (multiples of 4, len > 0)", i,
+                      (long long)e.start, (long long)e.len);
+        DICOW_REQUIRE_SPAN(e.start, e.len, numel, "covers", "elements of the store", "adamw_table: piece %d", i);
+        DICOW_REQUIRE(e.start >= end, "adamw_table: piece %d starts at %lld, inside or before the piece ahead of it (ends at %lld)", i,
+                      (long long)e.start, (long long)end);
+        DICOW_REQUIRE(e.run >= 0 && e.run < n_runs, "adamw_table: piece %d: run %d of %d", i, e.run, n_runs);
+        if (e.R || e.C) {
+            DICOW_REQUIRE(e.R > 0 && e.C > 0 && e.R % 4 == 0 && e.C % 4 == 0 && (int64_t)e.R * e.C == e.len,
+                          "adamw_table: piece %d: matrix [%d, %d] over %lld elements (R, C multiples of 4, len = R C)", i, e.R, e.C, (long long)e.len);
+            DICOW_REQUIRE(dicow_aligned(8, e.dst, e.dst_t) && (!e.dst || e.ld % 4 == 0) && (!e.dst_t || e.ld_t % 4 == 0),
+                          "adamw_table: piece %d: dst / dst_t not 8-byte aligned or ld=%lld / ld_t=%lld no multiple of 4", i, (long long)e.ld, (long long)e.ld_t);
+            DICOW_REQUIRE(!e.dst || adamw_image_ok(e.dst, e.ld, e.R, e.C, e.dst_lo, e.dst_bytes),
+                          "adamw_table: piece %d: the [%d, %d] image (ld %lld) leaves its buffer of %lld bytes", i, e.R, e.C, (long long)e.ld, (long long)e.dst_bytes);
+            DICOW_REQUIRE(!e.dst_t || adamw_image_ok(e.dst_t, e.ld_t, e.C, e.R, e.dst_t_lo, e.dst_t_bytes),
+                          "adamw_table: piece %d: the transposed [%d, %d] image (ld_t %lld) leaves its buffer of %lld bytes", i, e.C, e.R, (long long)e.ld_t,
+                          (long long)e.dst_t_bytes);
+        }
+        end = e.start + e.len;
+        adamw_piece_t& q = piece[i];
+        q.start = e.start; q.len = e.len; q.R = e.R; q.C = e.C; q.run = e.run; q.pre = e.pre != 0;
+        q.dst = e.R ? (unsigned short*)e.dst : nullptr; q.dst_t = e.R ? (unsigned short*)e.dst_t : nullptr;
+        q.ld = e.ld; q.ld_t = e.ld_t;
+        item0[i] = (int)items;
+        items += adamw_piece_items(e);
+        DICOW_REQUIRE(items < (1LL << 30), "adamw_table: more than 2^30 work items");
+    }
+    item0[n] = (int)items;
+    hipStream_t st = (hipStream_t)stream;
+    if (upload)
+        if (int rc = dicow_upload("adamw_table", ws, stage.data(), need, st)) return rc;
+    static const int ncu = [] { hipDeviceProp_t pr; int d = 0; (void)hipGetDevice(&d); return hipGetDeviceProperties(&pr, d) == hipSuccess ? pr.multiProcessorCount : 256; }();
+    adamw_table_kargs_t a;
+    a.p = p; a.g = g; a.m = m; a.v = v;
+    a.piece = reinterpret_cast<const adamw_piece_t*>(ws);
+    a.item0 = reinterpret_cast<const int*>(static_cast<const char*>(ws) + (size_t)n * sizeof(adamw_piece_t));
+    a.n = n; a.items = (int)items;
+    a.hyper = hyper; a.gnorm_sq = gnorm_sq;
+    a.b1 = beta1; a.b2 = beta2; a.eps = eps; a.wd = weight_decay; a.max_norm = max_norm; a.preheat_only = preheat_only;
+    const int64_t grid = items < (int64_t)ADAMW_TABLE_WGS_PER_CU * ncu ? items : (int64_t)ADAMW_TABLE_WGS_PER_CU * ncu;
+    hipLaunchKernelGGL(adamw_table_kernel, dim3((unsigned)grid), dim3(256), 0, st, a);
+    DICOW_CHECK_LAUNCH("adamw_table");
     return DICOW_OK;
 }
 
diff --git a/ts-asr-whisper_amd/engine.py b/ts-asr-whisper_amd/engine.py
--- a/ts-asr-whisper_amd/engine.py
+++ b/ts-asr-whisper_amd/engine.py
@@ -106,19 +106,23 @@
 _BIAS_COPIES = None
 
 
-def prep_linear(weights, biases, dev, need_t=True, n_pad=None, scale_info=None, bias_buf=None):
+def prep_linear(weights, biases, dev, need_t=True, n_pad=None, scale_info=None, bias_buf=None, bufs=None, fresh=None):
     K = weights[0].shape[1]
     Ns = [w.shape[0] for w in weights]
     N = sum(Ns)
     Np = N if n_pad is None else n_pad
     lw = LinW()
     lw.N, lw.K = Np, K
-    lw.w = torch.zeros(Np, K, dtype=BF16, device=dev) if Np != N else _e((Np, K), BF16, dev)
-    lw.wt = (torch.zeros(K, Np, dtype=BF16, device=dev) if Np != N else _e((K, Np), BF16, dev)) if need_t else None
+    if bufs is not None:
+        lw.w, lw.wt = bufs
+    else:
+        lw.w = torch.zeros(Np, K, dtype=BF16, device=dev) if Np != N else _e((Np, K), BF16, dev)
+        lw.wt = (torch.zeros(K, Np, dtype=BF16, device=dev) if Np != N else _e((K, Np), BF16, dev)) if need_t else None
     off = 0
     for w, n in zip(weights, Ns):
-        ops.cast_transpose_bf16(w.detach(), out=lw.w[off:off + n], out_t=None if lw.wt is None else lw.wt[:, off:off + n],
-                                ld=K, ld_t=Np)
+        if fresh is None or id(w) not in fresh:
+            ops.cast_transpose_bf16(w.detach(), out=lw.w[off:off + n], out_t=None if lw.wt is None else lw.wt[:, off:off + n],
+                                    ld=K, ld_t=Np)
         off += n
     if biases is None or all(b is None for b in biases):
         lw.b = None
@@ -136,15 +140,15 @@
     return lw
 
 
-def prep_attention(att, dev, fuse_qkv=True, bias_buf=None):
+def prep_attention(att, dev, fuse_qkv=True, bias_buf=None, bufs=None, fresh=None):
     a = NS()
     if fuse_qkv:
         a.qkv = prep_linear([att.q_proj.weight, att.k_proj.weight, att.v_proj.weight],
-                            [att.q_proj.bias, None, att.v_proj.bias], dev, bias_buf=bias_buf)
+                            [att.q_proj.bias, None, att.v_proj.bias], dev, bias_buf=bias_buf, bufs=bufs and bufs["qkv"], fresh=fresh)
     else:
         a.q = prep_linear([att.q_proj.weight], [att.q_proj.bias], dev)
         a.kv = prep_linear([att.k_proj.weight, att.v_proj.weight], [None, att.v_proj.bias], dev)
-    a.o = prep_linear([att.out_proj.weight], [att.out_proj.bias], dev)
+    a.o = prep_linear([att.out_proj.weight], [att.out_proj.bias], dev, bufs=bufs and bufs["o"], fresh=fresh)
     return a
 
 
@@ -477,7 +481,34 @@
         self.enc = enc
         self.cfg = enc.config
 
-    def prepare(self):
+    def layer_buffers(self):
+        enc, cfg = self.enc, self.cfg
+        dev = enc.conv1.weight.device
+        if getattr(self, "_layer_bufs", None) is None or self._layer_bufs_dev != dev:
+            D, F_ = cfg.d_model, cfg.encoder_ffn_dim
+            pair = lambda n, k: (_e((n, k), BF16, dev), _e((k, n), BF16, dev))
+            self._layer_bufs = [{"qkv": pair(3 * D, D), "o": pair(D, D), "fc1": pair(F_, D), "fc2": pair(D, F_)} for _ in enc.layers]
+            self._layer_bufs_dev = dev
+            self._layer_copies = None
+        return self._layer_bufs
+
+    def layer_copies(self):
+        bufs = self.layer_buffers()
+        if self._layer_copies is None:
+            out = []
+            for lyr, b in zip(self.enc.layers, bufs):
+                att = lyr.self_attn
+                D = att.q_proj.weight.shape[0]
+                w, wt = b["qkv"]
+                for k, lin in enumerate((att.q_proj, att.k_proj, att.v_proj)):
+                    out.append((lin.weight, w[k * D:(k + 1) * D], w.shape[1], wt[:, k * D:(k + 1) * D], wt.shape[1]))
+                for lin, key in ((att.out_proj, "o"), (lyr.fc1, "fc1"), (lyr.fc2, "fc2")):
+                    w, wt = b[key]
+                    out.append((lin.weight, w, w.shape[1], wt, wt.shape[1]))
+            self._layer_copies = out
+        return self._layer_copies
+
+    def prepare(self, fresh=None):
         enc, cfg = self.enc, self.cfg
         dev = enc.conv1.weight.device
         D, M = cfg.d_model, cfg.num_mel_bins
@@ -490,12 +521,13 @@
         if getattr(self, "_qkv_bias", None) is None or self._qkv_bias[0].device != dev:
             self._qkv_bias = [torch.zeros(3 * D, dtype=F32, device=dev) for _ in enc.layers]
         _BIAS_COPIES = []
+        bufs = self.layer_buffers()
         for li, lyr in enumerate(enc.layers):
             w = NS()
             with ops.cast_group():
-                w.att = prep_attention(lyr.self_attn, dev, bias_buf=self._qkv_bias[li])
-                w.fc1 = prep_linear([lyr.fc1.weight], [lyr.fc1.bias], dev)
-                w.fc2 = prep_linear([lyr.fc2.weight], [lyr.fc2.bias], dev)
+                w.att = prep_attention(lyr.self_attn, dev, bias_buf=self._qkv_bias[li], bufs=bufs[li], fresh=fresh)
+                w.fc1 = prep_linear([lyr.fc1.weight], [lyr.fc1.bias], dev, bufs=bufs[li]["fc1"], fresh=fresh)
+                w.fc2 = prep_linear([lyr.fc2.weight], [lyr.fc2.bias], dev, bufs=bufs[li]["fc2"], fresh=fresh)
             W.layers.append(w)
         if _BIAS_COPIES:
             torch._foreach_copy_([d for d, _ in _BIAS_COPIES], [s_ for _, s_ in _BIAS_COPIES])
diff --git a/ts-asr-whisper_amd/modeling.py b/ts-asr-whisper_amd/modeling.py
--- a/ts-asr-whisper_amd/modeling.py
+++ b/ts-asr-whisper_amd/modeling.py
@@ -309,6 +309,7 @@
             self.ca_enrolls = nn.ModuleList([SpeakerCommunicationBlock(config) for _ in range(config.scb_layers)])
         self._eng = None
         self._sig = None
+        self._fresh = None
         self._ctc_eng = None
         self._ctc_sig = None
 
@@ -343,14 +344,18 @@
                 self._ctc_sig = sig
         return self._ctc_eng
 
+    def _engine_sig(self):
+        ctc_ids = {id(p) for p in self.ctc_parameters()} if self.ctc_weight > 0.0 else set()
+        return _param_sig([p for p in self.parameters() if id(p) not in ctc_ids])
+
     def _engine(self, prepare=True):
         if self._eng is None:
             self._eng = EncoderEngine(self)
         if prepare:
-            ctc_ids = {id(p) for p in self.ctc_parameters()} if self.ctc_weight > 0.0 else set()
-            sig = _param_sig([p for p in self.parameters() if id(p) not in ctc_ids])
+            sig = self._engine_sig()
             if sig != self._sig:
-                self._eng.prepare()
+                token, self._fresh = self._fresh, None
+                self._eng.prepare(fresh=token[1] if token is not None and token[0] == sig else None)
                 self._sig = sig
         return self._eng
 
diff --git a/ts-asr-whisper_amd/ops.py b/ts-asr-whisper_amd/ops.py
--- a/ts-asr-whisper_amd/ops.py
+++ b/ts-asr-whisper_amd/ops.py
@@ -585,6 +585,45 @@
            eps, wd, _p(gnorm_sq), max_norm, L.stream())
 
 
+def adamw_matrix_ok(R, Cc, start, dst, ld, dst_t, ld_t) -> bool:
+    return (R > 0 and Cc > 0 and R % 4 == 0 and Cc % 4 == 0 and start % 4 == 0 and (dst is not None or dst_t is not None)
+            and (dst is None or (ld % 4 == 0 and dst.data_ptr() % 8 == 0)) and (dst_t is None or (ld_t % 4 == 0 and dst_t.data_ptr() % 8 == 0)))
+
+
+class AdamwTable:
+
+    def __init__(self, pieces, device):
+        self.n = len(pieces)
+        self.arr = (L.AdamwEntry * max(self.n, 1))()
+        self.keep = []
+        for e, pc in zip(self.arr, pieces):
+            e.start, e.len, e.run, e.pre = int(pc[0]), int(pc[1]), int(pc[2]), int(bool(pc[3]))
+            if len(pc) > 4:
+                e.R, e.C = int(pc[4]), int(pc[5])
+                for t, ld, f in ((pc[6], pc[7], "dst"), (pc[8], pc[9], "dst_t")):
+                    if t is None:
+                        continue
+                    _req(t, BF16, f"AdamwTable.{f}")
+                    st = t.untyped_storage()
+                    setattr(e, f, t.data_ptr())
+                    setattr(e, "ld" if f == "dst" else "ld_t", int(ld))
+                    setattr(e, f + "_lo", st.data_ptr())
+                    setattr(e, f + "_bytes", st.nbytes())
+                    self.keep.append(t)
+        with torch.cuda.device(device):
+            self.ws, self.nbytes = table_workspace("adamw_table", L.lib().dicow_adamw_table_ws_bytes, self.n, device=device, pooled=False)
+        self.uploaded = False
+
+
+def adamw_table(tab: AdamwTable, p, g, m, v, hyper, beta1, beta2, eps, wd, gnorm_sq=None, max_norm=0.0, preheat_only=False):
+    capturing = torch.cuda.is_current_stream_capturing()
+    L.call("dicow_adamw_table", p.data_ptr(), g.data_ptr(), m.data_ptr(), v.data_ptr(), p.numel(), tab.arr, tab.n, hyper.data_ptr(),
+           hyper.shape[0], int(preheat_only), beta1, beta2, eps, wd, _p(gnorm_sq), max_norm, int(capturing or not tab.uploaded),
+           tab.ws.data_ptr(), tab.nbytes, L.stream())
+    if not capturing:
+        tab.uploaded = True
+
+
 def multi_adamw(tensors_ptr, chunks_ptr, n_chunks, classes, cls_base=0, clip_coef=None):
     L.check(L.lib().dicow_multi_adamw_f32(tensors_ptr, chunks_ptr, n_chunks, C.byref(classes), cls_base, _p(clip_coef), L.stream()),
             "dicow_multi_adamw_f32")
diff --git a/ts-asr-whisper_amd/trainer.py b/ts-asr-whisper_amd/trainer.py
--- a/ts-asr-whisper_amd/trainer.py
+++ b/ts-asr-whisper_amd/trainer.py
@@ -159,6 +159,40 @@
         self.counters = torch.zeros(1 + len(store.runs), dtype=torch.int32, device=dev)
         self.hyper = torch.zeros(len(store.runs), 3, dtype=F32, device=dev)
         self.is_pre = torch.tensor([int(pre) for _, _, pre in store.runs], dtype=torch.int32, device=dev)
+        self.table = None
+        self.table_covered = set()
+
+    def register_copies(self, matrices=()):
+        s = self.s
+        where = {id(p): o for p, o, _, _ in s.entries}
+        mats = {}
+        for p, dst, ld, dst_t, ld_t in matrices:
+            o = where.get(id(p))
+            if o is None or p.dim() != 2:
+                continue
+            R, Cc = p.shape
+            if ops.adamw_matrix_ok(R, Cc, o, dst, ld, dst_t, ld_t):
+                mats[o] = (p, R, Cc, dst, ld, dst_t, ld_t)
+        starts = sorted(mats)
+        pieces, covered, k = [], set(), 0
+        for i, (a, b, pre) in enumerate(s.runs):
+            cur = a
+            while k < len(starts) and starts[k] < b:
+                o = starts[k]
+                k += 1
+                p, R, Cc, dst, ld, dst_t, ld_t = mats[o]
+                if o > cur:
+                    pieces.append((cur, o - cur, i, pre))
+                pieces.append((o, R * Cc, i, pre, R, Cc, dst, ld, dst_t, ld_t))
+                covered.add(id(p))
+                cur = o + R * Cc
+            if b > cur:
+                pieces.append((cur, b - cur, i, pre))
+        self.table = ops.AdamwTable(pieces, s.params.device)
+        self.table_covered = covered
+
+    def clear_table(self):
+        self.table, self.table_covered = None, set()
 
     def sync_counters(self):
         self.counters.copy_(torch.tensor([self.t] + list(self.run_t), dtype=torch.int32))
@@ -189,6 +223,10 @@
                 int(self.schedule == "cosine"), float(self.betas[0]), float(self.betas[1]), L_.stream())
         self.gnorm_sq.zero_()
         ops.sumsq(s.grads, self.gnorm_sq)
+        if self.table is not None:
+            ops.adamw_table(self.table, s.params, s.grads, s.exp_avg, s.exp_avg_sq, self.hyper, self.betas[0], self.betas[1], self.eps,
+                            self.wd, gnorm_sq=self.gnorm_sq, max_norm=self.max_norm, preheat_only=preheat_only)
+            return
         for i, (a, b, pre) in enumerate(s.runs):
             if preheat_only and not pre:
                 continue
@@ -469,12 +507,13 @@
         self.store = FlatStore(model, preheat_prefixes)
         self.opt = FusedAdamW(self.store, lr, fddt_lr_multiplier, weight_decay=weight_decay, max_grad_norm=max_grad_norm,
                               warmup_steps=warmup_steps, max_steps=max_steps)
+        self.use_table = True
+        self._copies = None
         self.reducer = GradReducer(self.store, process_group)
         self.replica_sync = replica_sync
         self.replica_sync_bytes = sync_replicas(model, self.store, process_group, mode=replica_sync)
         if self.replica_sync_bytes and replica_sync == "broadcast":
-            model.model.encoder._sig = None
-            model.model.encoder._ctc_sig = None
+            self._stale_encoder()
             model._sig = None
         model.model.encoder._segment_hook = self.reducer.segment_ready
         model._segment_hook = self.reducer.segment_ready
@@ -521,13 +560,32 @@
             self.reducer.finish()
         if self.first_writer and not self.warmup_phase:
             self.store.settle_first_writers()
+        enc = self.model.model.encoder
+        self._ensure_table()
+        sig = enc._engine_sig() if self.opt.table is not None else None
+        valid = sig is not None and enc._sig is not None and enc._sig == sig
         with tracing.range("optimizer"):
             self.opt.step(preheat_only=self.warmup_phase)
-        enc = self.model.model.encoder
         if not (self.warmup_phase and self._preheat_is_vectors_only):
             enc._sig = None
             enc._ctc_sig = None
+            enc._fresh = (sig, self.opt.table_covered) if valid else None
         self._invalidate_decoder_copies()
+
+    def _ensure_table(self):
+        if not self.use_table or not self.store.params.is_cuda:
+            if self.opt.table is not None:
+                self.opt.clear_table()
+                self._copies = None
+            return
+        copies = self.model.model.encoder._engine(prepare=False).layer_copies()
+        if self.opt.table is None or copies is not self._copies:
+            self.opt.register_copies(copies)
+            self._copies = copies
+
+    def _stale_encoder(self):
+        enc = self.model.model.encoder
+        enc._sig = enc._ctc_sig = enc._fresh = None
 
     def _micro(self, batch, scale):
         if self.split_streams and self._can_split(batch):
@@ -612,11 +670,23 @@
             else:
                 dst[k].copy_(v, non_blocking=True)
 
-    def _invalidate_weight_copies(self):
+    def _invalidate_weight_copies(self, fresh=None):
         enc = self.model.model.encoder
         enc._sig = None
         enc._ctc_sig = None
+        enc._fresh = fresh
         self._invalidate_decoder_copies()
+
+    def _layers_token(self):
+        enc = self.model.model.encoder
+        self._ensure_table()
+        if self.opt.table is None:
+            return None
+        sig = enc._engine_sig()
+        if not ((enc._fresh is not None and enc._fresh[0] == sig) or (enc._sig is not None and enc._sig == sig)):
+            enc._sig = enc._fresh = None
+            enc._engine()
+        return (sig, self.opt.table_covered)
 
     def _graph_step(self, batch):
         if self.reducer.world > 1 or self.reducer.force:
@@ -631,13 +701,14 @@
         if key not in self._eager_done:
             self._eager_done.add(key)
             return self._eager_step([batch])
+        token = self._layers_token()
         if key not in self._graphs:
             while len(self._graphs) >= max(1, self.max_graphs):
                 self._graphs.popitem(last=False)
             if self._graph_pool is None:
                 self._graph_pool = torch.cuda.graph_pool_handle()
             static = self._clone(batch)
-            self._invalidate_weight_copies()
+            self._invalidate_weight_copies(token)
             torch.cuda.synchronize()
             g = torch.cuda.CUDAGraph()
             with torch.cuda.graph(g, pool=self._graph_pool):
@@ -652,7 +723,7 @@
         self._copy_into(static, batch)
         self.opt.advance(preheat_only=self.warmup_phase)
         g.replay()
-        self._invalidate_weight_copies()
+        self._invalidate_weight_copies(token)
         return loss.clone()
 
     def step(self, batch, eager=False):
@@ -693,8 +764,7 @@
         if self.replica_sync == "none" or self.reducer.world <= 1:
             return 0
         n = sync_replicas(self.model, self.store, self.reducer.pg, mode=self.replica_sync)
-        self.model.model.encoder._sig = None
-        self.model.model.encoder._ctc_sig = None
+        self._stale_encoder()
         self.model._sig = None
         return n
 
@@ -758,8 +828,7 @@
                               extra=(self.store.exp_avg, self.store.exp_avg_sq, self.opt.counters))
             p0 = self._sync_host_counters_phase(phase)
             phase = p0 if p0 is not None else phase
-            self.model.model.encoder._sig = None
-            self.model.model.encoder._ctc_sig = None
+            self._stale_encoder()
             self.model._sig = None
         sd = dict(sd, warmup_phase=phase)
         if bool(sd["warmup_phase"]) != self.warmup_phase:
```
